# Genesis-Embodied-AI/ThinShellLab

Measured on AMD Instinct MI355X. Metric: element-steps/s (fwd+adjoint), 100k-tri cloth; 1/2/4/8-GPU scaling, higher is better.
Workload: dtype f64

## Files before the change

thinshelllab_amd/csrc/direct_group.hpp:

```cpp
#pragma once
#include <condition_variable>
#include <functional>
#include <thread>
#include "direct_host.hpp"

struct GroupPool {
  std::vector<std::thread> th;
  std::mutex mu;
  std::condition_variable cv, cv_done;
  std::function<int(int)> job;
  std::vector<int> rc;
  std::vector<std::string> err;
  int gen = 0, pending = 0, dev = 0;
  bool stop = false;
  void start(int n, int device) {
    dev = device; rc.assign(n, 0); err.assign(n, "");
    for (int i = 1; i < n; i++) th.emplace_back([this, i] {
      (void)hipSetDevice(dev);
      int seen = 0;
      for (;;) {
        std::unique_lock<std::mutex> lk(mu);
        cv.wait(lk, [&] { return stop || gen != seen; });
        if (stop) return;
        seen = gen;
// ... 40 lines not shown
  std::vector<tsl_ctx*> m;
  tsl_ctx* g = nullptr;
  DevBuf<double> vals, cH, vb, vx, arena, sarena, garena, w;
  std::vector<size_t> vals_off, cH_off, vec_off;
  std::vector<int> nv_off, nc_off;
  std::vector<size_t> cap_a, cap_s, cap_g, cap_w, off_a, off_s, off_g, off_w;
  std::vector<long> seen_gen;
  bool merged_valid = false;
  bool flow_lost = false;
  std::vector<hipEvent_t> ev_m;
  hipEvent_t ev_g = nullptr;
  long n_merge = 0, n_relayout = 0, n_own_path = 0;
  double t_merge = 0;
  std::unique_ptr<GroupPool> pool;
  ~tsl_group();
};

static inline size_t grp_align(size_t n) { return (n + 31) & ~(size_t)31; }

static int group_ensure_arenas(tsl_ctx* c) {
  tsl_group* G = c->group;
  std::lock_guard<std::mutex> lk(G->mu_layout);
  int me = -1;
  for (size_t i = 0; i < G->m.size(); i++) if (G->m[i] == c) me = (int)i;
  if (me < 0) return tsl_fail("scene group: context is not a member");
  const DirectPlan& P = c->ds.plan;
  if ((size_t)P.arena <= G->cap_a[me] && (size_t)P.sarena <= G->cap_s[me] && (size_t)P.garena <= G->cap_g[me] && (size_t)P.ylen <= G->cap_w[me]) return 0;
  HIP_OK(hipDeviceSynchronize());
  auto grow = [&](std::vector<size_t>& cap, size_t need) { if (need > cap[me]) cap[me] = grp_align(need + need / 4 + 32); };
  grow(G->cap_a, (size_t)P.arena); grow(G->cap_s, (size_t)P.sarena); grow(G->cap_g, (size_t)P.garena); grow(G->cap_w, (size_t)P.ylen);
  const size_t n = G->m.size();
  auto lay = [&](const std::vector<size_t>& cap, std::vector<size_t>& off, DevBuf<double>& buf, const char* what) -> int {
    size_t tot = 0;
    for (size_t i = 0; i < n; i++) { off[i] = tot; tot += cap[i]; }
    if (buf.n < tot) { if (buf.alloc(tot + tot / 16 + 32)) return tsl_fail("scene group: out of device memory (%.2f GB of %s for %zu scenes)", tot * 8e-9, what, n); }
    return 0;
  };
  TSL_TRY(lay(G->cap_a, G->off_a, G->arena, "front panels")); TSL_TRY(lay(G->cap_s, G->off_s, G->sarena, "Schur complements"));
  TSL_TRY(lay(G->cap_g, G->off_g, G->garena, "G panels")); TSL_TRY(lay(G->cap_w, G->off_w, G->w, "sweep vectors"));
  for (size_t i = 0; i < n; i++) {
    DirectSolver& d = G->m[i]->ds;
    d.arena.view(G->arena.p + G->off_a[i], G->cap_a[i]); d.sarena.view(G->sarena.p + G->off_s[i], G->cap_s[i]);
    d.garena.view(G->garena.p + G->off_g[i], G->cap_g[i]); d.w.view(G->w.p + G->off_w[i], G->cap_w[i]);
    d.numeric_valid = false; d.have_factor = false; d.prezero_pending = false;
  }
  DirectSolver& gd = G->g->ds;
  gd.arena.view(G->arena.p, G->arena.n); gd.sarena.view(G->sarena.p, G->sarena.n); gd.garena.view(G->garena.p, G->garena.n); gd.w.view(G->w.p, G->w.n);
  gd.numeric_valid = false; gd.have_factor = false; gd.prezero_pending = false;
  G->merged_valid = false;
  G->n_relayout++;
  return 0;
}

static int group_merge(tsl_group* G) {
  const auto t0 = std::chrono::steady_clock::now();
  tsl_ctx* g = G->g;
  DirectSolver& gd = g->ds;
  DirectPlan& M = gd.plan;
  hipStream_t s = g->stream;
  const int n = (int)G->m.size();
  HIP_OK(hipStreamSynchronize(s));
  if (gd.zstream) HIP_OK(hipStreamSynchronize(gd.zstream));
  gd.prezero_pending = false;
  std::vector<int> sn_base(n + 1, 0), pmap_base(n + 1, 0), vtx_base(n + 1, 0), ch_base(n + 1, 0);
  int L = 0, nc_tot = 0;
  for (int i = 0; i < n; i++) {
    const DirectSolver& d = G->m[i]->ds;
    if (!d.plan_valid) return tsl_fail("scene group: member %d has no plan", i);
    const DirectPlan& P = d.plan;
    sn_base[i + 1] = sn_base[i] + (int)P.fr.size(); pmap_base[i + 1] = pmap_base[i] + (int)P.pmap.size();
    vtx_base[i + 1] = vtx_base[i] + (int)P.vtx.size(); ch_base[i + 1] = ch_base[i] + (int)P.ch_rec.size();
    L = std::max(L, P.n_levels);
    nc_tot += G->m[i]->nc;
    if ((long long)pmap_base[i] + (long long)P.pmap.size() > 0x7fffffffLL) return tsl_fail("scene group: child tables exceed 2^31 entries");
  }
  g->nc = nc_tot;
  M.n_cu = G->m[0]->ds.plan.n_cu; M.split_small = G->m[0]->ds.plan.split_small; M.split_rem = G->m[0]->ds.plan.split_rem;
  M.fr.resize(sn_base[n]); M.pmap.resize(pmap_base[n]); M.ch_rec.resize(ch_base[n]);
  std::vector<int> vtxp(vtx_base[n]), owner(sn_base[n]);
  M.arena = (long long)G->arena.n; M.sarena = (long long)G->sarena.n; M.garena = (long long)G->garena.n; M.ylen = (long long)G->w.n;
  M.flops = 0; M.leaf_ranges.clear(); M.arena_leaf = 0;
  std::vector<std::vector<int>> by_level(L);
  std::vector<int> all(n);
  for (int i = 0; i < n; i++) all[i] = i;
  TSL_TRY(G->pool->run(all, [&](int i) -> int {
    tsl_ctx* c = G->m[i];
    const DirectPlan& P = c->ds.plan;
    const long long oa = (long long)G->off_a[i], os = (long long)G->off_s[i], og = (long long)G->off_g[i];
    const int ow = (int)G->off_w[i];
    for (size_t q = 0; q < P.fr.size(); q++) {
      DsFrontDesc f = P.fr[q];
      f.off += oa; f.off21 += oa; f.soff += os; f.goff += og;
      if (f.parent >= 0) f.parent += sn_base[i];
      f.pmap_off += pmap_base[i]; f.vtx_off += vtx_base[i]; f.yoff += ow; f.ch_off += ch_base[i];
      for (int k = 0; k < std::min(4, f.nchild); k++) { f.cpm[k] += pmap_base[i]; f.cy[k] += ow; }
      M.fr[sn_base[i] + q] = f;
      owner[sn_base[i] + q] = i;
    }
    std::copy(P.pmap.begin(), P.pmap.end(), M.pmap.begin() + pmap_base[i]);
    for (size_t q = 0; q < P.vtx.size(); q++) vtxp[vtx_base[i] + q] = c->h_rowpos[P.vtx[q]] + G->nv_off[i];
    for (size_t q = 0; q < P.ch_rec.size(); q++) {
      DsChildRec r = P.ch_rec[q];
      r.soff += os; r.pmap_off += pmap_base[i]; r.sn += sn_base[i]; r.yoff += ow;
      M.ch_rec[ch_base[i] + q] = r;
    }
    return 0;
  }));
  for (int i = 0; i < n; i++) {
    const DirectPlan& P = G->m[i]->ds.plan;
    for (int l = 0; l < P.n_levels; l++)
      for (int q = P.level_ptr[l]; q < P.level_ptr[l + 1]; q++) by_level[l].push_back(sn_base[i] + P.level_sn[q]);
    M.flops += P.flops;
    M.leaf_ranges.push_back({(long long)G->off_a[i], P.arena_leaf});
    M.arena_leaf += P.arena_leaf;
  }
  M.build_levels(by_level);
  {
    const int wb = gd.gemv_wide_below;
    M.wl_front.clear(); M.wl_row.clear(); M.wl_own_ptr.assign(L + 1, 0); M.wl_bnd_ptr.assign(L, 0); M.wl_own_wide.assign(L, 0); M.wl_bnd_wide.assign(L, 0);
    for (int l = 0; l < L; l++) {
      auto wide = [&](int i, bool bnd) {
        const DirectPlan& P = G->m[i]->ds.plan;
        if (l >= P.n_levels) return false;
        const int cnt = bnd ? P.wl_own_ptr[l + 1] - P.wl_bnd_ptr[l] : P.wl_bnd_ptr[l] - P.wl_own_ptr[l];
        return wb > 0 && cnt < wb;
      };
      M.wl_own_ptr[l] = (int)M.wl_front.size();
      for (int part = 0; part < 2; part++) {
        if (part == 1) M.wl_own_wide[l] = (int)M.wl_front.size();
        for (int q = M.level_ptr[l]; q < M.level_ptr[l + 1]; q++) {
          const int sfr = M.level_sn[q];
          if ((int)wide(owner[sfr], false) != part) continue;
          for (int r = 0; r < M.fr[sfr].p; r += 16) { M.wl_front.push_back(sfr); M.wl_row.push_back(r); }
        }
      }
      M.wl_bnd_ptr[l] = (int)M.wl_front.size();
      for (int part = 0; part < 2; part++) {
        if (part == 1) M.wl_bnd_wide[l] = (int)M.wl_front.size();
        for (int q = M.level_ptr[l]; q < M.level_ptr[l + 1]; q++) {
          const int sfr = M.level_sn[q];
          if ((int)wide(owner[sfr], true) != part) continue;
          for (int r = 0; r < M.fr[sfr].b; r += 16) { M.wl_front.push_back(sfr); M.wl_row.push_back(r); }
        }
      }
    }
    M.wl_own_ptr[L] = (int)M.wl_front.size();
  }
  M.level_maxld.assign(L, 0);
  for (int l = 0; l < L; l++) for (int q = M.level_ptr[l]; q < M.level_ptr[l + 1]; q++) M.level_maxld[l] = std::max(M.level_maxld[l], M.fr[M.level_sn[q]].ld);
  size_t nbk = 0, ngr = 0, nge = 0;
  for (int i = 0; i < n; i++) { const DirectPlan& P = G->m[i]->ds.plan; nbk += P.blk_q.size(); ngr += P.cgr_dst.size(); nge += P.cgr_ent.size(); }
  std::vector<int> src(nbk), ld(nbk), cg_ptr, cg_ent, cg_ld;
  std::vector<long long> dst(nbk), cg_dst;
  cg_ptr.reserve(ngr + 1); cg_ent.reserve(nge); cg_ld.reserve(ngr); cg_dst.reserve(ngr);
  M.blk_lptr.assign(L + 1, 0); M.cgr_lptr.assign(L + 1, 0);
  {
    std::vector<size_t> at((size_t)L * n, 0);
    size_t o = 0;
    for (int l = 0; l < L; l++) {
      for (int i = 0; i < n; i++) {
        tsl_ctx* c = G->m[i];
        const DirectPlan& P = c->ds.plan;
        if (l >= P.n_levels) continue;
        if (G->vals_off[i] + c->vals.n > 0x7fffffffULL) return tsl_fail("scene group: matrix values exceed 2^31 doubles");
        at[(size_t)l * n + i] = o;
        o += (size_t)(P.blk_lptr[l + 1] - P.blk_lptr[l]);
        if (c->nc > 0 && !P.cgr_lptr.empty()) {
          const long long oa = (long long)G->off_a[i];
          const int eo = 16 * G->nc_off[i];
          for (int gq = P.cgr_lptr[l]; gq < P.cgr_lptr[l + 1]; gq++) {
            cg_ptr.push_back((int)cg_ent.size());
            for (int e = P.cgr_ptr[gq]; e < P.cgr_ptr[gq + 1]; e++) cg_ent.push_back(P.cgr_ent[e] + eo);
            cg_dst.push_back(P.cgr_dst[gq] + oa); cg_ld.push_back(P.cgr_ld[gq]);
          }
        }
      }
      M.blk_lptr[l + 1] = (int)o;
      M.cgr_lptr[l + 1] = (int)cg_dst.size();
    }
    cg_ptr.push_back((int)cg_ent.size());
    TSL_TRY(G->pool->run(all, [&](int i) -> int {
      tsl_ctx* c = G->m[i];
      const DirectPlan& P = c->ds.plan;
      const int vo = (int)G->vals_off[i];
      const long long oa = (long long)G->off_a[i];
      for (int l = 0; l < P.n_levels; l++) {
        size_t w = at[(size_t)l * n + i];
        for (int k = P.blk_lptr[l]; k < P.blk_lptr[l + 1]; k++, w++) { const int q = P.blk_q[k]; src[w] = c->ds.h_c2s[q] + vo; dst[w] = P.blk_dst[q] + oa; ld[w] = P.blk_ld[q]; }
      }
      return 0;
    }));
  }
  std::vector<DsFrontDesc> frl(M.level_sn.size());
  for (size_t i = 0; i < frl.size(); i++) frl[i] = M.fr[M.level_sn[i]];
  ds_pin_reset(gd, 16 * nbk + 2 * sizeof(DsFrontDesc) * M.fr.size() + sizeof(DsChildRec) * M.ch_rec.size() +
                       4 * (M.level_sn.size() + M.pmap.size() + vtxp.size() + M.wl_front.size() + M.wl_row.size()) + 20 * (cg_ent.size() + cg_ptr.size()) + 64 * 256);
  TSL_TRY(ds_upload_grow(gd.fr, M.fr, s, &gd)); TSL_TRY(ds_upload_grow(gd.frl, frl, s, &gd)); TSL_TRY(ds_upload_grow(gd.level_sn, M.level_sn, s, &gd));
  TSL_TRY(ds_upload_grow(gd.pmap, M.pmap, s, &gd)); TSL_TRY(ds_upload_grow(gd.ch_rec, M.ch_rec, s, &gd)); TSL_TRY(ds_upload_grow(gd.vtx, vtxp, s, &gd));
  TSL_TRY(ds_upload_grow(gd.blk_q, src, s, &gd)); TSL_TRY(ds_upload_grow(gd.blk_dst, dst, s, &gd)); TSL_TRY(ds_upload_grow(gd.blk_ld, ld, s, &gd));
  TSL_TRY(ds_upload_grow(gd.cgr_ptr, cg_ptr, s, &gd)); TSL_TRY(ds_upload_grow(gd.cgr_ent, cg_ent, s, &gd)); TSL_TRY(ds_upload_grow(gd.cgr_ld, cg_ld, s, &gd)); TSL_TRY(ds_upload_grow(gd.cgr_dst, cg_dst, s, &gd));
  TSL_TRY(ds_upload_grow(gd.wl_front, M.wl_front, s, &gd)); TSL_TRY(ds_upload_grow(gd.wl_row, M.wl_row, s, &gd));
  if (gd.scr.n < (size_t)M.scratch) { if (gd.scr.alloc((size_t)M.scratch + (size_t)M.scratch / 8)) return -1; }
  HIP_OK(hipStreamSynchronize(s));
  gd.plan_valid = true; gd.numeric_valid = false; gd.have_factor = false;
  for (int i = 0; i < n; i++) G->seen_gen[i] = G->m[i]->ds.plan_gen;
  G->merged_valid = true;
  G->n_merge++;
  G->t_merge += std::chrono::duration<double>(std::chrono::steady_clock::now() - t0).count();
  if (g->verbose >= 3)
    for (const DsBatch& b : M.batches) {
      fprintf(stderr, "[tsl]   merged level %2d: %5d fronts, pivots <= %4d, boundary <= %4d, dataflow workgroups %ld (cap %d)%s; fronts by padded pivot count:", b.level, b.count, b.max_pp, b.max_bp,
              ds_flow_wgs(M, b), gd.flow_cap, ds_use_small(gd, b) ? " (LDS kernel)" : "");
      for (int q = 0, run = 0; q < b.count; q++) {
        run++;
        if (q + 1 == b.count || M.fr[M.level_sn[b.first + q + 1]].pp != M.fr[M.level_sn[b.first + q]].pp) { fprintf(stderr, " %d x %d", run, M.fr[M.level_sn[b.first + q]].pp); run = 0; }
      }
      fprintf(stderr, "\n");
    }
  if (g->verbose >= 2)
    fprintf(stderr, "[tsl] scene group: merged plan of %d scenes: %zu fronts, %d levels, %zu batches, %.1f GFLOP per factorisation, %d constraints; host %.2f ms\n", n, M.fr.size(), L, M.batches.size(),
            M.flops * 1e-9, nc_tot, 1e3 * std::chrono::duration<double>(std::chrono::steady_clock::now() - t0).count());
  return 0;
}

static int group_create(tsl_ctx* const* ctxs, int n, tsl_group** out) {
  if (n < 1 || n > 64) return tsl_fail("tsl_group_create: 1..64 scenes");
  int dev = ctxs[0]->ds.device;
  for (int i = 0; i < n; i++) {
    if (ctxs[i]->group) return tsl_fail("tsl_group_create: scene %d is a member of another group", i);
    if (ctxs[i]->ds.device != dev) return tsl_fail("tsl_group_create: the scenes of a group live on one device");
    for (int j = 0; j < i; j++) if (ctxs[j] == ctxs[i]) return tsl_fail("tsl_group_create: scene %d listed twice", i);
  }
  HIP_OK(hipDeviceSynchronize());
  std::unique_ptr<tsl_group> G(new tsl_group());
  G->m.assign(ctxs, ctxs + n);
  G->vals_off.resize(n); G->cH_off.resize(n); G->vec_off.resize(n); G->nv_off.resize(n); G->nc_off.resize(n);
  for (auto* v : {&G->cap_a, &G->cap_s, &G->cap_g, &G->cap_w, &G->off_a, &G->off_s, &G->off_g, &G->off_w}) v->assign(n, 0);
  G->seen_gen.assign(n, -1);
  size_t tv = 0, th = 0, tx = 0;
  int tnv = 0, tnc = 0;
  for (int i = 0; i < n; i++) {
    tsl_ctx* c = ctxs[i];
    G->vals_off[i] = tv; tv += grp_align(c->vals.n);
    G->cH_off[i] = th; G->nc_off[i] = tnc; th += c->c_H.n; tnc += (int)(c->c_H.n / 144);
    G->vec_off[i] = tx; G->nv_off[i] = tnv; tx += 3 * (size_t)c->NV; tnv += c->NV;
    if (c->c_H.n % 144) return tsl_fail("tsl_group_create: contact block buffer of scene %d is not a multiple of 144 doubles", i);
  }
  TSL_TRY(G->vals.alloc(tv + 32)); TSL_TRY(G->cH.alloc(th + 144)); TSL_TRY(G->vb.alloc(tx + 32)); TSL_TRY(G->vx.alloc(tx + 32));
  HIP_OK(hipMemset(G->vals.p, 0, G->vals.n * sizeof(double)));
  tsl_ctx* g = new tsl_ctx();
  G->g = g;
  g->NV = tnv; g->nc = 0; g->verbose = ctxs[0]->verbose;
  HIP_OK(hipStreamCreateWithFlags(&g->stream, hipStreamNonBlocking));
  g->vals.view(G->vals.p, G->vals.n); g->c_H.view(G->cH.p, G->cH.n);
  DirectSolver& gd = g->ds;
  const DirectSolver& d0 = ctxs[0]->ds;
  gd.merged = true; gd.enable = 1; gd.device = dev; gd.flow = d0.flow; gd.small_rounds = d0.small_rounds * n; gd.xcd_map = d0.xcd_map; gd.gemv_wide_below = d0.gemv_wide_below;
  gd.g32_below = d0.g32_below; gd.piv_tol = d0.piv_tol; gd.prezero = d0.prezero;
  gd.static_ready = true;
  if (gd.bad.alloc(DS_BAD_INTS)) return -1;
  HIP_OK(hipFuncSetAttribute((const void*)k_ds_inv_small, hipFuncAttributeMaxDynamicSharedMemorySize, (int)ds_small_lds(DS_SMALL)));
  HIP_OK(hipEventCreateWithFlags(&G->ev_g, hipEventDisableTiming));
  G->ev_m.assign(n, nullptr);
  for (int i = 0; i < n; i++) HIP_OK(hipEventCreateWithFlags(&G->ev_m[i], hipEventDisableTiming));
  for (int i = 0; i < n; i++) {
    tsl_ctx* c = ctxs[i];
    auto copy = [&](const DevBuf<double>& b, double* dstp, size_t cnt) -> int {
      if (b.n && b.p) HIP_OK(hipMemcpy(dstp, b.p, std::min(b.n, cnt) * sizeof(double), hipMemcpyDeviceToDevice));
      return 0;
    };
    TSL_TRY(copy(c->vals, G->vals.p + G->vals_off[i], c->vals.n)); TSL_TRY(copy(c->c_H, G->cH.p + G->cH_off[i], c->c_H.n));
    TSL_TRY(copy(c->v_b, G->vb.p + G->vec_off[i], 3 * (size_t)c->NV)); TSL_TRY(copy(c->v_x, G->vx.p + G->vec_off[i], 3 * (size_t)c->NV));
    DirectSolver& d = c->ds;
    if (d.prezero_pending) { HIP_OK(hipEventSynchronize(d.ev_zero)); d.prezero_pending = false; }
  }
  HIP_OK(hipDeviceSynchronize());
  for (int i = 0; i < n; i++) {
    tsl_ctx* c = ctxs[i];
    const size_t nvals = c->vals.n, nch = c->c_H.n;
    c->vals.view(G->vals.p + G->vals_off[i], nvals); c->c_H.view(G->cH.p + G->cH_off[i], nch);
    c->v_b.view(G->vb.p + G->vec_off[i], 3 * (size_t)c->NV); c->v_x.view(G->vx.p + G->vec_off[i], 3 * (size_t)c->NV);
    DirectSolver& d = c->ds;
    d.arena.release(); d.sarena.release(); d.garena.release(); d.w.release();
    d.arena.view(nullptr, 0); d.sarena.view(nullptr, 0); d.garena.view(nullptr, 0); d.w.view(nullptr, 0);
    d.plan_valid = false; d.numeric_valid = false; d.have_factor = false; d.cons_checked = false;
    for (auto& sl : d.cache) sl->used = false;
  }
  for (int i = 0; i < n; i++) { ctxs[i]->group = G.get(); ctxs[i]->ds.token_lender = &gd; ctxs[i]->ds.keep_host_maps = true; ds_flow_token_release(ctxs[i]->ds); }
  G->pool.reset(new GroupPool());
  if (n > 1 && !getenv("TSL_GROUP_NO_THREADS")) G->pool->start(n, dev);
  *out = G.release();
  return 0;
}

static void group_destroy(tsl_group* G) {
  if (!G) return;
  G->pool.reset();
  (void)hipDeviceSynchronize();
  for (tsl_ctx* c : G->m) {
    auto give = [&](DevBuf<double>& b) {
      const double* src = b.p; const size_t cnt = b.n;
      b.view(nullptr, 0); b.release();
      if (cnt && b.alloc(cnt) == 0) (void)hipMemcpy(b.p, src, cnt * sizeof(double), hipMemcpyDeviceToDevice);
      else if (cnt) fprintf(stderr, "[tsl] scene group: out of device memory while a member took back a buffer of %zu doubles: the member is left with an EMPTY buffer (its next call fails loudly)\n", cnt);
    };
    give(c->vals); give(c->c_H); give(c->v_b); give(c->v_x);
    DirectSolver& d = c->ds;
    d.arena.release(); d.sarena.release(); d.garena.release(); d.w.release();
    d.plan_valid = false; d.numeric_valid = false; d.have_factor = false; d.cons_checked = false; d.prezero_pending = false;
    for (auto& sl : d.cache) sl->used = false;
    d.token_lender = nullptr; d.keep_host_maps = false;
    c->group = nullptr;
  }
  delete G;
}

tsl_group::~tsl_group() {
  pool.reset();
  if (g) {
    ds_flow_token_release(g->ds);
    DirectSolver& gd = g->ds;
    if (gd.zstream) (void)hipStreamDestroy(gd.zstream);
    for (int k = 0; k < DS_NSIDE; k++) if (gd.fstream[k]) (void)hipStreamDestroy(gd.fstream[k]);
    if (gd.pin) (void)hipHostFree(gd.pin);
    if (g->stream) (void)hipStreamDestroy(g->stream);
    delete g;
    g = nullptr;
  }
  for (hipEvent_t e : ev_m) if (e) (void)hipEventDestroy(e);
  if (ev_g) (void)hipEventDestroy(ev_g);
}
```

thinshelllab_amd/csrc/direct_host.hpp:

```cpp
#pragma once
#include <array>
#include <chrono>

#include "k_direct.hpp"
#include "tsl_ctx.hpp"

#include <cerrno>
#include <fcntl.h>
#include <sys/file.h>
#include <sys/stat.h>
#include <unistd.h>
static void ds_flow_token_acquire(DirectSolver& d) {
  char bus[64] = "dev";
  if (hipDeviceGetPCIBusId(bus, sizeof(bus), d.device) != hipSuccess) { (void)hipGetLastError(); snprintf(bus, sizeof(bus), "dev%d", d.device); }
  for (char* q = bus; *q; q++) if (*q == ':' || *q == '/') *q = '_';
  d.flow_token = -1; d.flow_token_asked = d.n_factor;
  for (const char* dir : {"/dev/shm", "/tmp"}) {
    const std::string path = std::string(dir) + "/tsl_flow_" + bus;
    int fd = open(path.c_str(), O_RDWR | O_CLOEXEC);
    if (fd < 0 && errno == ENOENT) {
      fd = open(path.c_str(), O_CREAT | O_RDWR | O_CLOEXEC, 0666);
      if (fd < 0 && (errno == ENOENT || errno == ENOTDIR)) continue;
      if (fd < 0 && errno == EEXIST) fd = open(path.c_str(), O_RDWR | O_CLOEXEC);
    } else if (fd < 0 && errno == ENOTDIR) continue;
    if (fd < 0) return;
    (void)fchmod(fd, 0666);
    if (flock(fd, LOCK_EX | LOCK_NB) == 0) { d.flow_token = 1; d.flow_token_fd = fd; }
    else close(fd);
    return;
  }
}
static void ds_flow_token_release(DirectSolver& d) {
  if (d.flow_token_fd >= 0) { (void)flock(d.flow_token_fd, LOCK_UN); close(d.flow_token_fd); }
  d.flow_token_fd = -1; d.flow_token = 0;
}
static bool ds_flow_token_held(DirectSolver& d) {
  if (d.token_lender) return ds_flow_token_held(*d.token_lender);
  if (d.flow_token == 0 || (d.flow_token < 0 && d.n_factor - d.flow_token_asked >= 256)) ds_flow_token_acquire(d);
  return d.flow_token > 0;
}

static inline int ds_nblk(long n, int b) { return (int)((n + b - 1) / b); }

static inline bool ds_use_small(const DirectSolver& d, const DsBatch& b) {
  if (b.max_pp > DS_SMALL) return false;
  return (size_t)b.count <= (size_t)d.plan.n_cu * ds_small_per_cu(b.max_pp) * (size_t)d.small_rounds;
}

static void ds_launch_gemm(hipStream_t s, const DsDev& D, const DsBatch& b, int mode, int ds_xcd_map, int ds_g32_below = 0, int part = 0, int max_lead = 0) {
  const int rows = mode == 0 ? b.max_pp : b.max_bp, cols = b.max_bp;
  const dim3 grid((cols + 63) / 64, (rows + 63) / 64, b.count);
  const long tiles = (long)grid.x * grid.y * grid.z;
  const int ta = (max_lead + 63) / 64;
  if (part == 1 && ta == 0) return;
  if (mode == 1 && part != 0) {
    hipLaunchKernelGGL((k_ds_gemm<1, 4>), part == 1 ? dim3(ta, ta, b.count) : grid, dim3(256), 0, s, D, b.first, part);
    return;
  }
  if (mode == 0 && ds_g32_below > 0 && tiles < ds_g32_below) {
    hipLaunchKernelGGL(k_ds_gemm_g32, dim3(part == 1 ? 2 * ta : (cols + 31) / 32, (rows + 31) / 32, b.count), dim3(256), 0, s, D, b.first, part);
    return;
  }
  if (mode == 0 && part != 0) {
    hipLaunchKernelGGL((k_ds_gemm<0, 4>), part == 1 ? dim3(ta, grid.y, b.count) : grid, dim3(256), 0, s, D, b.first, part);
    return;
  }
  if (ds_xcd_map > 0 && b.count >= ds_xcd_map) {
    const int gx = grid.x, gy = grid.y, nf = b.count;
    const long ng = ((long)nf + 7) / 8 * 8 * gx * gy;
    if (mode == 0) hipLaunchKernelGGL((k_ds_gemm_x<0, 4>), dim3((unsigned)ng), dim3(256), 0, s, D, b.first, gx, gy, nf);
    else hipLaunchKernelGGL((k_ds_gemm_x<1, 4>), dim3((unsigned)ng), dim3(256), 0, s, D, b.first, gx, gy, nf);
    return;
  }
  if (mode == 0) hipLaunchKernelGGL((k_ds_gemm<0, 4>), grid, dim3(256), 0, s, D, b.first, 0);
  else hipLaunchKernelGGL((k_ds_gemm<1, 4>), grid, dim3(256), 0, s, D, b.first, 0);
}
static void ds_launch_extend(hipStream_t s, const DsDev& D, int lv0, int nf, int max_ld, int part = 0, int max_span = 0) {
  const int xspan = part == 1 ? 64 * DS_XU : DS_XSPAN;
  const int nsp = ((part == 0 ? max_ld : max_span) + xspan - 1) / xspan;
  if (nsp <= 0) return;
  hipLaunchKernelGGL(k_ds_extend_panels, dim3(((max_ld / 3 + 2 + 3) / 4) * nsp, nf), dim3(256), 0, s, D, lv0, nsp, part, xspan);
}
static void ds_launch_level_start(tsl_ctx* c, hipStream_t s, const DsDev& D, int l, int part = 0, const DsBatch* b = nullptr) {
  DirectSolver& d = c->ds;
  const DirectPlan& P = d.plan;
  const int lv0 = P.level_ptr[l], nf = P.level_ptr[l + 1] - lv0;
  if (l > 0) ds_launch_extend(s, D, lv0, nf, P.level_maxld[l], part, part == 0 ? 0 : part == 1 ? b->max_pp : std::max(b->max_bp, b->max_pp));
  const int i0 = part == 2 ? P.blk_lmid[l] : P.blk_lptr[l], i1 = part == 1 ? P.blk_lmid[l] : P.blk_lptr[l + 1];
  const int nb = i1 - i0, npad = part == 2 ? 0 : nf;
  const long nt = (long)nb * 9 + (long)npad * DS_T;
  if (nt > 0)
    hipLaunchKernelGGL(k_ds_assemble_level, dim3(ds_nblk(nt, 256)), dim3(256), 0, s, i0, nb, (const int*)d.blk_q.p, (const double*)c->vals.p, (const long long*)d.blk_dst.p,
                       (const int*)d.blk_ld.p, lv0, npad, d.frl.p, d.arena.p, l == 0 ? 1 : 0);
  if (c->nc > 0) {
    const int g0 = part == 2 ? P.cgr_lmid[l] : P.cgr_lptr[l], g1 = part == 1 ? P.cgr_lmid[l] : P.cgr_lptr[l + 1];
    const int ng = g1 - g0;
    if (ng > 0) hipLaunchKernelGGL(k_ds_assemble_contacts_level, dim3(ds_nblk((long)ng * 64, 256)), dim3(256), 0, s, g0, ng, (const int*)d.cgr_ptr.p, (const int*)d.cgr_ent.p,
                                   (const long long*)d.cgr_dst.p, (const int*)d.cgr_ld.p, (const double*)c->c_H.p, d.arena.p);
  }
}


static long ds_flow_wgs(const DirectPlan& P, const DsBatch& b) {
  long n = 0;
  for (int z = 0; z < b.count; z++) { const long ns = (P.fr[P.level_sn[b.first + z]].pp / DS_T + DS_FLOW_B - 1) / DS_FLOW_B; n += ns * ns; }
  return n;
}
static bool ds_flow_eligible(DirectSolver& d, const DirectPlan& P, const DsBatch& b, hipStream_t s) {
  if (!d.flow || b.count > DS_FLOW_MAXF || b.max_pp < 2 * DS_T) return false;
  { hipStreamCaptureStatus cs = hipStreamCaptureStatusNone;
    if (hipStreamIsCapturing(s, &cs) != hipSuccess || cs != hipStreamCaptureStatusNone) return false; }
  if (!ds_flow_token_held(d)) return false;
  if (ds_use_small(d, b) && !(d.flow & 2)) return false;
  if (d.flow_cap == 0) {
    int occ = 0, dev = 0;
    hipDeviceProp_t prop;
    if (hipGetDevice(&dev) != hipSuccess || hipGetDeviceProperties(&prop, dev) != hipSuccess ||
        hipOccupancyMaxActiveBlocksPerMultiprocessor(&occ, (const void*)k_ds_gj_flow<DS_FLOW_B>, 256, 0) != hipSuccess) { d.flow_cap = -1; return false; }
    d.flow_cap = std::max(1, occ * prop.multiProcessorCount);
    if (getenv("TSL_FLOW_DEBUG")) fprintf(stderr, "[tsl] k_ds_gj_flow: %d workgroups per CU x %d CUs resident\n", occ, prop.multiProcessorCount);
  }
  return ds_flow_wgs(P, b) <= d.flow_cap;
}
static bool ds_flow_prepare(DirectSolver& d, const DirectPlan& P, const DsBatch& b, bool flow_free, DsFlowArgs& a, hipStream_t s) {
  if (!flow_free || !ds_flow_eligible(d, P, b, s)) return false;
  long wgs = 0, x = 0, fl = 0;
  for (int z = 0; z < b.count; z++) {
    const long nt = P.fr[P.level_sn[b.first + z]].pp / DS_T, ns = (nt + DS_FLOW_B - 1) / DS_FLOW_B;
    a.tile0[z] = (int)wgs; a.xoff[z] = x; a.foff[z] = (int)fl;
    wgs += ns * ns; x += (nt + 2 * nt * nt) * (DS_T * DS_T); fl += 32 * nt + 2 * nt * nt;
  }
  a.tile0[b.count] = (int)wgs; a.nf = b.count;
  if (d.flow_x.n < (size_t)x) { if (d.flow_x.alloc((size_t)x)) return false; }
  if (d.flow_f.n < (size_t)fl) {
    if (d.flow_f.alloc((size_t)fl + 1024)) return false;
    if (hipMemsetAsync(d.flow_f.p, 0, d.flow_f.n * sizeof(int), s) != hipSuccess) return false;
  }
  a.epoch = ++d.flow_epoch;
  return true;
}
#define DS_FLOW_PIECES 4
static std::vector<DsBatch> ds_flow_pieces(DirectSolver& d, const DirectPlan& P, const DsBatch& b, bool flow_free, hipStream_t s) {
  std::vector<DsBatch> out;
  if (!flow_free) return out;
  if (ds_flow_eligible(d, P, b, s)) { out.push_back(b); return out; }
  if (ds_use_small(d, b) || b.count < 2) return out;
  DsBatch one = b;
  one.count = 1;
  if (!ds_flow_eligible(d, P, one, s) || d.flow_cap <= 0) return out;
  int start = 0;
  while (start < b.count) {
    DsBatch pc{};
    pc.first = b.first + start; pc.level = b.level; pc.act_off = b.act_off;
    long wgs = 0;
    while (start + pc.count < b.count && pc.count < DS_FLOW_MAXF) {
      const DsFrontDesc& f = P.fr[P.level_sn[pc.first + pc.count]];
      const long ns = (f.pp / DS_T + DS_FLOW_B - 1) / DS_FLOW_B;
      if (pc.count > 0 && wgs + ns * ns > d.flow_cap) break;
      wgs += ns * ns; pc.count++;
      pc.max_pp = std::max(pc.max_pp, f.pp); pc.max_bp = std::max(pc.max_bp, f.bp); pc.max_ld = std::max(pc.max_ld, f.ld);
    }
    if (pc.max_pp < 2 * DS_T || !ds_flow_eligible(d, P, pc, s) || (int)out.size() == DS_FLOW_PIECES) { out.clear(); return out; }
    out.push_back(pc);
    start += pc.count;
  }
  return out;
}
static void ds_flow_launch(hipStream_t s, const DsDev& D, int lv0, const DsFlowArgs& fa, DirectSolver& d) {
  hipLaunchKernelGGL(k_ds_gj_flow<DS_FLOW_B>, dim3(fa.tile0[fa.nf]), dim3(256), 0, s, D, lv0, fa, d.flow_x.p, d.flow_f.p);
}

static bool direct_enabled(tsl_ctx* c) {
  DirectSolver& d = c->ds;
  if (d.enable == 0) return false;
  if (d.enable == 1) return true;
  for (const DsGrid& g : d.grids) if ((long)g.N * g.M >= 1024) return true;
  return false;
}

static DsDev ds_dev(tsl_ctx* c) {
  DirectSolver& d = c->ds;
  DsDev D;
  D.fr = d.fr.p; D.frl = d.frl.p; D.level_sn = d.level_sn.p; D.A = d.arena.p; D.S = d.sarena.p; D.Y = d.w.p; D.G = d.garena.p; D.scr = d.scr.p; D.ch = d.ch_rec.p; D.pmap = d.pmap.p; D.vtx = d.vtx.p; D.bad = d.bad.p; D.dbg = d.dbg; D.piv_tol = d.piv_tol;
  D.tlog = (d.dbg == 30 && d.tlog.n >= 1024) ? d.tlog.p : nullptr;
  return D;
}

static void ds_pin_reset(DirectSolver& d, size_t need) {
  if (d.pin_cap < need) {
    if (d.pin) (void)hipHostFree(d.pin);
    d.pin = nullptr; d.pin_cap = 0;
    void* p = nullptr;
    if (hipHostMalloc(&p, need + need / 4) == hipSuccess) { d.pin = (char*)p; d.pin_cap = need + need / 4; }
    else (void)hipGetLastError();
  }
  d.pin_off = 0;
}
static void* ds_pin_take(DirectSolver& d, size_t bytes) {
  const size_t o = (d.pin_off + 255) & ~(size_t)255;
  if (!d.pin || o + bytes > d.pin_cap) return nullptr;
  d.pin_off = o + bytes;
  return d.pin + o;
}
template <class T>
static int ds_upload_grow(DevBuf<T>& buf, const std::vector<T>& h, hipStream_t s, DirectSolver* d = nullptr) {
  if (buf.n < h.size()) { if (buf.alloc(h.size() + h.size() / 4 + 16)) return -1; }
  if (h.empty()) return 0;
  const void* src = h.data();
  if (d) if (void* st = ds_pin_take(*d, h.size() * sizeof(T))) { memcpy(st, h.data(), h.size() * sizeof(T)); src = st; }
  HIP_OK(hipMemcpyAsync(buf.p, src, h.size() * sizeof(T), hipMemcpyHostToDevice, s));
  return 0;
}

static int ds_upload_con(DirectSolver& d, hipStream_t s) {
  const DirectPlan& P = d.plan;
  TSL_TRY(ds_upload_grow(d.cgr_ptr, P.cgr_ptr, s, &d)); TSL_TRY(ds_upload_grow(d.cgr_ent, P.cgr_ent, s, &d)); TSL_TRY(ds_upload_grow(d.cgr_ld, P.cgr_ld, s, &d));
  TSL_TRY(ds_upload_grow(d.cgr_dst, P.cgr_dst, s, &d));
  return 0;
}

static int direct_static(tsl_ctx* c) {
  DirectSolver& d = c->ds;
  if (d.static_ready) return 0;
  const int NV = c->NV;
  d.row_ptr.assign(NV + 1, 0);
  for (int v = 0; v < NV; v++) d.row_ptr[v + 1] = d.row_ptr[v] + (int)c->h_rows[v].size();
  std::vector<int> c2s(d.row_ptr[NV]);
  for (int v = 0; v < NV; v++) {
    const int p = c->h_rowpos[v], s = p >> 6, lane = p & 63;
    for (int k = 0; k < (int)c->h_rows[v].size(); k++) c2s[d.row_ptr[v] + k] = (int)(((long)c->h_slice_off[s] + 64L * k) * 9 + lane);
  }
  d.h_c2s = c2s;
  if (d.bad.alloc(DS_BAD_INTS)) return -1;
  HIP_OK(hipFuncSetAttribute((const void*)k_ds_inv_small, hipFuncAttributeMaxDynamicSharedMemorySize, (int)ds_small_lds(DS_SMALL)));
  { hipDeviceProp_t prop;
    if (hipGetDeviceProperties(&prop, d.device) == hipSuccess && prop.multiProcessorCount > 0) d.plan.n_cu = prop.multiProcessorCount; else (void)hipGetLastError(); }
  d.plan.sym.build_partition(NV, c->h_rows, d.grids, d.blocks, d.leaf);
  d.cache.clear();
  d.static_ready = true;
  d.plan_valid = false;
  return 0;
}

static uint64_t ds_cons_key(const std::vector<int>& cons) {
  uint64_t h = 1469598103934665603ull;
  for (int v : cons) { h ^= (uint64_t)(uint32_t)v; h *= 1099511628211ull; }
  return h ^ (uint64_t)cons.size();
}
static void ds_swap_slot(DirectSolver& d, DsPlanSlot& sl) {
  std::swap(d.plan, sl.plan); d.h_cons.swap(sl.h_cons); d.h_cset.swap(sl.h_cset);
  if (!d.keep_host_maps) { d.plan.blk_dst.swap(sl.plan.blk_dst); d.plan.blk_ld.swap(sl.plan.blk_ld); d.plan.blk_q.swap(sl.plan.blk_q); d.plan.pmap.swap(sl.plan.pmap); }
  d.plan.lists.swap(sl.plan.lists); d.plan.locs.swap(sl.plan.locs); d.plan.tpos.swap(sl.plan.tpos);
  d.level_sn.swap(sl.level_sn); d.pmap.swap(sl.pmap); d.ch_rec.swap(sl.ch_rec); d.vtx.swap(sl.vtx); d.blk_ld.swap(sl.blk_ld); 
  d.wl_front.swap(sl.wl_front); d.wl_row.swap(sl.wl_row); d.blk_dst.swap(sl.blk_dst); d.fr.swap(sl.fr); d.frl.swap(sl.frl); d.blk_q.swap(sl.blk_q); d.cgr_ptr.swap(sl.cgr_ptr); d.cgr_ent.swap(sl.cgr_ent); d.cgr_ld.swap(sl.cgr_ld); d.cgr_dst.swap(sl.cgr_dst);
}

static size_t ds_slot_bytes(const DsPlanSlot& sl) {
  const DirectPlan& P = sl.plan;
  size_t b = 4 * (sl.level_sn.n + sl.pmap.n + sl.vtx.n + sl.blk_ld.n + sl.cgr_ptr.n + sl.cgr_ent.n + sl.cgr_ld.n + sl.wl_front.n + sl.wl_row.n + sl.blk_q.n) + 8 * (sl.blk_dst.n + sl.cgr_dst.n) +
             sizeof(DsFrontDesc) * (sl.fr.n + sl.frl.n) + sizeof(DsChildRec) * sl.ch_rec.n;
  b += 4 * (P.pmap.size() + P.vtx.size() + P.blk_ld.size() + P.blk_q.size() + P.wl_front.size() + P.wl_row.size() + P.level_sn.size()) + 8 * P.blk_dst.size() + sizeof(DsFrontDesc) * P.fr.size();
  return b;
}
static void ds_cache_trim(DirectSolver& d) {
  for (;;) {
    size_t total = 0;
    DsPlanSlot* lru = nullptr;
    for (auto& sl : d.cache) if (sl->used) { total += ds_slot_bytes(*sl); if (!lru || sl->stamp < lru->stamp) lru = sl.get(); }
    if (!lru || total <= (size_t)d.cache_mb << 20) return;
    lru->used = false;
    lru->level_sn.release(); lru->pmap.release(); lru->vtx.release(); lru->blk_ld.release(); lru->cgr_ptr.release(); lru->cgr_ent.release(); lru->cgr_ld.release(); lru->cgr_dst.release(); lru->wl_front.release(); lru->wl_row.release();
    lru->blk_q.release(); lru->blk_dst.release(); lru->fr.release(); lru->frl.release(); lru->ch_rec.release();
    d.n_plan_evicted++;
  }
}

static int group_ensure_arenas(tsl_ctx* c);
static int direct_plan(tsl_ctx* c) {
  DirectSolver& d = c->ds;
  if (d.merged) return 0;
  hipStream_t s = c->stream;
  TSL_TRY(direct_static(c));
  if (d.plan_valid && d.cons_checked) return 0;
  std::vector<int> cons((size_t)c->nc * 4);
  if (c->nc > 0) {
    HIP_OK(hipMemcpyAsync(cons.data(), c->c_idx.p, cons.size() * sizeof(int), hipMemcpyDeviceToHost, s));
    HIP_OK(hipStreamSynchronize(s));
  }
  d.cons_checked = true;
  if (d.plan_valid && cons == d.h_cons) return 0;
  std::vector<std::array<int, 4>> canon((size_t)c->nc);
  for (int e = 0; e < c->nc; e++) canon[e] = {cons[4 * e], cons[4 * e + 1], cons[4 * e + 2], cons[4 * e + 3]};
  std::sort(canon.begin(), canon.end());
  std::vector<int> cset((size_t)c->nc * 4);
  for (int e = 0; e < c->nc; e++) for (int k = 0; k < 4; k++) cset[4 * e + k] = canon[e][k];
  auto same_set_new_order = [&]() -> int {
    if (cons != d.h_cons) {
      HIP_OK(hipStreamSynchronize(s));
      if (d.plan.build_con(cons.data(), c->nc)) return tsl_fail("direct solver: constraint vertex outside its front");
      ds_pin_reset(d, 20 * (d.plan.cgr_ent.size() + d.plan.cgr_ptr.size()) + 4096);
      TSL_TRY(ds_upload_con(d, s));
      HIP_OK(hipStreamSynchronize(s));
      d.h_cons = cons;
      d.plan_gen++;
    }
    d.numeric_valid = false; d.have_factor = false;
    return 0;
  };
  if (d.plan_valid && cset == d.h_cset) return same_set_new_order();
  if (d.cache_cap > 0) {
    const uint64_t key = ds_cons_key(cset);
    HIP_OK(hipStreamSynchronize(s));
    for (auto& sl : d.cache)
      if (sl->used && sl->key == key && sl->h_cset == cset) {
        ds_swap_slot(d, *sl);
        sl->used = d.plan_valid; sl->key = ds_cons_key(sl->h_cset); sl->stamp = ++d.cache_clock;
        d.plan_valid = true;
        d.n_plan_hits++; d.plan_gen++;
        if (c->group) TSL_TRY(group_ensure_arenas(c));
        if (c->verbose >= 2) fprintf(stderr, "[tsl] direct plan: cached plan reused (nc %d, %d supernodes)\n", c->nc, d.plan.sym.n_sn);
        return same_set_new_order();
      }
    if (d.plan_valid) {
      DsPlanSlot* dst = nullptr;
      for (auto& sl : d.cache) if (!sl->used) { dst = sl.get(); break; }
      if (!dst && (int)d.cache.size() < d.cache_cap) {
        d.cache.emplace_back(new DsPlanSlot());
        dst = d.cache.back().get();
        dst->plan.sym.copy_partition(d.plan.sym); dst->plan.threads = d.plan.threads; dst->plan.n_cu = d.plan.n_cu; dst->plan.split_small = d.plan.split_small; dst->plan.split_rem = d.plan.split_rem;
      }
      if (!dst) { for (auto& sl : d.cache) if (!dst || sl->stamp < dst->stamp) dst = sl.get(); }
      ds_swap_slot(d, *dst);
      dst->used = true; dst->key = ds_cons_key(dst->h_cset); dst->stamp = ++d.cache_clock;
      d.plan_valid = false;
      ds_cache_trim(d);
    }
  }
  const auto t0 = std::chrono::steady_clock::now();
  const int rc = d.plan.build(c->h_rows, d.row_ptr, cons.data(), c->nc);
  const auto t_build = std::chrono::steady_clock::now();
  if (rc) return tsl_fail("direct solver: inconsistent elimination tree (code %d)", rc);
  DirectPlan& P = d.plan;
  std::vector<int> vtxp(P.vtx.size());
  for (size_t i = 0; i < vtxp.size(); i++) vtxp[i] = c->h_rowpos[P.vtx[i]];
  HIP_OK(hipStreamSynchronize(s));
  const size_t nbk = P.blk_q.size();
  ds_pin_reset(d, 16 * nbk + 2 * sizeof(DsFrontDesc) * P.fr.size() + sizeof(DsChildRec) * P.ch_rec.size() +
                      4 * (P.level_sn.size() + P.pmap.size() + vtxp.size() + P.wl_front.size() + P.wl_row.size()) + 20 * (P.cgr_ent.size() + P.cgr_ptr.size()) + 64 * 256);
  TSL_TRY(ds_upload_grow(d.fr, P.fr, s, &d)); TSL_TRY(ds_upload_grow(d.level_sn, P.level_sn, s, &d)); TSL_TRY(ds_upload_grow(d.pmap, P.pmap, s, &d)); TSL_TRY(ds_upload_grow(d.ch_rec, P.ch_rec, s, &d));
  TSL_TRY(ds_upload_grow(d.vtx, vtxp, s, &d));
  {
    std::vector<int> src_v, ld_v;
    std::vector<long long> dst_v;
    int* src_l = (int*)ds_pin_take(d, 4 * nbk); int* ld_l = (int*)ds_pin_take(d, 4 * nbk); long long* dst_l = (long long*)ds_pin_take(d, 8 * nbk);
    if (!src_l || !ld_l || !dst_l) { src_v.resize(nbk); ld_v.resize(nbk); dst_v.resize(nbk); src_l = src_v.data(); ld_l = ld_v.data(); dst_l = dst_v.data(); }
    ds_parallel_for((int)((nbk + 4095) / 4096), P.n_threads(), 1, [&](int, int ch) {
      for (size_t i = (size_t)ch * 4096; i < std::min(nbk, (size_t)(ch + 1) * 4096); i++) { const int q = P.blk_q[i]; src_l[i] = d.h_c2s[q]; dst_l[i] = P.blk_dst[q]; ld_l[i] = P.blk_ld[q]; }
    });
    if (d.blk_dst.n < nbk) { if (d.blk_dst.alloc(nbk + nbk / 4 + 16)) return -1; }
    if (d.blk_ld.n < nbk) { if (d.blk_ld.alloc(nbk + nbk / 4 + 16)) return -1; }
    if (d.blk_q.n < nbk) { if (d.blk_q.alloc(nbk + nbk / 4 + 16)) return -1; }
    if (nbk > 0) {
      HIP_OK(hipMemcpyAsync(d.blk_dst.p, dst_l, 8 * nbk, hipMemcpyHostToDevice, s));
      HIP_OK(hipMemcpyAsync(d.blk_ld.p, ld_l, 4 * nbk, hipMemcpyHostToDevice, s));
      HIP_OK(hipMemcpyAsync(d.blk_q.p, src_l, 4 * nbk, hipMemcpyHostToDevice, s));
      if (!src_v.empty()) HIP_OK(hipStreamSynchronize(s));
    }
  }
  TSL_TRY(ds_upload_con(d, s));
  std::vector<DsFrontDesc> frl(P.level_sn.size());
  for (size_t i = 0; i < frl.size(); i++) frl[i] = P.fr[P.level_sn[i]];
  TSL_TRY(ds_upload_grow(d.frl, frl, s, &d));
  TSL_TRY(ds_upload_grow(d.wl_front, P.wl_front, s, &d)); TSL_TRY(ds_upload_grow(d.wl_row, P.wl_row, s, &d));
  if (c->group) TSL_TRY(group_ensure_arenas(c));
  else {
    if (d.prezero_pending && d.arena.n < (size_t)P.arena) { HIP_OK(hipEventSynchronize(d.ev_zero)); d.prezero_pending = false; }
    if (d.arena.n < (size_t)P.arena) { if (d.arena.alloc((size_t)P.arena + (size_t)P.arena / 8)) return tsl_fail("direct solver: out of device memory (%.2f GB of front panels)", P.arena * 8e-9); }
    if (d.sarena.n < (size_t)P.sarena) { if (d.sarena.alloc((size_t)P.sarena + (size_t)P.sarena / 8 + 16)) return tsl_fail("direct solver: out of device memory (%.2f GB of Schur complements)", P.sarena * 8e-9); }
    if (d.garena.n < (size_t)P.garena) { if (d.garena.alloc((size_t)P.garena + (size_t)P.garena / 8 + 16)) return tsl_fail("direct solver: out of device memory (G arena)"); }
    if (d.w.n < (size_t)P.ylen) { if (d.w.alloc((size_t)P.ylen + (size_t)P.ylen / 4 + 16)) return -1; }
  }
  if (d.scr.n < (size_t)P.scratch) { if (d.scr.alloc((size_t)P.scratch + (size_t)P.scratch / 8)) return -1; }
  HIP_OK(hipStreamSynchronize(s));
  d.h_cons.swap(cons); d.h_cset.swap(cset);
  d.plan_valid = true;
  d.numeric_valid = false;
  d.have_factor = false;
  d.n_plans++; d.plan_gen++;
  d.t_plan += std::chrono::duration<double>(std::chrono::steady_clock::now() - t0).count();
  if (c->verbose >= 2)
    fprintf(stderr, "[tsl] direct plan: %d supernodes, %d levels, %zu batches, %.2f + %.2f GB of panels + Schur complements, %.1f GFLOP per factorisation, nc %d; host %.2f ms (tree + maps %.2f)\n", P.sym.n_sn, P.n_levels, P.batches.size(), P.arena * 8e-9, P.sarena * 8e-9,
            P.flops * 1e-9, c->nc, 1e3 * std::chrono::duration<double>(std::chrono::steady_clock::now() - t0).count(), 1e3 * std::chrono::duration<double>(t_build - t0).count());
  if (c->verbose >= 2) fprintf(stderr, "[tsl]   plan phases (ms): tree %.2f, descriptors + parent maps %.2f, levels %.2f, static block map %.2f, contact map %.2f\n", P.phase_ms[0], P.phase_ms[1], P.phase_ms[2], P.phase_ms[3], P.phase_ms[4]);
  if (c->verbose >= 3)
    for (const DsBatch& b : P.batches) {
      fprintf(stderr, "[tsl]   level %2d: %5d fronts, pivots <= %4d, boundary <= %4d%s; fronts by padded pivot count:", b.level, b.count, b.max_pp, b.max_bp, ds_use_small(d, b) ? " (LDS kernel)" : "");
      for (int q = 0, run = 0; q < b.count; q++) {
        run++;
        if (q + 1 == b.count || P.fr[P.level_sn[b.first + q + 1]].pp != P.fr[P.level_sn[b.first + q]].pp) { fprintf(stderr, " %d x %d", run, P.fr[P.level_sn[b.first + q]].pp); run = 0; }
      }
      fprintf(stderr, "\n");
    }
  return 0;
}

static int direct_prezero(tsl_ctx* c) {
  DirectSolver& d = c->ds;
  if (!d.prezero || !d.plan_valid || d.arena.n == 0 || d.prezero_pending) return 0;
  if (d.zstream == nullptr) {
    HIP_OK(hipStreamCreateWithFlags(&d.zstream, hipStreamNonBlocking));
    HIP_OK(hipEventCreateWithFlags(&d.ev_zfork, hipEventDisableTiming));
    HIP_OK(hipEventCreateWithFlags(&d.ev_zero, hipEventDisableTiming));
  }
  HIP_OK(hipEventRecord(d.ev_zfork, c->stream));
  HIP_OK(hipStreamWaitEvent(d.zstream, d.ev_zfork, 0));
  d.prezero_n = (size_t)d.plan.arena_leaf;
  if (d.plan.leaf_ranges.empty()) HIP_OK(hipMemsetAsync(d.arena.p, 0, d.prezero_n * sizeof(double), d.zstream));
  else for (const auto& r : d.plan.leaf_ranges) HIP_OK(hipMemsetAsync(d.arena.p + r.first, 0, (size_t)r.second * sizeof(double), d.zstream));
  HIP_OK(hipEventRecord(d.ev_zero, d.zstream));
  d.prezero_pending = true;
  d.numeric_valid = false; d.have_factor = false;
  return 0;
}

static void ds_launch_gemv(hipStream_t s, const DsDev& D, DirectSolver& d, int o, int n, int mode, const double* vin, double* vout, int wide_from = -1) {
  if (n <= 0) return;
  if (wide_from >= 0) {
    const int n0 = wide_from - o, n1 = o + n - wide_from;
    if (n0 > 0) hipLaunchKernelGGL(k_ds_gemv, dim3(n0), dim3(256), 0, s, D, d.wl_front.p, d.wl_row.p, o, mode, vin, vout);
    if (n1 > 0) hipLaunchKernelGGL(k_ds_gemv_wide, dim3(4 * n1), dim3(256), 0, s, D, d.wl_front.p, d.wl_row.p, wide_from, mode, vin, vout);
    return;
  }
  if (d.gemv_wide_below > 0 && n < d.gemv_wide_below) hipLaunchKernelGGL(k_ds_gemv_wide, dim3(4 * n), dim3(256), 0, s, D, d.wl_front.p, d.wl_row.p, o, mode, vin, vout);
  else hipLaunchKernelGGL(k_ds_gemv, dim3(n), dim3(256), 0, s, D, d.wl_front.p, d.wl_row.p, o, mode, vin, vout);
}
static void ds_sweep_up_level(hipStream_t s, const DsDev& D, DirectSolver& d, int l, const double* r, double* z) {
  const DirectPlan& P = d.plan;
  const int o0 = P.wl_own_ptr[l], b0 = P.wl_bnd_ptr[l], o1 = P.wl_own_ptr[l + 1];
  ds_launch_gemv(s, D, d, o0, b0 - o0, 0, r, z, P.wl_own_wide.empty() ? -1 : P.wl_own_wide[l]);
  ds_launch_gemv(s, D, d, b0, o1 - b0, 1, (const double*)z, nullptr, P.wl_bnd_wide.empty() ? -1 : P.wl_bnd_wide[l]);
}
static int direct_factor(tsl_ctx* c, int stop_sn = -1, const char* dump_path = nullptr, const double* eager_r = nullptr, double* eager_z = nullptr) {
  DirectSolver& d = c->ds;
  hipStream_t s = c->stream;
  TSL_TRY(direct_plan(c));
  if (d.numeric_valid) return 0;
  d.eager_n = 0;
  const DirectPlan& P = d.plan;
  const DsDev D = ds_dev(c);
  if (d.prezero_pending) {
    HIP_OK(hipStreamWaitEvent(s, d.ev_zero, 0));
    d.prezero_pending = false;
    if (P.leaf_ranges.empty() && d.prezero_n < (size_t)P.arena_leaf) HIP_OK(hipMemsetAsync(d.arena.p + d.prezero_n, 0, ((size_t)P.arena_leaf - d.prezero_n) * sizeof(double), s));
  } else if (P.leaf_ranges.empty()) HIP_OK(hipMemsetAsync(d.arena.p, 0, (size_t)P.arena_leaf * sizeof(double), s));
  else for (const auto& r : P.leaf_ranges) HIP_OK(hipMemsetAsync(d.arena.p + r.first, 0, (size_t)r.second * sizeof(double), s));
  HIP_OK(hipMemsetAsync(d.bad.p, 0, 8 * sizeof(int), s));
  bool swept_at_root = false;
  int flow_wgs_sent = 0;
  auto invert_batch = [&](const DsBatch& b, hipStream_t bs, bool& flow_free) {
    const int lv0 = b.first, nf = b.count;
    const int tp = b.max_pp / DS_T;
    bool flowed = false;
    {
      const std::vector<DsBatch> pieces = ds_flow_pieces(d, P, b, flow_free, bs);
      std::vector<DsFlowArgs> fas(pieces.size());
      bool ready = !pieces.empty();
      for (size_t i = 0; ready && i < pieces.size(); i++) ready = ds_flow_prepare(d, P, pieces[i], true, fas[i], bs);
      if (ready) {
        for (size_t i = 0; i < pieces.size(); i++) { ds_flow_launch(bs, D, pieces[i].first, fas[i], d); d.n_flow++; flow_wgs_sent += fas[i].tile0[fas[i].nf]; }
        flowed = true; flow_free = false;
      }
    }
    if (flowed) {}
    else if (ds_use_small(d, b)) hipLaunchKernelGGL(k_ds_inv_small, dim3(nf), dim3(256), ds_small_lds(b.max_pp), bs, D, lv0, b.max_pp + 1);
    else {
      hipLaunchKernelGGL(k_ds_pivot0, dim3(nf), dim3(256), 0, bs, D, lv0);
      for (int k = 0; k < tp; k++) { const int na = P.act_n[b.act_off + k]; hipLaunchKernelGGL(k_ds_gj_step, dim3(na + na * tp * tp), dim3(256), 0, bs, D, lv0, k, tp, na); }
      hipLaunchKernelGGL(k_ds_gj_finish, dim3(tp, nf), dim3(256), 0, bs, D, lv0);
    }
  };
  auto run_batch = [&](const DsBatch& b, hipStream_t bs, bool& flow_free) {
    invert_batch(b, bs, flow_free);
    if (b.max_bp > 0) {
      ds_launch_gemm(bs, D, b, 0, d.xcd_map, d.g32_below);
      ds_launch_gemm(bs, D, b, 1, d.xcd_map);
    }
  };
  auto side_streams = [&]() -> int {
    if (d.fstream[0] == nullptr)
      for (int k = 0; k < DS_NSIDE; k++) { HIP_OK(hipStreamCreateWithFlags(&d.fstream[k], hipStreamNonBlocking)); HIP_OK(hipEventCreateWithFlags(&d.ev_fjoin[k], hipEventDisableTiming)); }
    if (d.ev_ffork == nullptr) HIP_OK(hipEventCreateWithFlags(&d.ev_ffork, hipEventDisableTiming));
    for (int k = 0; k < 5; k++) if (d.ev_la[k] == nullptr) HIP_OK(hipEventCreateWithFlags(&d.ev_la[k], hipEventDisableTiming));
    if (d.lastream == nullptr) {
      int lo = 0, hi = 0;
      HIP_OK(hipDeviceGetStreamPriorityRange(&lo, &hi));
      HIP_OK(hipStreamCreateWithPriority(&d.lastream, hipStreamNonBlocking, lo));
    }
    return 0;
  };
  const bool la_on = (d.lookahead & 1) && stop_sn < 0 && !P.blk_lmid.empty() && P.la_from < P.n_levels && ds_flow_token_held(d);
  if (la_on) TSL_TRY(side_streams());
  hipStream_t ls = d.lastream;
  enum { LA_W = 0, LA_GA = 1, LA_A = 2, LA_REST = 3, LA_DRAIN = 4 };
  for (size_t bi = 0; bi < P.batches.size();) {
    size_t be = bi;
    while (be < P.batches.size() && P.batches[be].level == P.batches[bi].level) be++;
    bool stop_here = false;
    if (stop_sn >= 0) for (int q = P.batches[bi].first; q < P.batches[be - 1].first + P.batches[be - 1].count; q++) stop_here |= P.level_sn[q] == stop_sn;
    const int lvl = P.batches[bi].level;
    const bool la_level = la_on && lvl >= P.la_from;
    const bool la_in = la_level && lvl > P.la_from;
    if (la_in) {
      ds_launch_level_start(c, s, D, lvl, 1, &P.batches[bi]);
      HIP_OK(hipStreamWaitEvent(ls, d.ev_la[LA_A], 0));
      ds_launch_level_start(c, ls, D, lvl, 2, &P.batches[bi]);
      HIP_OK(hipEventRecord(d.ev_la[LA_REST], ls));
    } else
    ds_launch_level_start(c, s, D, lvl);
    if (la_level) {
      const DsBatch& b = P.batches[bi];
      bool flow_free = true;
      if (la_in && ds_flow_wgs(P, b) > P.n_cu) {
// ... 36 lines not shown
    }
    if (stop_here) {
      const DsFrontDesc& f = P.fr[stop_sn];
      std::vector<double> h((size_t)f.pp * f.ld);
      HIP_OK(hipStreamSynchronize(s));
      HIP_OK(hipMemcpy(h.data(), d.arena.p + f.off, h.size() * sizeof(double), hipMemcpyDeviceToHost));
      if (FILE* fp = fopen(dump_path, "wb")) {
        const int hdr[8] = {f.p, f.pp, f.b, f.bp, f.ld, f.nv_own, f.nv_bnd, 0};
        fwrite(hdr, sizeof(int), 8, fp);
        fwrite(&P.vtx[f.vtx_off], sizeof(int), (size_t)f.nv_own + f.nv_bnd, fp);
        fwrite(h.data(), sizeof(double), h.size(), fp);
        fclose(fp);
      }
      d.numeric_valid = false; d.have_factor = false;
      return 0;
    }
    const int nside = (int)std::min<size_t>(be - bi - 1, DS_NSIDE);
    if (nside > 0) {
      TSL_TRY(side_streams());
      HIP_OK(hipEventRecord(d.ev_ffork, s));
      for (int k = 0; k < nside; k++) HIP_OK(hipStreamWaitEvent(d.fstream[k], d.ev_ffork, 0));
    }
    bool flow_free = true;
    for (size_t q = bi; q < be; q++) {
      const int k = (int)(q - bi);
      run_batch(P.batches[q], (nside > 0 && k > 0) ? d.fstream[(k - 1) % nside] : s, flow_free);
    }
    for (int k = 0; k < nside; k++) { HIP_OK(hipEventRecord(d.ev_fjoin[k], d.fstream[k])); HIP_OK(hipStreamWaitEvent(s, d.ev_fjoin[k], 0)); }
    bi = be;
  }
  if (++d.anorm_age >= 64) d.anorm_valid = false;
  if (stop_sn >= 0 || c->verbose >= 2) HIP_OK(hipStreamSynchronize(s));
  if (d.dbg == 30) {
    if (d.tlog.n < 1024) { if (d.tlog.alloc(1024)) return -1; HIP_OK(hipMemset(d.tlog.p, 0, 1024 * sizeof(unsigned long long))); HIP_OK(hipMemset(d.tlog.p + 194, 0xff, sizeof(unsigned long long))); }
    else {
      unsigned long long h[1024];
      HIP_OK(hipStreamSynchronize(s));
      HIP_OK(hipMemcpy(h, d.tlog.p, sizeof(h), hipMemcpyDeviceToHost));
      int khz = 100000;
      (void)hipDeviceGetAttribute(&khz, hipDeviceAttributeWallClockRate, d.device);
      auto us = [&](unsigned long long t) { return t ? (double)(long long)(t - h[192]) * 1e3 / khz : -1.0; };
      fprintf(stderr, "[tsl] dataflow chain of the last launch (us since its start): pivot published | step finished by the last workgroup | by the first of the last super-row; first workgroup started at %.2f, last ended at %.2f\n", us(h[194]), us(h[193]));
      for (int k = 0; k < 64 && (h[k] || h[64 + k]); k++) {
        fprintf(stderr, "[tsl]   %2d  %8.2f (+%5.2f)   %8.2f   %8.2f   | owner of the pivot, relative to the publication of the previous one: flags seen, operands in LDS, R' done, tile updated, inverted:", k, us(h[k]), k ? us(h[k]) - us(h[k - 1]) : 0.0, us(h[64 + k]), us(h[128 + k]));
        for (int i = 0; i < 5; i++) fprintf(stderr, " %6.2f", h[256 + 8 * k + i] && k ? us(h[256 + 8 * k + i]) - us(h[k - 1]) : 0.0);
        fprintf(stderr, "\n");
      }
      HIP_OK(hipMemset(d.tlog.p, 0, 1024 * sizeof(unsigned long long)));
      HIP_OK(hipMemset(d.tlog.p + 194, 0xff, sizeof(unsigned long long)));
    }
  }
  if (swept_at_root) HIP_OK(hipStreamWaitEvent(s, d.ev_la[LA_DRAIN], 0));
  HIP_OK(hipGetLastError());
  d.flow_wgs_last = flow_wgs_sent;
  d.numeric_valid = true;
  d.have_factor = true;
  d.n_factor++;
  return 0;
}

static int direct_anorm(tsl_ctx* c) {
  DirectSolver& d = c->ds;
  if (d.anorm_valid) return 0;
  hipStream_t s = c->stream;
  if (d.anorm_dev.n == 0 && d.anorm_dev.alloc(1)) return -1;
  if (d.h_anorm == nullptr) HIP_OK(hipHostMalloc((void**)&d.h_anorm, sizeof(double)));
  HIP_OK(hipMemsetAsync(d.anorm_dev.p, 0, sizeof(double), s));
  hipLaunchKernelGGL(k_ds_rownorm, dim3(ds_nblk(c->NV, 256)), dim3(256), 0, s, c->NV, c->slice_off.p, c->slice_len.p, c->vals.p, d.anorm_dev.p);
  HIP_OK(hipMemcpyAsync(d.h_anorm, d.anorm_dev.p, sizeof(double), hipMemcpyDeviceToHost, s));
  HIP_OK(hipStreamSynchronize(s));
  d.anorm = *d.h_anorm;
  d.anorm_valid = true; d.anorm_age = 0;
  return 0;
}

static int direct_apply(tsl_ctx* c, const double* r, double* z) {
  DirectSolver& d = c->ds;
  hipStream_t s = c->stream;
  const DirectPlan& P = d.plan;
  const DsDev D = ds_dev(c);
  const int l0 = (d.eager_n > 0 && r == d.eager_r && z == d.eager_z) ? d.eager_n : 0;
  d.eager_n = 0;
  for (int l = l0; l < P.n_levels; l++) ds_sweep_up_level(s, D, d, l, r, z);
  for (int l = P.n_levels - 2; l >= 0; l--) {
    const int o0 = P.wl_own_ptr[l], b0 = P.wl_bnd_ptr[l];
    ds_launch_gemv(s, D, d, o0, b0 - o0, 2, (const double*)z, z, P.wl_own_wide.empty() ? -1 : P.wl_own_wide[l]);
  }
  d.n_apply++;
  return 0;
}

static int direct_bench(tsl_ctx* c, int cls, int reps, double* out) {
  DirectSolver& d = c->ds;
  hipStream_t s = c->stream;
  if (!d.plan_valid || d.arena.n == 0) return tsl_fail("tsl_bench_direct: no factorisation yet");
  if (d.prezero_pending) { HIP_OK(hipStreamWaitEvent(s, d.ev_zero, 0)); d.prezero_pending = false; }
  const DirectPlan& P = d.plan;
  if (!d.have_factor) {
    HIP_OK(hipMemsetAsync(d.arena.p, 0x3F, (size_t)P.arena * sizeof(double), s));
    HIP_OK(hipMemsetAsync(d.sarena.p, 0x3F, (size_t)P.sarena * sizeof(double), s));
    HIP_OK(hipMemsetAsync(d.garena.p, 0x3F, (size_t)P.garena * sizeof(double), s));
  }
  const DsDev D = ds_dev(c);
  if (cls == 0 || cls == 3 || cls == 5) {
    HIP_OK(hipMemsetAsync(d.arena.p, 0x3F, (size_t)P.arena * sizeof(double), s));
    hipLaunchKernelGGL(k_ds_bench_diag, dim3((unsigned)P.fr.size()), dim3(256), 0, s, D);
    d.have_factor = false;
  }
  double flops = 0, bytes = 0;
  long launches = 0;
  auto child_entries = [&](const DsFrontDesc& f, double& to_s, double& to_panels) {
    to_s = 0; to_panels = 0;
    for (int q = f.ch_off; q < f.ch_off + f.nchild; q++) {
      const DsChildRec& cr = P.ch_rec[q];
      const double nb = cr.nb, b = cr.b;
      to_s += nb * nb; to_panels += b * b - nb * nb;
    }
  };
  auto issue = [&](bool count) {
    if (cls == 4) {
      (void)direct_apply(c, c->v_b.p, c->v_t4.p);
      d.n_apply--;
      if (count) {
        for (int l = 0; l < P.n_levels; l++) launches += 1 + (P.wl_own_ptr[l + 1] > P.wl_bnd_ptr[l]) + (l < P.n_levels - 1);
        for (const DsFrontDesc& f : P.fr) { bytes += 8.0 * ((double)f.p * f.p + 2.0 * (double)f.p * f.b); flops += 2.0 * ((double)f.p * f.p + 2.0 * (double)f.p * f.b); }
      }
      return;
    }
    if (cls == 7) {
      const int bq = d.bench_batch;
      if (bq < 1 || bq >= (int)P.batches.size()) return;
      const DsBatch& bf = P.batches[bq];
      const DsBatch& bg = P.batches[bq - 1];
      DsFlowArgs fa;
      if (!ds_flow_prepare(d, P, bf, true, fa, s) || bg.max_bp == 0) return;
      (void)hipEventRecord(d.ev_ffork, s);
      (void)hipStreamWaitEvent(d.fstream[0], d.ev_ffork, 0);
      ds_flow_launch(s, D, bf.first, fa, d);
      ds_launch_gemm(d.fstream[0], D, bg, 0, d.xcd_map, d.g32_below);
      ds_launch_gemm(d.fstream[0], D, bg, 1, d.xcd_map);
      (void)hipEventRecord(d.ev_fjoin[0], d.fstream[0]);
      (void)hipStreamWaitEvent(s, d.ev_fjoin[0], 0);
      if (count) launches++;
      return;
    }
    int bi = -1;
    for (const DsBatch& b : P.batches) {
      bi++;
      if (d.bench_batch >= 0 && bi != d.bench_batch) continue;
      const int lv0 = b.first, nf = b.count;
      const int tp = b.max_pp / DS_T, tb = b.max_bp / DS_T;
      if (cls == 6) {
        if (b.level == 0) continue;
        ds_launch_extend(s, D, b.first, b.count, b.max_pp + b.max_bp);
        if (count) {
          launches++;
          for (int i = 0; i < nf; i++) {
            const DsFrontDesc& f = P.fr[P.level_sn[lv0 + i]];
            double to_s, to_p;
            child_entries(f, to_s, to_p);
            bytes += 8.0 * (to_p + (double)f.pp * f.ld + (double)f.bp * f.pp); flops += to_p;
          }
        }
      } else if (cls == 0 || cls == 3 || cls == 5) {
        bool flow_free = true;
        for (int q = 0; q < bi; q++) if (P.batches[q].level == b.level && !ds_flow_pieces(d, P, P.batches[q], true, s).empty()) flow_free = false;
        const std::vector<DsBatch> pieces = ds_flow_pieces(d, P, b, flow_free, s);
        const int mine = !pieces.empty() ? 5 : (ds_use_small(d, b) ? 3 : 0);
        if (mine != cls) continue;
        if (cls == 5) { for (const DsBatch& pc : pieces) { DsFlowArgs fa; if (ds_flow_prepare(d, P, pc, true, fa, s)) { ds_flow_launch(s, D, pc.first, fa, d); if (count) launches++; } } }
        else if (cls == 3) { hipLaunchKernelGGL(k_ds_inv_small, dim3(nf), dim3(256), ds_small_lds(b.max_pp), s, D, lv0, b.max_pp + 1); if (count) launches++; }
        else {
          hipLaunchKernelGGL(k_ds_pivot0, dim3(nf), dim3(256), 0, s, D, lv0);
          for (int k = 0; k < tp; k++) { const int na = P.act_n[b.act_off + k]; hipLaunchKernelGGL(k_ds_gj_step, dim3(na + na * tp * tp), dim3(256), 0, s, D, lv0, k, tp, na); }
          hipLaunchKernelGGL(k_ds_gj_finish, dim3(tp, nf), dim3(256), 0, s, D, lv0);
          if (count) launches += tp + 2;
        }
        if (count) for (int i = 0; i < nf; i++) {
          const DsFrontDesc& f = P.fr[P.level_sn[lv0 + i]];
          flops += 2.0 * (double)f.pp * f.pp * f.pp;
          bytes += 16.0 * (double)f.pp * f.pp * (cls != 0 ? 1.0 : f.pp / (double)DS_T);
        }
      } else if (tb > 0) {
        if (cls == 1 || cls == 2) ds_launch_gemm(s, D, b, cls == 2 ? 0 : 1, d.xcd_map, cls == 2 ? d.g32_below : 0);
        else continue;
        if (count) {
          launches++;
          for (int i = 0; i < nf; i++) {
            const DsFrontDesc& f = P.fr[P.level_sn[lv0 + i]];
            if (cls == 1) {
              double to_s, to_p;
              child_entries(f, to_s, to_p);
              flops += 2.0 * (double)f.bp * f.bp * f.pp; bytes += 8.0 * (2.0 * (double)f.bp * f.pp + (double)f.b * f.b + to_s);
            } else { flops += 2.0 * (double)f.pp * f.pp * f.bp; bytes += 8.0 * ((double)f.pp * f.pp + 2.0 * (double)f.pp * f.bp); }
          }
        }
      }
    }
  };
  if (d.ev0 == nullptr) { HIP_OK(hipEventCreate(&d.ev0)); HIP_OK(hipEventCreate(&d.ev1)); }
  if (cls == 7) {
    if (d.fstream[0] == nullptr)
      for (int k = 0; k < DS_NSIDE; k++) { HIP_OK(hipStreamCreateWithFlags(&d.fstream[k], hipStreamNonBlocking)); HIP_OK(hipEventCreateWithFlags(&d.ev_fjoin[k], hipEventDisableTiming)); }
    if (d.ev_ffork == nullptr) HIP_OK(hipEventCreateWithFlags(&d.ev_ffork, hipEventDisableTiming));
  }
  issue(true);
  HIP_OK(hipEventRecord(d.ev0, s));
  for (int r = 0; r < reps; r++) issue(false);
  HIP_OK(hipEventRecord(d.ev1, s));
  HIP_OK(hipEventSynchronize(d.ev1));
  HIP_OK(hipGetLastError());
  float ms = 0;
  HIP_OK(hipEventElapsedTime(&ms, d.ev0, d.ev1));
  d.numeric_valid = false; d.have_factor = false;
  out[0] = launches > 0 ? ms * 1e3 / ((double)launches * reps) : 0.0;
  out[1] = launches > 0 ? flops / launches : 0.0;
  out[2] = launches > 0 ? bytes / launches : 0.0;
  out[3] = (double)launches;
  return 0;
}
```

thinshelllab_amd/csrc/direct_plan.hpp:

```cpp
#pragma once
#include <atomic>
#include <chrono>
#include <thread>
#include "direct_sym.hpp"

#define DS_T 32
#define DS_SMALL 128
static inline size_t ds_small_lds(int max_pp) { return (size_t)max_pp * (max_pp + 1) * sizeof(double); }
static inline int ds_small_per_cu(int max_pp) { return (int)std::max<size_t>(1, std::min<size_t>(8, (160 * 1024) / (ds_small_lds(max_pp) + 5 * 1024))); }

struct DsFrontDesc {
  long long off;
  long long off21;
  long long soff;
  long long goff;
  int p, pp, b, bp, ld;
  int parent;
  int pmap_off;
  int vtx_off;
  int nv_own, nv_bnd;
  int scr_off;
  int yoff;
  int cpm[4], cy[4];
  int ch_off, nchild;
  int lead;
};
struct DsChildRec {
  long long soff;
  int bp, b;
  int pmap_off;
  int sn;
  int nb;
  int yoff;
};

struct DsBatch {
  int first, count, level;
  int max_pp, max_ld, max_bp;
  int act_off;
};

template <class F>
static void ds_parallel_for(int n, int nt, int chunk, F body) {
  nt = std::max(1, std::min(nt, (n + chunk - 1) / chunk));
  if (nt == 1) { for (int i = 0; i < n; i++) body(0, i); return; }
  std::atomic<int> next{0};
  auto work = [&](int t) {
    for (;;) {
      const int i0 = next.fetch_add(chunk);
      if (i0 >= n) break;
      for (int i = i0; i < std::min(n, i0 + chunk); i++) body(t, i);
    }
  };
  std::vector<std::thread> th;
  for (int t = 1; t < nt; t++) th.emplace_back(work, t);
  work(0);
  for (auto& x : th) x.join();
}

struct DirectPlan {
  DirectSym sym;
  std::vector<DsFrontDesc> fr;
  std::vector<int> pmap, vtx;
  std::vector<DsChildRec> ch_rec;
  std::vector<long long> blk_dst;
  std::vector<int> blk_ld;
  std::vector<int> blk_q, blk_lptr;
  std::vector<int> blk_lmid, cgr_lmid;
  int la_from = 1 << 30;
  std::vector<long long> con_dst;
  std::vector<int> con_ld, con_lvl;
  std::vector<int> cgr_lptr, cgr_ptr, cgr_ent, cgr_ld;
  std::vector<long long> cgr_dst;
  std::vector<int> level_maxld;
  long long arena_leaf = 0;
  std::vector<std::pair<long long, long long>> leaf_ranges;
  std::vector<int> wl_own_wide, wl_bnd_wide;
  std::vector<std::vector<int>> lists;
  std::vector<int> level_ptr, level_sn;
  std::vector<DsBatch> batches;
  std::vector<int> act_n, act_ld;
  std::vector<int> sweep_cache; int sweep_cache_L0 = -1;
  std::vector<int> wl_front, wl_row, wl_own_ptr, wl_bnd_ptr;
  int n_levels = 0;
  long long arena = 0;
  long long sarena = 0;
  long long garena = 0;
  long long ylen = 0;
  long long scratch = 0;
  double phase_ms[6] = {0, 0, 0, 0, 0, 0};
  std::vector<int> tpos;
  std::vector<std::vector<int>> locs;
  int threads = 0;
  int n_cu = 256;
  bool split_small = true, split_rem = true;
  int n_threads() const { return threads > 0 ? threads : (int)std::max(1u, std::min(8u, std::thread::hardware_concurrency())); }
  double flops = 0;

  static int pad(int n) { return (n + DS_T - 1) / DS_T * DS_T; }

  int local_dof(int s, int v) const {
    const int l = sym.local(s, v);
    if (l < 0) return -1;
    const int no = sym.own(s);
    return l < no ? 3 * l : fr[s].pp + 3 * (l - no);
  }
  static long long panel_addr(const DsFrontDesc& f, int lr, int lc, int* ld_out) {
    if (lr < f.pp) { *ld_out = f.ld; return f.off + (long long)lr * f.ld + lc; }
    if (lc >= f.pp) { *ld_out = 0; return -1; }
    *ld_out = f.pp;
    return f.off21 + (long long)(lr - f.pp) * f.pp + lc;
  }

  void build_levels(std::vector<std::vector<int>>& by_level) {
    const int L = (int)by_level.size();
    n_levels = L;
    level_ptr.assign(L + 1, 0); level_sn.clear();
    batches.clear(); act_n.clear(); act_ld.clear();
    wl_front.clear(); wl_row.clear(); wl_own_ptr.assign(L + 1, 0); wl_bnd_ptr.assign(L, 0);
    sweep_cache_L0 = -1;
    scratch = 0;
    for (int l = 0; l < L; l++) {
      std::vector<int>& fl = by_level[l];
      std::stable_sort(fl.begin(), fl.end(), [&](int a, int b) { return fr[a].pp > fr[b].pp; });
      long long scr = 0;
      for (size_t i = 0; i < fl.size(); i++) {
        const int s = fl[i];
        DsFrontDesc& f = fr[s];
        if (i == 0 || 4 * f.pp <= batches.back().max_pp || (fl.size() > 256 && batches.back().count >= 32 && f.pp < fr[fl[i - 1]].pp) ||
            (split_small && batches.back().max_pp > DS_SMALL && f.pp <= DS_SMALL && 2 * f.pp <= batches.back().max_pp)) {
          DsBatch b{};
          b.first = (int)level_sn.size(); b.count = 0; b.level = l;
          batches.push_back(b);
        }
        DsBatch& b = batches.back();
        b.count++;
        b.max_pp = std::max(b.max_pp, f.pp); b.max_ld = std::max(b.max_ld, f.ld); b.max_bp = std::max(b.max_bp, f.bp);
        level_sn.push_back(s);
        f.scr_off = (int)scr;
        scr += 2LL * DS_T * DS_T + 4LL * DS_T * f.pp;
      }
      if (split_rem)
        for (size_t q = 0; q < batches.size(); q++) {
          DsBatch& b = batches[q];
          if (b.level != l || b.max_pp > DS_SMALL) continue;
          const int cap = n_cu * ds_small_per_cu(b.max_pp), rem = b.count % cap;
          if (b.count <= cap || rem == 0 || rem > cap / 8) continue;
          DsBatch r{};
          r.first = b.first + b.count - rem; r.count = rem; r.level = l;
          b.count -= rem;
          for (int z = 0; z < r.count; z++) { const DsFrontDesc& f = fr[level_sn[r.first + z]]; r.max_pp = std::max(r.max_pp, f.pp); r.max_ld = std::max(r.max_ld, f.ld); r.max_bp = std::max(r.max_bp, f.bp); }
          b.max_ld = 0; b.max_bp = 0;
          for (int z = 0; z < b.count; z++) { const DsFrontDesc& f = fr[level_sn[b.first + z]]; b.max_ld = std::max(b.max_ld, f.ld); b.max_bp = std::max(b.max_bp, f.bp); }
          batches.insert(batches.begin() + q + 1, r);
          q++;
        }
      level_ptr[l + 1] = (int)level_sn.size();
      scratch = std::max(scratch, scr);
      wl_own_ptr[l] = (int)wl_front.size();
      for (int s : fl) for (int r = 0; r < fr[s].p; r += 16) { wl_front.push_back(s); wl_row.push_back(r); }
      wl_bnd_ptr[l] = (int)wl_front.size();
      for (int s : fl) for (int r = 0; r < fr[s].b; r += 16) { wl_front.push_back(s); wl_row.push_back(r); }
    }
    wl_own_ptr[L] = (int)wl_front.size();
    {
      std::vector<int> nb(L, 0);
      for (const DsBatch& b : batches) nb[b.level]++;
      int l0 = L;
      while (l0 > 0 && nb[l0 - 1] == 1) l0--;
      la_from = (L - l0 >= 2) ? std::max(l0, 1) : (1 << 30);
    }
    for (DsBatch& b : batches) {
      b.act_off = (int)act_n.size();
      for (int k = 0; k * DS_T < b.max_pp; k++) {
        int n = 0, mld = 0;
        while (n < b.count && fr[level_sn[b.first + n]].pp > k * DS_T) { mld = std::max(mld, fr[level_sn[b.first + n]].ld); n++; }
        act_n.push_back(n); act_ld.push_back(mld);
      }
    }
  }

  int build(const std::vector<std::vector<int>>& adj, const std::vector<int>& row_ptr, const int* cons, int n_cons) {
    auto tick = std::chrono::steady_clock::now();
    auto lap = [&](int k) { const auto n = std::chrono::steady_clock::now(); phase_ms[k] = 1e3 * std::chrono::duration<double>(n - tick).count(); tick = n; };
    sym.build_tree(adj, cons, n_cons, 4);
    lap(0);
    const int S = sym.n_sn;
    fr.assign(S, DsFrontDesc{});
    pmap.clear(); vtx.clear(); ch_rec.clear();
    arena = 0; sarena = 0; garena = 0; flops = 0; ylen = 0;
    for (int s = 0; s < S; s++) {
      DsFrontDesc& f = fr[s];
      f.nv_own = sym.own(s); f.nv_bnd = (int)sym.bnd[s].size();
      f.p = 3 * f.nv_own; f.b = 3 * f.nv_bnd;
      f.pp = pad(f.p); f.bp = pad(f.b); f.ld = f.pp + f.bp;
      f.parent = sym.parent[s];
      f.vtx_off = (int)vtx.size();
      for (int q = sym.sn_ptr[s]; q < sym.sn_ptr[s + 1]; q++) vtx.push_back(sym.order[q]);
      for (int v : sym.bnd[s]) vtx.push_back(v);
      const double p = f.pp, b = f.bp;
      flops += 2.0 * p * p * p + 2.0 * p * p * b + 2.0 * p * b * b;
    }
    {
      std::vector<int> cnt(sym.n_levels + 1, 0), ord(S);
      for (int s = 0; s < S; s++) cnt[sym.level[s] + 1]++;
      for (int l = 0; l < sym.n_levels; l++) cnt[l + 1] += cnt[l];
      for (int s = 0; s < S; s++) ord[cnt[sym.level[s]]++] = s;
      for (int s : ord) {
        DsFrontDesc& f = fr[s];
        f.off = arena; f.off21 = arena + (long long)f.pp * f.ld;
        arena += (long long)f.pp * f.ld + (long long)f.bp * f.pp;
        f.soff = sarena; sarena += (long long)f.bp * f.bp;
        f.goff = garena; garena += (long long)f.pp * f.bp;
        f.yoff = (int)ylen; ylen += f.bp;
      }
    }
    {
      std::vector<int> cptr(S + 1, 0);
      for (int s = 0; s < S; s++) if (fr[s].parent >= 0) { cptr[fr[s].parent + 1]++; fr[fr[s].parent].nchild++; }
      for (int s = 0; s < S; s++) cptr[s + 1] += cptr[s];
      ch_rec.assign(cptr[S], DsChildRec{});
      long long total = 0;
      { std::vector<int> fill(cptr.begin(), cptr.end() - 1);
        for (int s = 0; s < S; s++) { fr[s].ch_off = cptr[s]; if (fr[s].parent >= 0) { fr[s].pmap_off = (int)total; total += fr[fr[s].parent].ld; ch_rec[fill[fr[s].parent]++].sn = s; } } }
      if (total > 0x7fffffffLL) return -1;
      pmap.assign((size_t)total, -1);
      if (locs.empty()) locs.resize(1);
      std::vector<int>& lc = locs[0];
      if ((int)lc.size() != sym.NV) lc.assign(sym.NV, -1);
      bool bad = false;
      for (int p = 0; p < S; p++) {
        if (cptr[p] == cptr[p + 1]) continue;
        const DsFrontDesc& f = fr[p];
        const int* fv = &vtx[f.vtx_off];
        for (int i = 0; i < f.nv_own; i++) lc[fv[i]] = 3 * i;
        for (int i = 0; i < f.nv_bnd; i++) lc[fv[f.nv_own + i]] = f.pp + 3 * i;
        for (int q = cptr[p]; q < cptr[p + 1]; q++) {
          DsChildRec& cr = ch_rec[q];
          const DsFrontDesc& ch = fr[cr.sn];
          cr.soff = ch.soff; cr.bp = ch.bp; cr.b = ch.b; cr.pmap_off = ch.pmap_off; cr.yoff = ch.yoff;
          if (q - cptr[p] < 4) { fr[p].cpm[q - cptr[p]] = ch.pmap_off; fr[p].cy[q - cptr[p]] = ch.yoff; }
          const int* cv = &vtx[ch.vtx_off + ch.nv_own];
          int* pm = &pmap[ch.pmap_off];
          int prev = -1;
          for (int i = 0; i < ch.nv_bnd; i++) {
            const int l = lc[cv[i]];
            if (l < 0 || l <= prev) { bad = true; continue; }
            prev = l;
            pm[l] = 3 * i; pm[l + 1] = 3 * i + 1; pm[l + 2] = 3 * i + 2;
            if (l >= f.pp) cr.nb += 3;
          }
          fr[cr.sn].lead = ch.b - cr.nb;
        }
        for (int i = 0; i < f.nv_own + f.nv_bnd; i++) lc[fv[i]] = -1;
      }
      if (bad) return -1;
      for (int s = 0; s < S; s++) if (fr[s].parent < 0 && fr[s].nv_bnd > 0) return -1;
    }
    lap(1);
    {
      std::vector<std::vector<int>> by_level(sym.n_levels);
      for (int s = 0; s < S; s++) by_level[sym.level[s]].push_back(s);
      build_levels(by_level);
    }
    const int L = sym.n_levels;
    const std::vector<int>& alap = sym.level;
    lap(2);
    const int NV = sym.NV;
    if ((int)tpos.size() != row_ptr[NV]) {
      tpos.assign(row_ptr[NV], -1);
      for (int r = 0; r < NV; r++)
        for (int k = 0; k < (int)adj[r].size(); k++) {
          const int c = adj[r][k];
          const auto& rc = adj[c];
          const auto it = std::lower_bound(rc.begin(), rc.end(), r);
          if (it != rc.end() && *it == r) tpos[row_ptr[r] + k] = row_ptr[c] + (int)(it - rc.begin());
        }
    }
    blk_dst.resize(row_ptr[NV]); blk_ld.resize(row_ptr[NV]);
    {
      const int nt = n_threads();
      if ((int)locs.size() < nt) locs.resize(nt);
      if ((int)lists.size() < 2 * nt * L) lists.resize((size_t)2 * nt * L);
      for (auto& v : lists) v.clear();
      std::atomic<int> bad{0};
      std::atomic<long long> written{0};
      ds_parallel_for(S, nt, 16, [&](int t, int s) {
        std::vector<int>& loc = locs[t];
        if ((int)loc.size() != NV) loc.assign(NV, -1);
        std::vector<int>& mine11 = lists[2 * ((size_t)t * L + alap[s])];
        std::vector<int>& mine = lists[2 * ((size_t)t * L + alap[s]) + 1];
        const DsFrontDesc& f = fr[s];
        const int no = f.nv_own;
        long long nw = 0;
        const int* fv = &vtx[f.vtx_off];
        for (int i = 0; i < no; i++) loc[fv[i]] = 3 * i;
        for (int i = 0; i < f.nv_bnd; i++) loc[fv[no + i]] = f.pp + 3 * i;
        for (int i = 0; i < no; i++) {
          const int r = fv[i];
          const auto& row = adj[r];
          for (int k = 0; k < (int)row.size(); k++) {
            const int c = row[k];
            if (sym.sn_of[c] < s) continue;
            const int lc = loc[c];
            if (lc < 0) { bad = 1; continue; }
            const int q = row_ptr[r] + k;
            blk_dst[q] = f.off + (long long)(3 * i) * f.ld + lc; blk_ld[q] = f.ld; nw++; (lc < f.pp ? mine11 : mine).push_back(q);
            if (sym.sn_of[c] > s) {
              const int qt = tpos[q];
              if (qt >= 0) { blk_dst[qt] = f.off21 + (long long)(lc - f.pp) * f.pp + 3 * i; blk_ld[qt] = f.pp; nw++; mine.push_back(qt); }
            }
          }
        }
        for (int i = 0; i < no + f.nv_bnd; i++) loc[fv[i]] = -1;
        written += nw;
      });
      if (bad || written != row_ptr[NV]) return -2;
      blk_q.resize(row_ptr[NV]); blk_lptr.assign(L + 1, 0); blk_lmid.assign(L, 0);
      size_t o = 0;
      for (int l = 0; l < L; l++) {
        for (int part = 0; part < 2; part++) {
          for (int t = 0; t < nt; t++) { const std::vector<int>& v = lists[2 * ((size_t)t * L + l) + part]; std::copy(v.begin(), v.end(), blk_q.begin() + o); o += v.size(); }
          if (part == 0) blk_lmid[l] = (int)o;
        }
        blk_lptr[l + 1] = (int)o;
      }
    }
    arena_leaf = 0;
    for (int q = level_ptr[0]; q < level_ptr[1]; q++) { const DsFrontDesc& f = fr[level_sn[q]]; arena_leaf = std::max(arena_leaf, f.off21 + (long long)f.bp * f.pp); }
    level_maxld.assign(L, 0);
    for (int l = 0; l < L; l++) for (int q = level_ptr[l]; q < level_ptr[l + 1]; q++) level_maxld[l] = std::max(level_maxld[l], fr[level_sn[q]].ld);
    lap(3);
    const int rc = build_con(cons, n_cons);
    lap(4);
    return rc;
  }

  int build_con(const int* cons, int n_cons) {
    con_dst.assign((size_t)n_cons * 16, -1); con_ld.assign((size_t)n_cons * 16, 0); con_lvl.assign((size_t)n_cons * 16, 0);
    for (int e = 0; e < n_cons; e++)
      for (int a = 0; a < 4; a++)
        for (int b = 0; b < 4; b++) {
          const int va = cons[4 * e + a], vb = cons[4 * e + b];
          const int s = std::min(sym.sn_of[va], sym.sn_of[vb]);
          const int lr = local_dof(s, va), lc = local_dof(s, vb);
          if (lr < 0 || lc < 0) return -3;
          int ldq = 0;
          const long long dst = panel_addr(fr[s], lr, lc, &ldq);
          if (dst < 0) return -3;
          con_dst[(size_t)e * 16 + a * 4 + b] = dst;
          con_ld[(size_t)e * 16 + a * 4 + b] = ldq;
          con_lvl[(size_t)e * 16 + a * 4 + b] = 2 * sym.level[s] + ((lr < fr[s].pp && lc < fr[s].pp) ? 0 : 1);
        }
    {
      const size_t n = (size_t)n_cons * 16;
      std::vector<int> ord(n);
      for (size_t i = 0; i < n; i++) ord[i] = (int)i;
      std::sort(ord.begin(), ord.end(), [&](int x, int y) {
        if (con_lvl[x] != con_lvl[y]) return con_lvl[x] < con_lvl[y];
        if (con_dst[x] != con_dst[y]) return con_dst[x] < con_dst[y];
        return x < y;
      });
      cgr_lptr.assign(n_levels + 1, 0); cgr_lmid.assign(n_levels, 0); cgr_ptr.clear(); cgr_ent.assign(ord.begin(), ord.end()); cgr_ld.clear(); cgr_dst.clear();
      for (size_t i = 0; i < n; i++) {
        const int x = ord[i];
        if (i == 0 || con_dst[x] != con_dst[ord[i - 1]] || con_lvl[x] != con_lvl[ord[i - 1]]) {
          cgr_ptr.push_back((int)i); cgr_dst.push_back(con_dst[x]); cgr_ld.push_back(con_ld[x]);
          cgr_lptr[(con_lvl[x] >> 1) + 1]++;
          if ((con_lvl[x] & 1) == 0) cgr_lmid[con_lvl[x] >> 1]++;
        }
      }
      cgr_ptr.push_back((int)n);
      for (int l = 0; l < n_levels; l++) { cgr_lmid[l] += cgr_lptr[l]; cgr_lptr[l + 1] += cgr_lptr[l]; }
    }
    return 0;
  }
};
```

thinshelllab_amd/csrc/k_direct.hpp:

```cpp
#pragma once
#include "direct_plan.hpp"
#include "tsl_device.hpp"

typedef double ds_d4 __attribute__((ext_vector_type(4)));

struct DsDev {
  const DsFrontDesc* fr;
  const DsFrontDesc* frl;
  const int* level_sn;
  double* A;
  double* S;
  double* G;
  double* scr;
  double* Y;
  const DsChildRec* ch;
  const int* pmap;
  const int* vtx;
  int* bad;
  double piv_tol;
  int dbg;
  unsigned long long* tlog;
};

__global__ void k_ds_rownorm(int NV, const int* __restrict__ slice_off, const int* __restrict__ slice_len, const double* __restrict__ vals, double* out) {
// ... 867 lines not shown
  }
}

#define DS_SK 32
#define DS_GMC 8
template <int mode, int WPC>
TSL_DEV void ds_gemm_tile(const DsDev& D, int lv0, int bx, int by, int bz, int part = 0) {
  constexpr int SA = DS_SK + 1, SB = 64 + 1;
  __shared__ double As[64 * SA];
  __shared__ double Bs[DS_SK * SB];
  const DsFrontDesc f = D.frl[lv0 + bz];
  const int Mr = mode == 0 ? f.pp : f.bp, Nc = f.bp, K = f.pp;
  const int I0 = by * 64, J0 = bx * 64;
  if (I0 >= Mr || J0 >= Nc) return;
  if (mode == 1 && part != 0 && ((I0 < f.lead && J0 < f.lead) != (part == 1))) return;
  if (mode == 0 && part != 0 && ((J0 < f.lead) != (part == 1))) return;
  const double* F = D.A + f.off;
  double* G = D.G + f.goff;
  const int ld = f.ld, pp = f.pp;
  const double* Am = mode == 0 ? F : D.A + f.off21;
  const int lda = mode == 0 ? ld : pp;
  const double* Bm = mode == 0 ? F + pp : G;
  const int ldb = mode == 0 ? ld : f.bp;
  const int lane = threadIdx.x & 63, w = threadIdx.x >> 6;
  const int wi = w >> 1, wj = w & 1;
  const int lr = lane & 15, lk = lane >> 4;
  const bool rows_hi = I0 + 32 < Mr, cols_hi = J0 + 32 < Nc;
  ds_d4 acc[2][2];
#pragma unroll
  for (int a = 0; a < 2; a++)
#pragma unroll
    for (int b = 0; b < 2; b++) acc[a][b] = ds_d4{0.0, 0.0, 0.0, 0.0};
  const int tx = threadIdx.x & 31, ty = threadIdx.x >> 5;
  double pa[8], pb0[4], pb1[4];
  auto gload = [&](int k0) {
#pragma unroll
    for (int q = 0; q < 8; q++) {
      const int r = ty + 8 * q;
      pa[q] = (r < 32 || rows_hi) ? Am[(size_t)(I0 + r) * lda + k0 + tx] : 0.0;
    }
#pragma unroll
    for (int q = 0; q < 4; q++) {
      const int r = ty + 8 * q;
      pb0[q] = Bm[(size_t)(k0 + r) * ldb + J0 + tx];
      pb1[q] = cols_hi ? Bm[(size_t)(k0 + r) * ldb + J0 + 32 + tx] : 0.0;
    }
  };
  gload(0);
  constexpr int GMC = DS_GMC;
  __shared__ int s_map[mode == 1 ? GMC : 1][128];
  __shared__ long long s_soff[mode == 1 ? GMC : 1];
  __shared__ int s_cbp[mode == 1 ? GMC : 1];
  int pre[GMC / 2];
  auto map_load = [&](int q) {
    const int k = threadIdx.x & 127;
    const int idx = k < 64 ? I0 + k : J0 + k - 64;
    return idx < f.bp ? D.pmap[D.ch[f.ch_off + q].pmap_off + pp + idx] : -1;
  };
  if (mode == 1) {
#pragma unroll
    for (int h = 0; h < GMC / 2; h++) { const int q = 2 * h + (threadIdx.x >> 7); pre[h] = q < f.nchild ? map_load(q) : -1; }
  }
  for (int k0 = 0; k0 < K; k0 += DS_SK) {
#pragma unroll
    for (int q = 0; q < 8; q++) As[(ty + 8 * q) * SA + tx] = pa[q];
#pragma unroll
    for (int q = 0; q < 4; q++) { Bs[(ty + 8 * q) * SB + tx] = pb0[q]; Bs[(ty + 8 * q) * SB + tx + 32] = pb1[q]; }
    __syncthreads();
    if (k0 + DS_SK < K) gload(k0 + DS_SK);
#pragma unroll
    for (int kk = 0; kk < DS_SK / 4; kk++) {
      const double a0 = As[(32 * wi + lr) * SA + 4 * kk + lk], a1 = As[(32 * wi + 16 + lr) * SA + 4 * kk + lk];
      const double b0 = Bs[(4 * kk + lk) * SB + 32 * wj + lr], b1 = Bs[(4 * kk + lk) * SB + 32 * wj + 16 + lr];
      acc[0][0] = __builtin_amdgcn_mfma_f64_16x16x4f64(a0, b0, acc[0][0], 0, 0, 0);
      acc[0][1] = __builtin_amdgcn_mfma_f64_16x16x4f64(a0, b1, acc[0][1], 0, 0, 0);
      acc[1][0] = __builtin_amdgcn_mfma_f64_16x16x4f64(a1, b0, acc[1][0], 0, 0, 0);
      acc[1][1] = __builtin_amdgcn_mfma_f64_16x16x4f64(a1, b1, acc[1][1], 0, 0, 0);
    }
    __syncthreads();
  }
  if (mode == 0) {
#pragma unroll
    for (int a = 0; a < 2; a++)
#pragma unroll
      for (int b = 0; b < 2; b++)
#pragma unroll
        for (int r = 0; r < 4; r++) {
          const int row = I0 + 32 * wi + 16 * a + lk + 4 * r, col = J0 + 32 * wj + 16 * b + lr;
          if (row < Mr && col < Nc) G[(size_t)row * f.bp + col] = acc[a][b][r];
        }
    return;
  }
  if (f.parent < 0) return;
  double s22[2][2][4];
#pragma unroll
  for (int a = 0; a < 2; a++)
#pragma unroll
    for (int b = 0; b < 2; b++)
#pragma unroll
      for (int r = 0; r < 4; r++) s22[a][b][r] = -acc[a][b][r];
  const int row0 = I0 + 32 * wi + lk, col0 = J0 + 32 * wj + lr;
  for (int q0 = 0; q0 < f.nchild; q0 += GMC) {
    const int nq = min(GMC, f.nchild - q0);
    if (q0 > 0) __syncthreads();
#pragma unroll
    for (int h = 0; h < GMC / 2; h++) {
      const int q = 2 * h + (threadIdx.x >> 7);
      if (q < nq) s_map[q][threadIdx.x & 127] = q0 == 0 ? pre[h] : map_load(q0 + q);
    }
    if ((int)threadIdx.x < nq) { const DsChildRec c = D.ch[f.ch_off + q0 + threadIdx.x]; s_soff[threadIdx.x] = c.soff; s_cbp[threadIdx.x] = c.bp; }
    __syncthreads();
    for (int q = 0; q < nq; q++) {
      const double* Sc = D.S + s_soff[q];
      const int cbp = s_cbp[q];
      const int cj0 = s_map[q][64 + 32 * wj + lr], cj1 = s_map[q][64 + 32 * wj + 16 + lr];
      const int dj0 = max(cj0, 0), dj1 = max(cj1, 0);
      int ci[2][4];
      double v0[2][4], v1[2][4];
#pragma unroll
      for (int a = 0; a < 2; a++)
#pragma unroll
        for (int r = 0; r < 4; r++) ci[a][r] = s_map[q][32 * wi + 16 * a + lk + 4 * r];
#pragma unroll
      for (int a = 0; a < 2; a++)
#pragma unroll
        for (int r = 0; r < 4; r++) {
          const double* Srow = Sc + (size_t)max(ci[a][r], 0) * cbp;
          v0[a][r] = Srow[dj0]; v1[a][r] = Srow[dj1];
        }
#pragma unroll
      for (int a = 0; a < 2; a++)
#pragma unroll
        for (int r = 0; r < 4; r++) {
          s22[a][0][r] = (ci[a][r] >= 0 && cj0 >= 0) ? s22[a][0][r] + v0[a][r] : s22[a][0][r];
          s22[a][1][r] = (ci[a][r] >= 0 && cj1 >= 0) ? s22[a][1][r] + v1[a][r] : s22[a][1][r];
        }
    }
  }
  double* Sf = D.S + f.soff;
#pragma unroll
  for (int a = 0; a < 2; a++)
#pragma unroll
    for (int r = 0; r < 4; r++) {
      const int row = row0 + 16 * a + 4 * r;
      if (row >= f.b) continue;
#pragma unroll
      for (int b = 0; b < 2; b++) {
        const int col = col0 + 16 * b;
        if (col < f.b) Sf[(size_t)row * f.bp + col] = s22[a][b][r];
      }
    }
}

#define DS_XU 4
#define DS_XSPAN 1024
#define DS_XMAXC 64
__global__ void __launch_bounds__(256) k_ds_extend_panels(DsDev D, int lv0, int nsp, int part, int xspan) {
  const DsFrontDesc f = D.frl[lv0 + blockIdx.y];
  const int ib = blockIdx.x / nsp, sp = blockIdx.x - ib * nsp;
  const int lane = threadIdx.x & 63, w = __builtin_amdgcn_readfirstlane(threadIdx.x >> 6);
  const int g = 4 * ib + w, ng = f.nv_own + f.nv_bnd;
  if (g >= ng + 2) return;
  const bool top = g >= ng ? g == ng : g < f.nv_own;
  if (!top && part == 1) return;
  const int ncol = top ? f.ld : f.pp;
  const int cA = (top && part == 2) ? f.pp : 0, cB = (top && part == 1) ? f.pp : ncol;
  const int c0 = cA + sp * xspan;
  if (c0 >= cB) return;
  const int c1 = min(cB, c0 + xspan);
  if (g >= ng) {
    const int nrow = top ? f.pp - f.p : f.bp - f.b;
    double* base = top ? D.A + f.off + (size_t)f.p * f.ld : D.A + f.off21 + (size_t)f.b * f.pp;
    for (int i = 0; i < nrow; i++)
      for (int j = c0 + lane; j < c1; j += 64) base[(size_t)i * ncol + j] = 0.0;
    return;
  }
  const int r = top ? 3 * g : f.pp + 3 * (g - f.nv_own);
  double* row = top ? D.A + f.off + (size_t)r * f.ld : D.A + f.off21 + (size_t)(r - f.pp) * f.pp;
  const DsChildRec* ch = D.ch + f.ch_off;
  if (f.nchild <= DS_XMAXC) {
    int my_ci = -1, my_off = 0, my_bp = 0;
    long long my_soff = 0;
    if (lane < f.nchild) { const DsChildRec c = ch[lane]; my_off = c.pmap_off; my_bp = c.bp; my_soff = c.soff; my_ci = D.pmap[c.pmap_off + r]; }
    const unsigned long long mask = __ballot(my_ci >= 0);
    for (int j0 = c0; j0 < c1; j0 += 64 * DS_XU) {
      double v[3][DS_XU];
#pragma unroll
      for (int k = 0; k < 3; k++)
#pragma unroll
        for (int u = 0; u < DS_XU; u++) v[k][u] = 0.0;
      auto child = [&](int q, int& ci, const int*& pm, const double*& S0, int& cbp) {
        ci = __builtin_amdgcn_readlane(my_ci, q);
        const int off = __builtin_amdgcn_readlane(my_off, q);
        cbp = __builtin_amdgcn_readlane(my_bp, q);
        const long long so = ((long long)__builtin_amdgcn_readlane((int)(my_soff >> 32), q) << 32) | (unsigned)__builtin_amdgcn_readlane((int)my_soff, q);
        pm = D.pmap + off;
        S0 = D.S + so + (size_t)ci * cbp;
      };
      unsigned long long m = mask;
      while (m != 0) {
        const int q0 = __builtin_ctzll(m);
        m &= m - 1;
        const bool two = m != 0;
        const int q1 = two ? __builtin_ctzll(m) : q0;
        if (two) m &= m - 1;
        int ci0, ci1, cbp0, cbp1;
        const int *pm0, *pm1;
        const double *Sa, *Sb;
        child(q0, ci0, pm0, Sa, cbp0);
        child(q1, ci1, pm1, Sb, cbp1);
        int cja[DS_XU], cjb[DS_XU];
#pragma unroll
        for (int u = 0; u < DS_XU; u++) { const int j = j0 + 64 * u + lane; cja[u] = j < c1 ? pm0[j] : -1; cjb[u] = (two && j < c1) ? pm1[j] : -1; }
        double sa[3][DS_XU], sb[3][DS_XU];
#pragma unroll
        for (int u = 0; u < DS_XU; u++) {
#pragma unroll
          for (int k = 0; k < 3; k++) { sa[k][u] = cja[u] >= 0 ? Sa[(size_t)k * cbp0 + cja[u]] : 0.0; sb[k][u] = cjb[u] >= 0 ? Sb[(size_t)k * cbp1 + cjb[u]] : 0.0; }
        }
#pragma unroll
        for (int u = 0; u < DS_XU; u++) {
          if (cja[u] >= 0) {
#pragma unroll
            for (int k = 0; k < 3; k++) v[k][u] += sa[k][u];
          }
          if (cjb[u] >= 0) {
#pragma unroll
            for (int k = 0; k < 3; k++) v[k][u] += sb[k][u];
          }
        }
      }
#pragma unroll
      for (int u = 0; u < DS_XU; u++) {
        const int j = j0 + 64 * u + lane;
        if (j < c1) {
#pragma unroll
          for (int k = 0; k < 3; k++) row[(size_t)k * ncol + j] = v[k][u];
        }
      }
    }
    return;
  }
  for (int j = c0 + lane; j < c1; j += 64) {
    double v[3] = {0.0, 0.0, 0.0};
    for (int q = 0; q < f.nchild; q++) {
      const int* pm = D.pmap + ch[q].pmap_off;
      const int ci = pm[r], cj = pm[j];
      if (ci >= 0 && cj >= 0) {
#pragma unroll
        for (int k = 0; k < 3; k++) v[k] += D.S[ch[q].soff + (size_t)(ci + k) * ch[q].bp + cj];
      }
    }
#pragma unroll
    for (int k = 0; k < 3; k++) row[(size_t)k * ncol + j] = v[k];
  }
}

__global__ void __launch_bounds__(256) k_ds_gemm_g32(DsDev D, int lv0, int part) {
  constexpr int SA = DS_SK + 1, SB = 32 + 1;
  __shared__ double As[32 * SA];
  __shared__ double Bs[DS_SK * SB];
  const DsFrontDesc f = D.frl[lv0 + blockIdx.z];
  const int Mr = f.pp, Nc = f.bp, K = f.pp;
  const int I0 = blockIdx.y * 32, J0 = blockIdx.x * 32;
  if (I0 >= Mr || J0 >= Nc) return;
  if (part != 0 && ((J0 < ((f.lead + 63) & ~63)) != (part == 1))) return;
  const double* F = D.A + f.off;
  double* G = D.G + f.goff;
  const int ld = f.ld;
  const double* Am = F;
  const double* Bm = F + f.pp;
  const int lane = threadIdx.x & 63, w = threadIdx.x >> 6, wi = w >> 1, wj = w & 1, lr = lane & 15, lk = lane >> 4;
  const int tx = threadIdx.x & 31, ty = threadIdx.x >> 5;
  ds_d4 acc = {0.0, 0.0, 0.0, 0.0};
  double pa[4], pb[4];
  auto gload = [&](int k0) {
#pragma unroll
    for (int q = 0; q < 4; q++) {
      const int r = ty + 8 * q;
      pa[q] = Am[(size_t)(I0 + r) * ld + k0 + tx];
      pb[q] = Bm[(size_t)(k0 + r) * ld + J0 + tx];
    }
  };
  gload(0);
  for (int k0 = 0; k0 < K; k0 += DS_SK) {
#pragma unroll
    for (int q = 0; q < 4; q++) { As[(ty + 8 * q) * SA + tx] = pa[q]; Bs[(ty + 8 * q) * SB + tx] = pb[q]; }
    __syncthreads();
    if (k0 + DS_SK < K) gload(k0 + DS_SK);
#pragma unroll
    for (int kk = 0; kk < DS_SK / 4; kk++)
      acc = __builtin_amdgcn_mfma_f64_16x16x4f64(As[(16 * wi + lr) * SA + 4 * kk + lk], Bs[(4 * kk + lk) * SB + 16 * wj + lr], acc, 0, 0, 0);
    __syncthreads();
  }
#pragma unroll
  for (int r = 0; r < 4; r++) G[(size_t)(I0 + 16 * wi + lk + 4 * r) * f.bp + J0 + 16 * wj + lr] = acc[r];
}

template <int mode, int WPC>
__global__ void __launch_bounds__(256, WPC) k_ds_gemm(DsDev D, int lv0, int part) {
  ds_gemm_tile<mode, WPC>(D, lv0, blockIdx.x, blockIdx.y, blockIdx.z, part);
}

template <int mode, int WPC>
__global__ void __launch_bounds__(256, WPC) k_ds_gemm_x(DsDev D, int lv0, int gx, int gy, int nf) {
  const unsigned L = blockIdx.x, xcd = L & 7, k = L >> 3;
  const unsigned tpf = (unsigned)gx * gy;
  const unsigned bz = (k / tpf) * 8 + xcd, t = k % tpf;
  if (bz >= (unsigned)nf) return;
  ds_gemm_tile<mode, WPC>(D, lv0, t % gx, t / gx, bz);
}

#define DS_VCHUNK 2048
TSL_DEV double ds_child_sum(const DsDev& D, const DsFrontDesc& f, int d) {
  int ci[4];
#pragma unroll
  for (int q = 0; q < 4; q++) ci[q] = q < f.nchild ? D.pmap[f.cpm[q] + d] : -1;
  double y[4];
#pragma unroll
  for (int q = 0; q < 4; q++) y[q] = ci[q] >= 0 ? D.Y[f.cy[q] + ci[q]] : 0.0;
  double a = ((y[0] + y[1]) + y[2]) + y[3];
  for (int q = 4; q < f.nchild; q++) {
    const DsChildRec c = D.ch[f.ch_off + q];
    const int cq = D.pmap[c.pmap_off + d];
    if (cq >= 0) a += D.Y[c.yoff + cq];
  }
  return a;
}
TSL_DEV void ds_gemv_stage(const DsDev& D, const DsFrontDesc& f, int mode, const int* vt, int in_v0, const double* vin, int c0, int cn, double* xs) {
  __syncthreads();
  for (int j = threadIdx.x; j < cn; j += 256) {
    const int jj = c0 + j;
    const double sub = (mode == 0 && f.nchild > 0) ? ds_child_sum(D, f, jj) : 0.0;
    xs[j] = vin[3 * (size_t)vt[in_v0 + jj / 3] + jj % 3] - sub;
  }
  __syncthreads();
}
__global__ void __launch_bounds__(256) k_ds_gemv(DsDev D, const int* __restrict__ wl_front, const int* __restrict__ wl_row, int wl0, int mode, const double* vin, double* vout) {
  __shared__ double xs[DS_VCHUNK];
  const DsFrontDesc f = D.fr[wl_front[wl0 + blockIdx.x]];
  const int r0 = wl_row[wl0 + blockIdx.x];
  const int nrows = mode == 1 ? f.b : f.p, ncols = mode == 2 ? f.b : f.p;
  const int* vt = D.vtx + f.vtx_off;
  const int in_v0 = mode == 2 ? f.nv_own : 0;
  const double* M = mode == 2 ? D.G + f.goff : D.A + (mode == 1 ? f.off21 : f.off);
  const int rs = mode == 2 ? f.bp : (mode == 1 ? f.pp : f.ld);
  const int lane = threadIdx.x & 63, w = threadIdx.x >> 6;
  double acc[4] = {0.0, 0.0, 0.0, 0.0};
  const int ib = r0 + 4 * w;
  const double* row0 = M + (size_t)min(ib, nrows - 1) * rs;
  const double* row1 = M + (size_t)min(ib + 1, nrows - 1) * rs;
  const double* row2 = M + (size_t)min(ib + 2, nrows - 1) * rs;
  const double* row3 = M + (size_t)min(ib + 3, nrows - 1) * rs;
  for (int c0 = 0; c0 < ncols; c0 += DS_VCHUNK) {
    const int cn = min(DS_VCHUNK, ncols - c0);
    ds_gemv_stage(D, f, mode, vt, in_v0, vin, c0, cn, xs);
#pragma unroll 4
    for (int j = lane; j < cn; j += 64) {
      const double xv = xs[j];
      acc[0] += row0[c0 + j] * xv; acc[1] += row1[c0 + j] * xv; acc[2] += row2[c0 + j] * xv; acc[3] += row3[c0 + j] * xv;
    }
  }
#pragma unroll
  for (int q = 0; q < 4; q++) {
    const int i = r0 + 4 * w + q;
    const double a = wave_sum(acc[q]);
    if (lane == 0 && i < nrows) {
      if (mode == 1) D.Y[f.yoff + i] = (f.nchild > 0 ? ds_child_sum(D, f, f.pp + i) : 0.0) + a;
      else {
        const size_t o = 3 * (size_t)vt[i / 3] + i % 3;
        vout[o] = mode == 0 ? a : vout[o] - a;
      }
    }
  }
}

__global__ void __launch_bounds__(256) k_ds_gemv_wide(DsDev D, const int* __restrict__ wl_front, const int* __restrict__ wl_row, int wl0, int mode, const double* vin, double* vout) {
  __shared__ double xs[DS_VCHUNK];
  __shared__ double part[4][4];
  const int e = wl0 + (blockIdx.x >> 2);
  const DsFrontDesc f = D.fr[wl_front[e]];
  const int nrows = mode == 1 ? f.b : f.p, ncols = mode == 2 ? f.b : f.p;
  const int r0 = wl_row[e] + 4 * (blockIdx.x & 3);
  if (r0 >= nrows) return;
  const int* vt = D.vtx + f.vtx_off;
  const int in_v0 = mode == 2 ? f.nv_own : 0;
  const double* M = mode == 2 ? D.G + f.goff : D.A + (mode == 1 ? f.off21 : f.off);
  const int rs = mode == 2 ? f.bp : (mode == 1 ? f.pp : f.ld);
  const int lane = threadIdx.x & 63, w = threadIdx.x >> 6;
  double acc[4] = {0.0, 0.0, 0.0, 0.0};
  const double* row0 = M + (size_t)min(r0, nrows - 1) * rs;
  const double* row1 = M + (size_t)min(r0 + 1, nrows - 1) * rs;
  const double* row2 = M + (size_t)min(r0 + 2, nrows - 1) * rs;
  const double* row3 = M + (size_t)min(r0 + 3, nrows - 1) * rs;
  for (int c0 = 0; c0 < ncols; c0 += DS_VCHUNK) {
    const int cn = min(DS_VCHUNK, ncols - c0);
    ds_gemv_stage(D, f, mode, vt, in_v0, vin, c0, cn, xs);
#pragma unroll 4
    for (int j = threadIdx.x; j < cn; j += 256) {
      const double xv = xs[j];
      acc[0] += row0[c0 + j] * xv; acc[1] += row1[c0 + j] * xv; acc[2] += row2[c0 + j] * xv; acc[3] += row3[c0 + j] * xv;
    }
  }
#pragma unroll
  for (int q = 0; q < 4; q++) { const double a = wave_sum(acc[q]); if (lane == 0) part[w][q] = a; }
  __syncthreads();
  if (threadIdx.x < 4) {
// ... 12 lines not shown
```

thinshelllab_amd/csrc/tsl_ctx.hpp:

```cpp
#pragma once
#include <memory>
#include <hip/hip_runtime.h>
#include <stdint.h>

#include <algorithm>
#include <cmath>
#include <cstdio>
#include <cstring>
#include <string>
#include <vector>

#include "../../include/tsl_hip.h"
#include "k_body.hpp"
#include "direct_plan.hpp"

#define TSL_SLICE 64

extern thread_local std::string g_tsl_err;
int tsl_fail(const char* fmt, ...);

#define HIP_OK(call)                                                                     \
  do {                                                                                   \
    hipError_t e__ = (call);                                                             \
    if (e__ != hipSuccess) return tsl_fail("%s failed: %s (%s:%d)", #call, hipGetErrorString(e__), __FILE__, __LINE__); \
  } while (0)

template <class T>
struct DevBuf {
  T* p = nullptr;
  size_t n = 0;
  bool owned = true;
  int alloc(size_t count) {
    if (!owned) return tsl_fail("internal: allocation of %zu B requested for a buffer that is a view into a scene group's memory", count * sizeof(T));
    release();
    n = count;
    if (count == 0) return 0;
    hipError_t e = hipMalloc((void**)&p, count * sizeof(T));
    if (e != hipSuccess) { p = nullptr; return tsl_fail("hipMalloc(%zu B) failed: %s", count * sizeof(T), hipGetErrorString(e)); }
    return 0;
  }
  int upload(const std::vector<T>& h) {
    if (alloc(h.size())) return -1;
    if (h.empty()) return 0;
    hipError_t e = hipMemcpy(p, h.data(), h.size() * sizeof(T), hipMemcpyHostToDevice);
    if (e != hipSuccess) return tsl_fail("hipMemcpy H2D failed: %s", hipGetErrorString(e));
    return 0;
  }
  int zero(hipStream_t s = 0) {
    if (!n) return 0;
    hipError_t e = hipMemsetAsync(p, 0, n * sizeof(T), s);
    if (e != hipSuccess) return tsl_fail("hipMemset failed: %s", hipGetErrorString(e));
    return 0;
  }
  void release() { if (p && owned) (void)hipFree(p); p = nullptr; n = 0; owned = true; }
  void view(T* q, size_t count) { release(); p = q; n = count; owned = false; }
  void swap(DevBuf& o) { std::swap(p, o.p); std::swap(n, o.n); std::swap(owned, o.owned); }
  DevBuf() = default;
  DevBuf(const DevBuf&) = delete;
  DevBuf& operator=(const DevBuf&) = delete;
  ~DevBuf() { release(); }
};

struct ClothDev {
  int face_start, NF, v_offset, NV;
  double dx, mass, Kl, Ka, Kb, k_angle;
};
struct ElasticDev {
  int kind, cell_start, n_cells, v_offset, n_verts;
  double mu, lam, alpha;
};

struct SolverScalars {
  double raw[32];
};

struct MgLevel {
  int N = 0, M = 0, n = 0;
  DevBuf<double> A, Dinv, x, x2, r, t;
  DevBuf<float> A32, S32;
  DevBuf<double> S;
  DevBuf<double> omega;
  DevBuf<float> Cinv;
  DevBuf<int> cbad;
  DevBuf<double> gjD, gjR, gjC, gjP;
  int gj_ld = 0;
};
struct MgCloth {
  int v_offset = 0, N0 = 0, M0 = 0;
  std::vector<MgLevel*> lv;
  int dense_lv = -1;
  ~MgCloth() { for (auto* l : lv) delete l; }
};

#define DS_NSIDE 2
struct DsPlanSlot {
  DirectPlan plan;
  std::vector<int> h_cons, h_cset;
  uint64_t key = 0;
  long stamp = 0;
  bool used = false;
  DevBuf<int> level_sn, pmap, vtx, blk_ld, wl_front, wl_row, blk_q, cgr_ptr, cgr_ent, cgr_ld;
  DevBuf<long long> blk_dst, cgr_dst;
  DevBuf<DsFrontDesc> fr, frl;
  DevBuf<DsChildRec> ch_rec;
};
struct DirectSolver {
  char* pin = nullptr; size_t pin_cap = 0, pin_off = 0;
  int enable = -1;
  bool hard = false;
  int hard_steps = 0, probe_cap = 60, probe_every = 16;
  hipStream_t zstream = 0;
  hipEvent_t ev_zfork = nullptr, ev_zero = nullptr;
  bool prezero_pending = false;
  size_t prezero_n = 0;
  int prezero = 1;
  hipStream_t fstream[2] = {nullptr, nullptr};
  hipEvent_t ev_ffork = nullptr, ev_fjoin[2] = {nullptr, nullptr};
  hipEvent_t ev_la[5] = {nullptr, nullptr, nullptr, nullptr, nullptr};
  hipStream_t lastream = nullptr;
  int eager_n = 0; const double* eager_r = nullptr; double* eager_z = nullptr;
  int lookahead = 103;
  int device = 0;
  int flow_wgs_last = 0;
  int flow = 3, flow_cap = 0, flow_epoch = 0;
  int flow_token = 0, flow_token_fd = -1;
  long flow_token_asked = 0;
  int small_rounds = 2;
  int xcd_map = 64;
  long n_flow = 0, n_flow_abort = 0;
  DevBuf<double> flow_x;
  DevBuf<int> flow_f;
  DevBuf<unsigned long long> tlog;
  int gemv_wide_below = 300;
  int g32_below = 1100;
  bool cons_checked = false;
  double* h_anorm = nullptr;
  int bench_batch = -1;
  double piv_tol = 1e-11;
  int fallback_cap = 1000;
  int leaf = 64;
  bool static_ready = false, numeric_valid = false;
  bool have_factor = false;
  int dbg = 0;
  double berr_tol = 1e-12, berr_rel_cap = 50.0;
  long berr_seen = 0, berr_accepted = 0;
  double berr_max = 0, berr_rel_max = 0;
  int n_setup_fail = 0;
  std::vector<std::unique_ptr<DsPlanSlot>> cache;
  int cache_cap = 64, cache_mb = 1024;
  long cache_clock = 0, n_plan_hits = 0, n_plan_evicted = 0;
  DirectPlan plan;
  std::vector<DsGrid> grids;
  std::vector<DsBlock> blocks;
  std::vector<int> row_ptr;
  std::vector<int> h_c2s;
  std::vector<int> h_cons;
  std::vector<int> h_cset;
  bool plan_valid = false;
  DevBuf<int> level_sn, pmap, vtx, blk_ld, bad, wl_front, wl_row, blk_q, cgr_ptr, cgr_ent, cgr_ld;
  DevBuf<long long> blk_dst, cgr_dst;
  DevBuf<DsFrontDesc> fr, frl;
  DevBuf<DsChildRec> ch_rec;
  DevBuf<double> arena, sarena, garena, scr, w;
  long n_plans = 0, n_factor = 0, n_apply = 0, n_perturbed = 0;
  long plan_gen = 0;
  bool keep_host_maps = false;
  bool merged = false;
  DirectSolver* token_lender = nullptr;
  double t_plan = 0;
  double anorm = 0;
  bool anorm_valid = false;
  int anorm_age = 0;
  int anorm_spd = -1;
  DevBuf<double> anorm_dev;
  hipEvent_t ev0 = nullptr, ev1 = nullptr;
};

struct tsl_group;
struct tsl_ctx {
  tsl_group* group = nullptr;
  hipStream_t stream = 0;
  hipStream_t user_stream = 0;
  hipEvent_t ev_in = nullptr, ev_out = nullptr;
  int depth = 0;
  hipGraphExec_t pcg_graph = nullptr;
  long pcg_graph_key = -1;
  hipGraphExec_t mr_graph = nullptr;
  long mr_graph_key = -1;
  int use_graph = 1;
  int NV = 0, NF = 0;
  double dt = 5e-3, k_contact = 1000, eps_contact = 1e-3, eps_v = 0.01, damping = 1.0, mu_cloth_elastic = 1.0, mu_cloth_cloth = 1.0;
  int max_n_constraints = 10000;
  int newton_cap = 1000, plastic = 0, contact_enable = 1;
  int spd_literal = 0;
  double cg_tol = 1e-10;
  int cg_maxit = 200000, cg_check = 32;
  double grid_h = 0.003;
  double grid_extent = 0.2;

  std::vector<ClothDev> h_cloth;
  DevBuf<ClothDev> d_cloth;
  int n_cface = 0, n_hinge = 0;
  DevBuf<int> cf_f2v, cf_cf, cf_cp, cf_cloth;
  DevBuf<double> cf_V, cf_li;
  DevBuf<int> cf_blk;
  DevBuf<int> cf_order;
  DevBuf<int> hg_info;
  DevBuf<int> hg_v;
  DevBuf<int> hg_blk;
  DevBuf<double> norm_dir;
  DevBuf<double> quirk;
  std::vector<int> h_cf_f2v, h_cf_cf, h_cf_cp;
  std::vector<double> h_stvk;
  DevBuf<double> d_stvk, cf_dminv;
  int n_stvk = 0;

  std::vector<ElasticDev> h_el;
  DevBuf<ElasticDev> d_el;
  int n_tet = 0;
  DevBuf<int> tet_v, tet_el, tet_blk;
  DevBuf<double> tet_B, tet_W;

  DevBuf<double> mass, grav, fext;
  DevBuf<int> frozen;
  DevBuf<int> diag_blk;
  std::vector<int> h_frozen;
  std::vector<double> h_mass;

  int n_slices = 0;
  long n_slots = 0;
  std::vector<int> h_rowpos, h_perm, h_slice_off, h_slice_len, h_colidx;
  std::vector<std::vector<int>> h_rows;
  DevBuf<int> rowpos, perm, slice_off, slice_len, colidx, diag_perm;
  DevBuf<double> vals, vals_full;
  DevBuf<float> vals32;
  bool vals32_valid = false;
  int mg_f32 = 1;
  DevBuf<double> Dinv;
  DevBuf<unsigned char> fzmask;
  DevBuf<double> mdt2;
  long nnzb = 0;

  DevBuf<double> v_x, v_r, v_z, v_p, v_Ap, v_b, v_t0, v_t1, v_t2, v_t3, v_t4, v_mg;
  BodyDenseArgs bd_args{};
  int bd_rows_n = 0, bd_n3max = 0, bd_wg = 0, bd_scr_n = 0, bd_enable = -1;
  size_t bd_w_total = 0;
  bool bd_valid = false;
  DevBuf<int> bd_rows, bd_body_of, bd_local_of, bd_bad;
  DevBuf<double> bd_W, bd_scr;
  DevBuf<double> bd_rb;
  int pcg_body_fold = 1;
  int mg_st_f32 = 1;
  int mg_chunk = 0;
  double mr_eta = 0.3;
  int mg_fr_rows = 32;
  DevBuf<float> bd_Binv;
  DevBuf<double> gm_V, gm_h;
  DevBuf<double> gm_Z;
  DevBuf<unsigned> cg_ent;
  DevBuf<int> cg_base, cg_ptr;
  DevBuf<double> cg_hrec, cg_frec;
  DevBuf<int> trans;
  DevBuf<int> vg_ptr, vg_idx;
  DevBuf<double> vg_stage, cg_trec;
  int vg_ns = 0, vg_hinge0 = 0, vg_tet0 = 0;
  DevBuf<double> vg_stage2;
  DevBuf<double> dot_part; DevBuf<int> dot_ticket;
  DevBuf<double> e_part;
  int n_cgblk = 0, n_cgblk_cloth = 0;
  DevBuf<double> tet_V;
  long tet_V_count = 0;
  int tet_warm = 1;
  DevBuf<double> ir_part;
  DevBuf<int> ir_ticket;
  double* h_ir = nullptr;
  double last_xmax = 0;
  bool last_xmax_valid = false;
  int gmres_m = 300, use_gmres = 1, use_minres = 1, verbose = 0;
  double adj_clamp = 1000.0;
  int adj_clamp_angleref = 1;
  DevBuf<double> dmu_accum;
  DevBuf<double> pg_part, pg_out;
  DevBuf<double> vals_pc, c_H_pc;
  bool pc_separate = false, pc_frozen = false, in_step = false;
  bool cdiag_valid = false;
  bool dinv_valid = false;
  const double *st_pos = nullptr, *st_prev = nullptr, *st_vel = nullptr, *st_ref = nullptr;
  int fwd_spd_pc = 1;
  int adj_spd_pc = 1;
  DevBuf<SolverScalars> scal;
  DevBuf<double> part_pAp, part_rz, part_rr;
  SolverScalars* h_scal = nullptr;
  SolverScalars* h_scal2 = nullptr;
  hipEvent_t rb_event[2] = {nullptr, nullptr};
  hipStream_t side = 0;
  hipEvent_t ev_fork = nullptr, ev_fork0 = nullptr, ev_g2 = nullptr, ev_join = nullptr, ev_join2 = nullptr, ev_hh = nullptr, ev_gf = nullptr;
  hipStream_t side2 = 0;

  DevBuf<double> F, pdir, x1;

  int n_body = 0, n_pair = 0;
  std::vector<tsl_body> h_bodies;
  std::vector<tsl_contact_pair> h_pairs;
  std::vector<int> self_contact;
  DevBuf<int> faces;
  DevBuf<int> border;
  DevBuf<double> vn;
  DevBuf<int> proj_flag, proj_dir, proj_idx;
  DevBuf<double> proj_w;
  DevBuf<int> nc_dev;
  int nc = 0;
  DevBuf<int> c_idx;
  DevBuf<double> c_w, c_n, c_dx0, c_k, c_mu, c_T;
// ... 72 lines not shown
```

thinshelllab_amd/csrc/tsl_hip.hip:

```cpp
#include <stdarg.h>
#include <cctype>
#include <chrono>
#include <mutex>

#include <array>
#include <map>

#include "k_cloth.hpp"
#include "k_contact.hpp"
#include "k_fem.hpp"
#include "k_mg.hpp"
#include "k_param.hpp"
#include "k_solver.hpp"
#include "tsl_ctx.hpp"

thread_local std::string g_tsl_err;
int tsl_fail(const char* fmt, ...) {
  char buf[1024];
  va_list ap;
  va_start(ap, fmt);
  vsnprintf(buf, sizeof(buf), fmt, ap);
  va_end(ap);
  g_tsl_err = buf;
  return -1;
// ... 305 lines not shown
  UP(mass, c->h_mass); UP(grav, grav); UP(fext, fext);
  c->h_frozen.assign(d->frozen_host, d->frozen_host + 3 * (size_t)NV);
  if (upload_frozen(c)) { delete c; return -1; }
#undef UP
  int rc = 0;
  rc |= c->norm_dir.alloc((size_t)std::max(c->n_cface, 1) * 3);
  rc |= c->quirk.alloc((size_t)std::max(d->n_cloth, 1) * 90);
  rc |= c->dot_part.alloc(64 * 512); rc |= c->dot_ticket.alloc(512);
  if (!rc) (void)hipMemset(c->dot_ticket.p, 0, 512 * sizeof(int));
  rc |= c->vals.alloc((size_t)P.n_slots * 9); rc |= c->vals_full.alloc((size_t)P.n_slots * 9);
  rc |= c->Dinv.alloc((size_t)NV * 9);
  const size_t n3 = (size_t)NV * 3;
  rc |= c->v_x.alloc(n3); rc |= c->v_r.alloc(n3); rc |= c->v_z.alloc(n3); rc |= c->v_p.alloc(n3); rc |= c->v_Ap.alloc(n3); rc |= c->v_b.alloc(n3);
  rc |= c->v_t0.alloc(n3); rc |= c->v_t1.alloc(n3); rc |= c->v_t2.alloc(n3); rc |= c->v_t3.alloc(n3); rc |= c->v_t4.alloc(n3); rc |= c->v_mg.alloc(n3);
  rc |= c->F.alloc(n3); rc |= c->pdir.alloc(n3); rc |= c->x1.alloc(n3);
  rc |= c->scal.alloc(1);
  rc |= c->part_pAp.alloc((size_t)P.n_slices + (size_t)(c->max_n_constraints + 63) / 64 + 8); rc |= c->part_rz.alloc((size_t)NV / 256 + 8 + 1024); rc |= c->part_rr.alloc((size_t)NV / 256 + 8 + 1024);
  if (rc) { delete c; return -1; }
  if (hipHostMalloc((void**)&c->h_scal, sizeof(SolverScalars) > sizeof(CgScal) ? sizeof(SolverScalars) : sizeof(CgScal)) != hipSuccess) { delete c; return tsl_fail("hipHostMalloc failed"); }
  if (hipHostMalloc((void**)&c->h_scal2, 2 * sizeof(SolverScalars)) != hipSuccess) { delete c; return tsl_fail("hipHostMalloc failed"); }
  for (int i = 0; i < 2; i++)
    if (hipEventCreateWithFlags(&c->rb_event[i], hipEventDisableTiming) != hipSuccess) { delete c; return tsl_fail("hipEventCreate failed"); }
  if (hipStreamCreateWithFlags(&c->side, hipStreamNonBlocking) != hipSuccess || hipStreamCreateWithFlags(&c->side2, hipStreamNonBlocking) != hipSuccess ||
      hipEventCreateWithFlags(&c->ev_join2, hipEventDisableTiming) != hipSuccess || hipEventCreateWithFlags(&c->ev_fork, hipEventDisableTiming) != hipSuccess || hipEventCreateWithFlags(&c->ev_fork0, hipEventDisableTiming) != hipSuccess || hipEventCreateWithFlags(&c->ev_g2, hipEventDisableTiming) != hipSuccess || hipEventCreateWithFlags(&c->ev_hh, hipEventDisableTiming) != hipSuccess || hipEventCreateWithFlags(&c->ev_gf, hipEventDisableTiming) != hipSuccess ||
      hipEventCreateWithFlags(&c->ev_join, hipEventDisableTiming) != hipSuccess) { delete c; return tsl_fail("side stream / event creation failed"); }
  c->vals.zero(); c->vals_full.zero(); c->scal.zero(); c->part_rz.zero(); c->part_rr.zero();

  c->n_body = d->n_body; c->n_pair = d->n_pair;
  if (d->n_body > 0) c->h_bodies.assign(d->bodies, d->bodies + d->n_body);
  if (d->n_pair > 0) c->h_pairs.assign(d->pairs, d->pairs + d->n_pair);
  if (contact_alloc(c, d)) { delete c; return -1; }
  if (mg_build(c, d)) { delete c; return -1; }
  if (body_dense_setup(c)) { delete c; return -1; }
  (void)hipDeviceSynchronize();
  (void)hipGetDevice(&c->ds.device);
  *out = c;
  return 0;
}

static void group_unregister_and_destroy(tsl_group* G);
extern "C" void tsl_ctx_destroy(tsl_ctx* c) {
  if (!c) return;
  if (c->group) group_unregister_and_destroy(c->group);
  (void)hipDeviceSynchronize();
  ds_flow_token_release(c->ds);
  if (c->h_scal) (void)hipHostFree(c->h_scal);
  if (c->h_scal2) (void)hipHostFree(c->h_scal2);
  for (int i = 0; i < 2; i++) if (c->rb_event[i]) (void)hipEventDestroy(c->rb_event[i]);
  if (c->pcg_graph) (void)hipGraphExecDestroy(c->pcg_graph);
  if (c->mr_graph) (void)hipGraphExecDestroy(c->mr_graph);
  if (c->ev_in) (void)hipEventDestroy(c->ev_in);
  if (c->ev_out) (void)hipEventDestroy(c->ev_out);
  for (int k = 0; k < DS_NSIDE; k++) if (c->ds.fstream[k]) { (void)hipStreamSynchronize(c->ds.fstream[k]); (void)hipEventDestroy(c->ds.ev_fjoin[k]); (void)hipStreamDestroy(c->ds.fstream[k]); }
  if (c->ds.ev_ffork) (void)hipEventDestroy(c->ds.ev_ffork);
  for (int k = 0; k < 5; k++) if (c->ds.ev_la[k]) (void)hipEventDestroy(c->ds.ev_la[k]);
  if (c->ds.lastream) { (void)hipStreamSynchronize(c->ds.lastream); (void)hipStreamDestroy(c->ds.lastream); }
  if (c->ds.h_anorm) (void)hipHostFree(c->ds.h_anorm);
  if (c->ds.pin) (void)hipHostFree(c->ds.pin);
  if (c->h_ir) (void)hipHostFree(c->h_ir);
  if (c->ds.zstream) { (void)hipStreamSynchronize(c->ds.zstream); (void)hipEventDestroy(c->ds.ev_zfork); (void)hipEventDestroy(c->ds.ev_zero); (void)hipStreamDestroy(c->ds.zstream); }
  if (c->ev_fork) (void)hipEventDestroy(c->ev_fork);
  if (c->ev_fork0) (void)hipEventDestroy(c->ev_fork0);
  if (c->ev_g2) (void)hipEventDestroy(c->ev_g2);
  if (c->ev_hh) (void)hipEventDestroy(c->ev_hh);
  if (c->ev_gf) (void)hipEventDestroy(c->ev_gf);
  if (c->ev_join) (void)hipEventDestroy(c->ev_join);
  if (c->side) (void)hipStreamDestroy(c->side);
  if (c->ev_join2) (void)hipEventDestroy(c->ev_join2);
  if (c->side2) (void)hipStreamDestroy(c->side2);
  if (c->stream) (void)hipStreamDestroy(c->stream);
  for (auto& e : c->ev_pool) { (void)hipEventDestroy(e.first); (void)hipEventDestroy(e.second); }
  delete c;
}

extern "C" int tsl_set_stream(tsl_ctx* c, void* s) { c->user_stream = (hipStream_t)s; return 0; }

static int stvk_prepare(tsl_ctx* c) {
  if (c->cf_dminv.n > 0 || c->n_cface == 0) return 0;
  std::vector<double> li(3 * (size_t)c->n_cface), dm(4 * (size_t)c->n_cface);
  HIP_OK(hipMemcpy(li.data(), c->cf_li.p, li.size() * sizeof(double), hipMemcpyDeviceToHost));
  std::vector<int> cid(c->n_cface);
  HIP_OK(hipMemcpy(cid.data(), c->cf_cloth.p, cid.size() * sizeof(int), hipMemcpyDeviceToHost));
  for (int f = 0; f < c->n_cface; f++) {
    const double l0 = li[3 * f], l1 = li[3 * f + 1], l2 = li[3 * f + 2];
    if (!(l0 > 0 && l1 > 0 && l2 > 0 && l0 < l1 + l2 && l1 < l2 + l0 && l2 < l0 + l1))
      return tsl_fail("tsl_set_param: StVK membrane: rest lengths (%g, %g, %g) of face %d (cloth %d, face %d of the cloth) violate the triangle inequality", l0, l1, l2, f,
                      cid[f], f - c->h_cloth[cid[f]].face_start);
    const double a = (l0 * l0 + l2 * l2 - l1 * l1) / (2.0 * l0), b = sqrt(l2 * l2 - a * a);
    dm[4 * f] = 1.0 / l0; dm[4 * f + 1] = -a / (l0 * b); dm[4 * f + 2] = 0.0; dm[4 * f + 3] = 1.0 / b;
  }
  return c->cf_dminv.upload(dm);
}

static int stvk_set(tsl_ctx* c, const char* key, long idx, const std::string& f, double v) {
  const int n_cloth = (int)c->h_cloth.size();
  if (f == "membrane") {
    if (v != 0.0 && v != 1.0) return tsl_fail("tsl_set_param: %s must be 0 or 1 (got %g)", key, v);
    if (v == 1.0) TSL_TRY(stvk_prepare(c));
  }
  if (c->h_stvk.empty()) {
    c->h_stvk.assign(4 * (size_t)n_cloth, 0.0);
    TSL_TRY(c->d_stvk.alloc(c->h_stvk.size()));
  }
  c->h_stvk[4 * idx + (f == "membrane" ? 0 : (f == "stvk_mu" ? 1 : 2))] = v;
  c->n_stvk = 0;
  for (int i = 0; i < n_cloth; i++) c->n_stvk += c->h_stvk[4 * i] != 0.0;
  HIP_OK(hipMemcpy(c->d_stvk.p, c->h_stvk.data(), c->h_stvk.size() * sizeof(double), hipMemcpyHostToDevice));
  return 0;
}

extern "C" int tsl_set_param(tsl_ctx* c, const char* key, double v) {
  Scope scope(c);
  (void)hipStreamSynchronize(c->stream);
  c->mg_omega_valid = false; c->mg_cinv_valid = false;
  c->ds.anorm_valid = false;
  std::string k(key);
  if (k == "mu_cloth_elastic") c->mu_cloth_elastic = v;
  else if (k == "mu_cloth_cloth") c->mu_cloth_cloth = v;
  else if (k == "k_contact") c->k_contact = v;
  else if (k == "eps_contact") c->eps_contact = v;
  else if (k == "eps_v") c->eps_v = v;
  else if (k == "damping") c->damping = v;
  else if (k == "cg_tol") c->cg_tol = v;
  else if (k == "cg_maxit") c->cg_maxit = (int)v;
  else if (k == "newton_cap") c->newton_cap = (int)v;
  else if (k == "plastic") c->plastic = (int)v;
  else if (k == "spd_literal") {
    if (v != 0.0 && v != 1.0) return tsl_fail("tsl_set_param: spd_literal must be 0 or 1 (got %g)", v);
    c->spd_literal = (int)v;
  }
  else if (k == "contact") c->contact_enable = (v != 0.0);
  else if (k == "contact_ee") {
    if (v != 0.0 && v != 1.0) return tsl_fail("tsl_set_param: contact_ee must be 0 or 1 (got %g)", v);
    c->contact_ee = (int)v;
    if (c->contact_ee) TSL_TRY(ee_prepare(c));
  }
  else if (k == "grid_h") c->grid_h = v;
  else if (k == "grid_extent") c->grid_extent = v;
  else if (k == "adj_spd_pc") c->adj_spd_pc = (int)v;
  else if (k == "adj_clamp") c->adj_clamp = v;
  else if (k == "adj_clamp_angleref") c->adj_clamp_angleref = (int)v;
  else if (k == "verbose") c->verbose = (int)v;
  else if (k == "direct") { c->ds.enable = (int)v; c->ds.numeric_valid = false; c->ds.hard = false; }
  else if (k == "direct_berr") c->ds.berr_tol = v;
  else if (k == "direct_small_rounds") { c->ds.small_rounds = std::max(1, (int)v); c->ds.plan_valid = false; c->ds.numeric_valid = false; c->ds.cache.clear(); }
  else if (k == "tet_warm") c->tet_warm = (int)v;
  else if (k == "ds_dbg") c->ds.dbg = (int)v;
  else if (k == "ds_bench_batch") c->ds.bench_batch = (int)v;
  else if (k == "direct_flow") c->ds.flow = std::max(0, (int)v);
  else if (k == "direct_flow_token") { if (v == 0) ds_flow_token_release(c->ds); }
  else if (k == "direct_gemv_wide_below") c->ds.gemv_wide_below = std::max(0, (int)v);
  else if (k == "direct_g32_below") c->ds.g32_below = std::max(0, (int)v);
  else if (k == "direct_lookahead") c->ds.lookahead = (int)v;
  else if (k == "direct_piv_tol") { c->ds.piv_tol = v; c->ds.numeric_valid = false; }
  else if (k == "direct_leaf") { c->ds.leaf = std::max(4, (int)v); c->ds.static_ready = false; c->ds.plan_valid = false; c->ds.numeric_valid = false; }
  else if (k == "gmres_m") c->gmres_m = (int)v;
  else if (k == "body_inv") { c->bd_enable = (int)v; c->bd_valid = false; }
  else if (k == "mg") c->mg_enable = (int)v;
  else if (k.rfind("self_contact", 0) == 0 && k.size() > 12) {
    char* endp = nullptr;
    const long b = strtol(k.c_str() + 12, &endp, 10);
    if (*endp != 0 || b < 0 || b >= c->n_body) return tsl_fail("tsl_set_param: bad body index in %s", key);
    if ((long)c->self_contact.size() < c->n_body) c->self_contact.assign(c->n_body, 0);
    c->self_contact[b] = (v != 0.0);
  }
  else if (k == "mg_coarse_exact") c->mg_coarse_exact = (int)v;
  else if (k == "mg_dense_nodes") { c->mg_dense_auto = v < 0; if (v >= 0) c->mg_dense_nodes = (int)v; c->mg_ops_valid = false; }
  else if ((k.rfind("cloth", 0) == 0 || k.rfind("elastic", 0) == 0) && k.find('.') != std::string::npos) {
    const bool is_cloth = k[0] == 'c';
    const size_t p0 = is_cloth ? 5 : 7, dot = k.find('.');
    char* endp = nullptr;
    const long idx = strtol(k.c_str() + p0, &endp, 10);
    if (endp != k.c_str() + dot || dot == p0) return tsl_fail("tsl_set_param: bad index in %s", key);
    const std::string f = k.substr(dot + 1);
    if (is_cloth) {
      if (idx < 0 || idx >= (long)c->h_cloth.size()) return tsl_fail("tsl_set_param: bad cloth index in %s", key);
      ClothDev& cd = c->h_cloth[idx];
      if (f == "membrane" || f == "stvk_mu" || f == "stvk_lam") return stvk_set(c, key, idx, f, v);
      if (f == "Kb") cd.Kb = v; else if (f == "Kl") cd.Kl = v; else if (f == "Ka") cd.Ka = v; else if (f == "k_angle") cd.k_angle = v;
      else return tsl_fail("tsl_set_param: unknown key %s", key);
      HIP_OK(hipMemcpy(c->d_cloth.p, c->h_cloth.data(), c->h_cloth.size() * sizeof(ClothDev), hipMemcpyHostToDevice));
    } else {
      if (idx < 0 || idx >= (long)c->h_el.size()) return tsl_fail("tsl_set_param: bad elastic index in %s", key);
      ElasticDev& ed = c->h_el[idx];
      if (f == "mu") ed.mu = v; else if (f == "lam") ed.lam = v; else if (f == "alpha") ed.alpha = v;
      else return tsl_fail("tsl_set_param: unknown key %s", key);
      HIP_OK(hipMemcpy(c->d_el.p, c->h_el.data(), c->h_el.size() * sizeof(ElasticDev), hipMemcpyHostToDevice));
      c->bd_valid = false;
    }
  } else return tsl_fail("tsl_set_param: unknown key %s", key);
  return 0;
}

extern "C" int tsl_set_frozen(tsl_ctx* c, const int32_t* fr) {
  Scope scope(c);
  (void)hipStreamSynchronize(c->stream);
  c->h_frozen.assign(fr, fr + 3 * (size_t)c->NV);
  c->mg_omega_valid = false; c->mg_cinv_valid = false;
  TSL_TRY(upload_frozen(c));
  if (c->pcg_graph) { (void)hipGraphExecDestroy(c->pcg_graph); c->pcg_graph = nullptr; }
  if (c->mr_graph) { (void)hipGraphExecDestroy(c->mr_graph); c->mr_graph = nullptr; }
  return body_dense_setup(c);
}
extern "C" int tsl_set_ext_force(tsl_ctx* c, const double* f) {
  Scope scope(c);
  (void)hipStreamSynchronize(c->stream);
  HIP_OK(hipMemcpy(c->fext.p, f, 3 * (size_t)c->NV * sizeof(double), hipMemcpyHostToDevice));
  return 0;
}
extern "C" int tsl_set_gravity(tsl_ctx* c, const double* g) {
  Scope scope(c);
  (void)hipStreamSynchronize(c->stream);
  HIP_OK(hipMemcpy(c->grav.p, g, 3 * (size_t)c->NV * sizeof(double), hipMemcpyHostToDevice));
  return 0;
}

template <bool STVK>
TSL_DEV void energy_body(VertArgs VA, ClothArgs CA, TetArgs TA, const double* __restrict__ pos, const double* __restrict__ prev,
                         const double* __restrict__ vel, const double* __restrict__ ref_angle, double* __restrict__ e_part, StvkArgs S) {
  const int t = blockIdx.x * blockDim.x + threadIdx.x;
  double e = 0;
  if (t < VA.NV) e += vert_energy(VA, t, pos, prev, vel);
  if (t < CA.n_cface) {
    int v[3]; d3 P[3];
    load_face(pos, CA.f2v, t, v, P);
    const double li[3] = {CA.li[3 * t], CA.li[3 * t + 1], CA.li[3 * t + 2]};
    if constexpr (STVK) e += cface_energy_sel(CA.cloth[CA.cid[t]], S.stvk + 4 * CA.cid[t], S.dminv + 4 * t, P, CA.V[t], li);
    else e += cface_energy(CA.cloth[CA.cid[t]], P, CA.V[t], li);
  }
  if (t < CA.n_hinge) e += hinge_energy(CA, t, pos, ref_angle);
  if (t < TA.n_tet) e += tet_energy(TA, t, pos);
  e = wave_sum(e);
  __shared__ double sw[4];
  if ((threadIdx.x & 63) == 0) sw[threadIdx.x >> 6] = e;
  __syncthreads();
  if (threadIdx.x == 0) e_part[blockIdx.x] = ((sw[0] + sw[1]) + sw[2]) + sw[3];
}
__global__ void k_energy(VertArgs VA, ClothArgs CA, TetArgs TA, const double* __restrict__ pos, const double* __restrict__ prev,
                         const double* __restrict__ vel, const double* __restrict__ ref_angle, double* __restrict__ e_part) {
  energy_body<false>(VA, CA, TA, pos, prev, vel, ref_angle, e_part, StvkArgs{nullptr, nullptr});
}
__global__ void k_energy_stvk(VertArgs VA, ClothArgs CA, TetArgs TA, const double* __restrict__ pos, const double* __restrict__ prev,
                              const double* __restrict__ vel, const double* __restrict__ ref_angle, double* __restrict__ e_part, StvkArgs S) {
  energy_body<true>(VA, CA, TA, pos, prev, vel, ref_angle, e_part, S);
}
__global__ void __launch_bounds__(256) k_energy_final(int n, const double* __restrict__ part, double* __restrict__ e_out) {
  __shared__ double sh[256];
  double a = 0.0;
  for (int i = threadIdx.x; i < n; i += 256) a += part[i];
  sh[threadIdx.x] = a;
  __syncthreads();
  for (int o = 128; o > 0; o >>= 1) { if ((int)threadIdx.x < o) sh[threadIdx.x] += sh[threadIdx.x + o]; __syncthreads(); }
  if (threadIdx.x == 0) *e_out = sh[0];
}

static CgScal* SC(tsl_ctx* c) { return (CgScal*)c->scal.p; }
static CgScal* HSC(tsl_ctx* c) { return (CgScal*)c->h_scal; }

static int energy_async(tsl_ctx* c, const double* pos, const double* prev, const double* vel, const double* ref) {
  hipStream_t s = c->stream;
  if (c->n_cface) hipLaunchKernelGGL(k_cloth_normals, dim3(nblk(c->n_cface, 256)), dim3(256), 0, s, c->n_cface, pos, c->cf_f2v.p, c->norm_dir.p);
  const int nmax = std::max(std::max(c->NV, c->n_cface), std::max(c->n_hinge, c->n_tet));
  const int nvf = c->nc - c->nc_ee;
  const int nb1 = nblk(nmax, 256), nb2 = nvf > 0 ? nblk(nvf, 64) : 0, nb3 = c->nc_ee > 0 ? nblk(c->nc_ee, 64) : 0;
  if (c->e_part.n < (size_t)nb1 + (size_t)nblk(c->max_n_constraints, 64) + 1) { if (c->e_part.alloc((size_t)nb1 + (size_t)nblk(c->max_n_constraints, 64) + 1)) return -1; }
  if (c->n_stvk > 0) hipLaunchKernelGGL(k_energy_stvk, dim3(nb1), dim3(256), 0, s, vert_args(c), cloth_args(c), tet_args(c), pos, prev, vel, ref, c->e_part.p, stvk_args(c));
  else hipLaunchKernelGGL(k_energy, dim3(nb1), dim3(256), 0, s, vert_args(c), cloth_args(c), tet_args(c), pos, prev, vel, ref, c->e_part.p);
  if (nb2 > 0) hipLaunchKernelGGL(k_contact_energy, dim3(nb2), dim3(64), 0, s, nvf, contact_args(c), pos, c->e_part.p + nb1);
  if (nb3 > 0) hipLaunchKernelGGL(k_ee_energy, dim3(nb3), dim3(64), 0, s, c->nc_ee, ee_args(contact_args(c), nvf), pos, c->e_part.p + nb1 + nb2);
  hipLaunchKernelGGL(k_energy_final, dim3(1), dim3(256), 0, s, nb1 + nb2 + nb3, (const double*)c->e_part.p, &SC(c)->energy);
  return 0;
}
static int energy_sync(tsl_ctx* c, const double* pos, const double* prev, const double* vel, const double* ref, double* E) {
  TSL_TRY(energy_async(c, pos, prev, vel, ref));
  HIP_OK(hipMemcpyAsync(&HSC(c)->energy, &SC(c)->energy, sizeof(double), hipMemcpyDeviceToHost, c->stream));
  HIP_OK(hipStreamSynchronize(c->stream));
  *E = HSC(c)->energy;
  return 0;
}

extern "C" int tsl_energy(tsl_ctx* c, const double* pos, const double* prev, const double* vel, const double* ref, double* E) {
  Scope scope(c);
  return energy_sync(c, pos, prev, vel, ref, E);
}

__global__ void k_vertex_gather(int NV, const int* __restrict__ vg_ptr, const int* __restrict__ vg_idx, const double* __restrict__ stage, int lo, int hi, double* __restrict__ F) {
  const int v = blockIdx.x * blockDim.x + threadIdx.x;
  if (v >= NV) return;
  d3 a = ld3(F, v);
  for (int e = vg_ptr[v]; e < vg_ptr[v + 1]; e++) { const int i = vg_idx[e]; if (i >= lo && i < hi) a = a + ld3(stage, i); }
  st3(F, v, a);
}
__global__ void __launch_bounds__(256) k_contact_row_gather(int NV, const int* __restrict__ rowpos, const int* __restrict__ cr_ptr, const int* __restrict__ cr_ent,
                                                            const double* __restrict__ cg, double* __restrict__ F) {
  const int v = (int)((blockIdx.x * (size_t)blockDim.x + threadIdx.x) >> 6), lane = threadIdx.x & 63;
  if (v >= NV) return;
  const int p = rowpos[v];
  const int r0 = cr_ptr[p], r1 = cr_ptr[p + 1];
  if (r1 <= r0) return;
  double a0 = 0, a1 = 0, a2 = 0;
  for (int e = r0 + lane; e < r1; e += 64) {
    const int q = cr_ent[e];
    const double* g = cg + 12 * (size_t)(q >> 2) + 3 * (q & 3);
    a0 += g[0]; a1 += g[1]; a2 += g[2];
  }
  a0 = wave_sum(a0); a1 = wave_sum(a1); a2 = wave_sum(a2);
// ... 1588 lines not shown
  const std::function<int(int)> assemble_one = [&](int i) -> int {
    tsl_ctx* c = m[i].c;
    TSL_TRY(assemble(c, m[i].pos, m[i].prev, m[i].vel, m[i].ref, 1, c->F.p));
    hipLaunchKernelGGL(k_gather_perm, dim3(nblk(c->NV, 256)), dim3(256), 0, c->stream, c->NV, c->perm.p, (const double*)c->F.p, c->v_b.p);
    return 0;
  };
  std::vector<tsl_solve_stats> ss(n);
  lap(-1);
  for (;;) {
    std::vector<int> act;
    for (int i = 0; i < n; i++) if (active[i] && iter[i] < m[i].c->newton_cap) act.push_back(i);
    if (act.empty()) break;
    for (int i : act) if (++iter[i] == 1) TSL_TRY(energy_issue(i));
    for (int i : act) { if (iter[i] == 1) { HIP_OK(hipStreamSynchronize(m[i].c->stream)); E0[i] = HSC(m[i].c)->energy; } else E0[i] = E[i]; }
    lap(0);
    if (pool) TSL_TRY(pool->run(act, assemble_one));
    else for (int i : act) TSL_TRY(assemble_one(i));
    lap(1);
    TSL_TRY(solve(act, ss, lap));
    lap(5);
    for (int i : act) {
      tsl_ctx* c = m[i].c;
      const size_t n3 = 3 * (size_t)c->NV;
      hipStream_t s = c->stream;
      add_solve_stats(st[i], ss[i]);
      const bool have_pmax = ss[i].method == 4 && ss[i].flag == 0 && c->last_xmax_valid;
      if (have_pmax) HSC(c)->pmax = c->last_xmax;
      else {
        HIP_OK(hipMemsetAsync(&SC(c)->pmax, 0, sizeof(double), s));
        hipLaunchKernelGGL(k_absmax, dim3(gsz(n3)), dim3(256), 0, s, n3, c->pdir.p, &SC(c)->pmax);
        HIP_OK(hipMemcpyAsync(&HSC(c)->pmax, &SC(c)->pmax, sizeof(double), hipMemcpyDeviceToHost, s));
      }
      HIP_OK(hipMemcpyAsync(c->x1.p, m[i].pos, n3 * sizeof(double), hipMemcpyDeviceToDevice, s));
      alpha[i] = 1.0;
    }
    std::vector<int> pend = act;
    while (!pend.empty()) {
      for (int i : pend) {
        tsl_ctx* c = m[i].c;
        const size_t n3 = 3 * (size_t)c->NV;
        hipLaunchKernelGGL(k_linesearch, dim3(gsz(n3)), dim3(256), 0, c->stream, n3, c->x1.p, c->pdir.p, alpha[i], m[i].pos);
        TSL_TRY(energy_issue(i));
      }
      std::vector<int> again;
      for (int i : pend) {
        HIP_OK(hipStreamSynchronize(m[i].c->stream));
        E[i] = HSC(m[i].c)->energy;
        st[i].ls_evals++;
        if (E[i] < E0[i]) continue;
        alpha[i] /= 2;
        if (alpha[i] > 1e-8) again.push_back(i);
      }
      pend.swap(again);
    }
    for (int i : act) {
      tsl_ctx* c = m[i].c;
      delta[i] = HSC(c)->pmax / c->dt;
      st[i].last_alpha = alpha[i]; st[i].energy = E[i];
      if (c->verbose >= 4) fprintf(stderr, "[tsl]   scene %d newton %2d: E0 %.12e  E - E0 %+.3e  alpha %.3g  |p|max %.3e  delta %.3e  (solve: %d its, rel_residual %.1e)\n", i, iter[i], E0[i], E[i] - E0[i], alpha[i],
                                   HSC(c)->pmax, delta[i], ss[i].iters, ss[i].rel_residual);
      if (delta[i] < 1e-7) active[i] = 0;
    }
    lap(6);
  }
  if (timed) {
    long its = 0;
    double loops = 0;
    for (int i = 0; i < n; i++) { its += st[i].cg_iters; loops += m[i].c->tm_loop; }
    fprintf(stderr, "[tsl] step of %d scene(s): %d Newton iterations (most of a scene), %ld solver iterations; energy %.3f s, assembly + preconditioner set-up %.3f s, solves %.3f s "
            "(merged plans + merge %.3f s, factorisation %.3f s, application %.3f s; iteration loops %.3f s), line search %.3f s\n",
            n, *std::max_element(iter.begin(), iter.end()), its, tph[0], tph[1], tph[2] + tph[3] + tph[4] + tph[5], tph[2], tph[3], tph[4], loops, tph[6]);
  }
  for (int i = 0; i < n; i++) {
    tsl_ctx* c = m[i].c;
    const size_t n3 = 3 * (size_t)c->NV;
    st[i].newton_iters = iter[i]; st[i].last_delta = delta[i];
    st[i].factorizations = (int)(c->ds.n_factor - fact0[i]) + (g && i == 0 ? (int)(g->ds.n_factor - gfact0) : 0); st[i].plans = (int)(c->ds.n_plans - plans0[i]);
    hipLaunchKernelGGL(k_update_vel, dim3(gsz(n3)), dim3(256), 0, c->stream, n3, m[i].pos, m[i].prev, c->damping / c->dt, m[i].vel);
    if (c->plastic) TSL_TRY(tsl_update_ref_angle(c, m[i].pos, m[i].ref));
  }
  for (int i = 0; i < n; i++) {
    tsl_ctx* c = m[i].c;
    HIP_OK(hipStreamSynchronize(c->stream));
    if (st[i].solves > 0) c->last_step_iters_per_solve = (double)st[i].cg_iters / st[i].solves;
    if (stats) stats[i] = st[i];
  }
  if (g) HIP_OK(hipStreamSynchronize(g->stream));
  HIP_OK(hipGetLastError());
  return 0;
}

extern "C" int tsl_step(tsl_ctx* c, double* pos, double* prev, double* vel, double* ref, tsl_step_stats* stats) {
  Scope scope(c);
  const StepSolve solve = [c](const std::vector<int>&, std::vector<tsl_solve_stats>& ss, const std::function<void(int)>&) -> int {
    TSL_TRY(solve_perm(c, &ss[0]));
    hipLaunchKernelGGL(k_scatter_perm, dim3(nblk(c->NV, 256)), dim3(256), 0, c->stream, c->NV, c->perm.p, (const double*)c->v_x.p, c->pdir.p);
    HIP_OK(hipGetLastError());
    if (ss[0].method == 4) TSL_TRY(direct_prezero(c));
    return 0;
  };
  return newton_step({StepMember{c, pos, prev, vel, ref}}, nullptr, nullptr, solve, stats);
}

static std::mutex g_group_mu;
static std::vector<tsl_group*> g_groups;
static void group_unregister_and_destroy(tsl_group* G) {
  { std::lock_guard<std::mutex> lk(g_group_mu);
    auto it = std::find(g_groups.begin(), g_groups.end(), G);
    if (it == g_groups.end()) return;
    g_groups.erase(it); }
  group_destroy(G);
}
extern "C" int tsl_group_create(tsl_ctx* const* ctxs, int32_t n, tsl_group** out) {
  for (int i = 0; i < n; i++) if (!direct_enabled(ctxs[i])) return tsl_fail("tsl_group_create: scene %d does not use the sparse direct solve (\"direct\" = 1 or a cloth grid of >= 1024 cells)", i);
  TSL_TRY(group_create(ctxs, n, out));
  std::lock_guard<std::mutex> lk(g_group_mu);
  g_groups.push_back(*out);
  return 0;
}
extern "C" void tsl_group_destroy(tsl_group* G) { if (G) group_unregister_and_destroy(G); }
extern "C" int tsl_group_info(tsl_group* G, double* out9) {
  out9[0] = (double)G->n_merge; out9[1] = (double)G->n_relayout; out9[2] = G->t_merge; out9[3] = 8.0 * (double)(G->arena.n + G->sarena.n + G->garena.n + G->w.n);
  out9[4] = (double)G->g->ds.n_factor; out9[5] = (double)G->g->ds.n_apply; out9[6] = (double)G->n_own_path;
  out9[7] = (double)G->g->ds.n_flow; out9[8] = (double)G->g->ds.n_flow_abort;
  return 0;
}

static int group_solve(tsl_group* G, const std::vector<int>& act, std::vector<tsl_solve_stats>& ss, const std::function<void(int)>& lap) {
  const int n = (int)G->m.size();
  tsl_ctx* g = G->g;
  {
    std::vector<int> todo;
    for (int i = 0; i < n; i++) { tsl_ctx* c = G->m[i]; if (!(c->ds.plan_valid && c->ds.cons_checked)) todo.push_back(i); }
    if (todo.size() > 1) TSL_TRY(G->pool->run(todo, [&](int i) -> int { return direct_plan(G->m[i]); }));
    for (int i = 0; i < n; i++) TSL_TRY(direct_plan(G->m[i]));
  }
  bool stale = !G->merged_valid;
  for (int i = 0; i < n; i++) stale |= G->seen_gen[i] != G->m[i]->ds.plan_gen;
  if (stale) {
    for (int i = 0; i < n; i++) HIP_OK(hipStreamSynchronize(G->m[i]->stream));
    TSL_TRY(group_merge(G));
  }
  lap(2);
  {
    DirectSolver& gd = g->ds;
    const DirectSolver& d0 = G->m[0]->ds;
    for (int i = 1; i < n; i++) {
      const DirectSolver& di = G->m[i]->ds;
      if (di.piv_tol != d0.piv_tol || di.flow != d0.flow || di.g32_below != d0.g32_below || di.gemv_wide_below != d0.gemv_wide_below || di.small_rounds != d0.small_rounds)
        return tsl_fail("scene group: members 0 and %d differ in a parameter of the factorisation (direct_piv_tol / _flow / _g32_below / _gemv_wide_below / _small_rounds)", i);
    }
    if (gd.piv_tol != d0.piv_tol) gd.piv_tol = d0.piv_tol;
    gd.flow = G->flow_lost ? 0 : d0.flow; gd.g32_below = d0.g32_below; gd.gemv_wide_below = d0.gemv_wide_below; gd.small_rounds = d0.small_rounds * n; gd.xcd_map = d0.xcd_map;
    gd.prezero = d0.prezero; gd.dbg = d0.dbg;
  }
  ss.assign(n, tsl_solve_stats{});
  std::vector<char> okv(n, 1);
  for (int attempt = 0; attempt < 2; attempt++) {
    DirectSolver& gd = g->ds;
    for (int i = 0; i < n; i++) { HIP_OK(hipEventRecord(G->ev_m[i], G->m[i]->stream)); HIP_OK(hipStreamWaitEvent(g->stream, G->ev_m[i], 0)); }
    gd.numeric_valid = false;
    if (attempt > 0) {
      gd.have_factor = false;
      if (gd.prezero_pending) { HIP_OK(hipStreamWaitEvent(g->stream, gd.ev_zero, 0)); gd.prezero_pending = false; }
    }
    TSL_TRY(direct_factor(g));
    if (attempt == 0) for (int i = 0; i < n; i++) { DirectSolver& d = G->m[i]->ds; if (++d.anorm_age >= 64) d.anorm_valid = false; }
    lap(3);
    TSL_TRY(direct_apply(g, G->vb.p, G->vx.p));
    HIP_OK(hipEventRecord(G->ev_g, g->stream));
    lap(4);
    for (int i = 0; i < n; i++) HIP_OK(hipStreamWaitEvent(G->m[i]->stream, G->ev_g, 0));
    for (int i : act) TSL_TRY(ir_pass_enqueue(G->m[i]));
    bool any_bad = false;
    for (int i : act) {
      tsl_ctx* c = G->m[i];
      HIP_OK(hipStreamSynchronize(c->stream));
      ss[i] = tsl_solve_stats{};
      const int ok = ir_pass_verdict(c, &ss[i], true);
      if (ok < 0) return -1;
      okv[i] = (char)ok;
      any_bad |= !ok;
    }
    if (attempt == 0) {
      int note[8];
      const int lost = ds_flow_lost(g, any_bad, note);
      if (lost < 0) return -1;
      if (lost) {
        fprintf(stderr, "[tsl] scene group: k_ds_gj_flow of the merged factorisation waited in vain for a flag: \"direct_flow\" disabled for the group, refactorising "
                "(workgroup %d of %d gave up; flag value %d, epoch %d)\n", note[2], note[1], note[3], note[4]);
        gd.flow = 0; gd.n_flow_abort++; G->flow_lost = true;
        continue;
      }
    }
    break;
  }
  for (int i : act) {
    tsl_ctx* c = G->m[i];
    tsl_solve_stats& s1 = ss[i];
    if (okv[i]) { s1.flag = 0; s1.method = 4; continue; }
    c->ds.numeric_valid = true; c->ds.have_factor = true;
    const tsl_solve_stats first = s1;
    TSL_TRY(solve_perm(c, &s1, &first));
    G->n_own_path++;
    if (c->verbose >= 2) fprintf(stderr, "[tsl] scene group: member %d went on from the merged pass (rel_residual %.2e) on its own path: flag %d after %d applications\n", i, first.rel_residual, s1.flag, s1.iters);
  }
  for (int i = 0; i < n; i++) { tsl_ctx* c = G->m[i]; c->ds.numeric_valid = false; c->ds.have_factor = false; HIP_OK(hipEventRecord(G->ev_m[i], c->stream)); HIP_OK(hipStreamWaitEvent(g->stream, G->ev_m[i], 0)); }
  TSL_TRY(direct_prezero(g));
  lap(5);
  return 0;
}

extern "C" int tsl_group_step(tsl_group* G, double* const* pos_a, double* const* prev_a, double* const* vel_a, double* const* ref_a, tsl_step_stats* stats) {
  const int n = (int)G->m.size();
  std::vector<std::unique_ptr<Scope>> scopes;
  for (int i = 0; i < n; i++) scopes.emplace_back(new Scope(G->m[i]));
  std::vector<StepMember> m(n);
  for (int i = 0; i < n; i++) {
    if (!direct_enabled(G->m[i])) return tsl_fail("tsl_group_step: scene %d does not use the sparse direct solve", i);
    m[i] = StepMember{G->m[i], pos_a[i], prev_a[i], vel_a[i], ref_a[i]};
  }
  G->g->verbose = G->m[0]->verbose;
  const StepSolve solve = [G](const std::vector<int>& act, std::vector<tsl_solve_stats>& ss, const std::function<void(int)>& lap) -> int {
    TSL_TRY(group_solve(G, act, ss, lap));
    for (int i : act) {
      tsl_ctx* c = G->m[i];
      hipLaunchKernelGGL(k_scatter_perm, dim3(nblk(c->NV, 256)), dim3(256), 0, c->stream, c->NV, c->perm.p, (const double*)c->v_x.p, c->pdir.p);
    }
    return 0;
  };
  return newton_step(m, G->pool.get(), G->g, solve, stats);
}

extern "C" int tsl_matrix_nnzb(tsl_ctx* c, int32_t* nb, int32_t* nnzb) {
  *nb = c->NV; *nnzb = (int32_t)c->nnzb;
  return 0;
}

extern "C" int tsl_matrix_export(tsl_ctx* c, int32_t* row_ptr, int32_t* col, double* vals) {
  Scope scope(c);
  HIP_OK(hipStreamSynchronize(c->stream));
  std::vector<double> hv(c->vals.n);
  HIP_OK(hipMemcpy(hv.data(), c->vals.p, hv.size() * sizeof(double), hipMemcpyDeviceToHost));
  long k = 0;
  row_ptr[0] = 0;
  for (int v = 0; v < c->NV; v++) {
    const auto& r = c->h_rows[v];
    const int p = c->h_rowpos[v], s = p >> 6, lane = p & 63;
    for (size_t j = 0; j < r.size(); j++, k++) {
      col[k] = r[j];
      const size_t base = ((size_t)c->h_slice_off[s] + 64 * j) * 9 + lane;
      for (int e = 0; e < 9; e++) vals[9 * k + e] = hv[base + 64 * e];
    }
    row_ptr[v + 1] = (int32_t)k;
  }
  return 0;
}

extern "C" int tsl_matrix_import(tsl_ctx* c, const double* vals) {
  Scope scope(c);
  HIP_OK(hipStreamSynchronize(c->stream));
  std::vector<double> hv(c->vals.n);
  HIP_OK(hipMemcpy(hv.data(), c->vals.p, hv.size() * sizeof(double), hipMemcpyDeviceToHost));
  long k = 0;
  for (int v = 0; v < c->NV; v++) {
    const int p = c->h_rowpos[v], s = p >> 6, lane = p & 63;
    for (size_t j = 0; j < c->h_rows[v].size(); j++, k++) {
      const size_t base = ((size_t)c->h_slice_off[s] + 64 * j) * 9 + lane;
      for (int e = 0; e < 9; e++) hv[base + 64 * e] = vals[9 * k + e];
    }
  }
  HIP_OK(hipMemcpy(c->vals.p, hv.data(), hv.size() * sizeof(double), hipMemcpyHostToDevice));
  c->ds.numeric_valid = false; c->ds.anorm_valid = false;
  c->mg_ops_valid = false; c->pc_separate = false;
  c->bd_valid = false; c->mg_omega_valid = false; c->mg_cinv_valid = false;
  return 0;
}

extern "C" int tsl_profile_reset(tsl_ctx* c, int enable) {
  c->prof_enable = enable; c->prof_ms = 0; c->prof_chunks = 0; c->ev_sample_next = false; c->prof_launches = 0; c->prof_samples = 0; c->ev_used = 0; c->prof_dev_used = 0; c->prof_dev_ticks = 0; c->prof_dev_n = 0;
  if (enable) {
    c->prof_waves = (size_t)c->n_slices * PCG_WPS;
    c->prof_dev_cap = 1;
    if (c->prof_dev.n == 0) TSL_TRY(c->prof_dev.alloc(2 * c->prof_waves * (size_t)c->prof_dev_cap));
    HIP_OK(hipMemset(c->prof_dev.p, 0, c->prof_dev.n * sizeof(unsigned long long)));
  }
  if (enable && c->ev_pool.empty()) {
    for (int i = 0; i < 64; i++) {
      hipEvent_t a, b;
      HIP_OK(hipEventCreate(&a)); HIP_OK(hipEventCreate(&b));
      c->ev_pool.push_back({a, b});
    }
  }
  return 0;
}

extern "C" int tsl_profile_read(tsl_ctx* c, double* ms_per_launch, int64_t* launches, int64_t* bytes_per_launch) {
  Scope scope(c);
  HIP_OK(hipStreamSynchronize(c->stream));
  prof_collect(c);
  double dev_ms = 0;
  long n_dev = c->prof_dev_n;
  {
    int dev = 0, khz = 100000;
    (void)hipGetDevice(&dev);
    if (hipDeviceGetAttribute(&khz, hipDeviceAttributeWallClockRate, dev) != hipSuccess || khz <= 0) khz = 100000;
    dev_ms = c->prof_dev_ticks / (double)khz;
// ... 387 lines not shown
```

Before: 518,700.

## Fuse matrix-entry scatter and contact assembly into the front extend-add kernel

Builds per-vertex-row tables of sparse matrix entries and contact Hessian groups at plan time. The extend-panels kernel then adds these original entries directly into each front row while assembling child updates, and level-start skips the separate scatter launch. The intent is to remove one kernel launch and one pass over the front memory per level. In exchange it adds plan-build work, extra device tables, and a per-row serial loop over contact groups inside the extend kernel.

```diff
diff --git a/thinshelllab_amd/csrc/direct_group.hpp b/thinshelllab_amd/csrc/direct_group.hpp
--- a/thinshelllab_amd/csrc/direct_group.hpp
+++ b/thinshelllab_amd/csrc/direct_group.hpp
@@ -216,6 +216,7 @@
   for (int i = 0; i < n; i++) { const DirectPlan& P = G->m[i]->ds.plan; nbk += P.blk_q.size(); ngr += P.cgr_dst.size(); nge += P.cgr_ent.size(); }
   std::vector<int> src(nbk), ld(nbk), cg_ptr, cg_ent, cg_ld;
   std::vector<long long> dst(nbk), cg_dst;
+  std::vector<std::vector<int>> gmap(n);
   cg_ptr.reserve(ngr + 1); cg_ent.reserve(nge); cg_ld.reserve(ngr); cg_dst.reserve(ngr);
   M.blk_lptr.assign(L + 1, 0); M.cgr_lptr.assign(L + 1, 0);
   {
@@ -232,7 +233,9 @@
         if (c->nc > 0 && !P.cgr_lptr.empty()) {
           const long long oa = (long long)G->off_a[i];
           const int eo = 16 * G->nc_off[i];
+          if (gmap[i].empty()) gmap[i].assign(P.cgr_dst.size(), -1);
           for (int gq = P.cgr_lptr[l]; gq < P.cgr_lptr[l + 1]; gq++) {
+            gmap[i][gq] = (int)cg_dst.size();
             cg_ptr.push_back((int)cg_ent.size());
             for (int e = P.cgr_ptr[gq]; e < P.cgr_ptr[gq + 1]; e++) cg_ent.push_back(P.cgr_ent[e] + eo);
             cg_dst.push_back(P.cgr_dst[gq] + oa); cg_ld.push_back(P.cgr_ld[gq]);
@@ -258,12 +261,45 @@
   std::vector<DsFrontDesc> frl(M.level_sn.size());
   for (size_t i = 0; i < frl.size(); i++) frl[i] = M.fr[M.level_sn[i]];
   ds_pin_reset(gd, 16 * nbk + 2 * sizeof(DsFrontDesc) * M.fr.size() + sizeof(DsChildRec) * M.ch_rec.size() +
-                       4 * (M.level_sn.size() + M.pmap.size() + vtxp.size() + M.wl_front.size() + M.wl_row.size()) + 20 * (cg_ent.size() + cg_ptr.size()) + 64 * 256);
+                       4 * (M.level_sn.size() + M.pmap.size() + vtxp.size() + M.wl_front.size() + M.wl_row.size()) + 20 * (cg_ent.size() + cg_ptr.size()) + 64 * 256 + 8 * ((size_t)vtx_base[n] + 1) + 1024 + [&] { size_t b = 0; for (int i = 0; i < n; i++) b += 8 * (G->m[i]->ds.plan.xs_col.size() + G->m[i]->ds.plan.xc_col.size()); return b; }());
   TSL_TRY(ds_upload_grow(gd.fr, M.fr, s, &gd)); TSL_TRY(ds_upload_grow(gd.frl, frl, s, &gd)); TSL_TRY(ds_upload_grow(gd.level_sn, M.level_sn, s, &gd));
   TSL_TRY(ds_upload_grow(gd.pmap, M.pmap, s, &gd)); TSL_TRY(ds_upload_grow(gd.ch_rec, M.ch_rec, s, &gd)); TSL_TRY(ds_upload_grow(gd.vtx, vtxp, s, &gd));
   TSL_TRY(ds_upload_grow(gd.blk_q, src, s, &gd)); TSL_TRY(ds_upload_grow(gd.blk_dst, dst, s, &gd)); TSL_TRY(ds_upload_grow(gd.blk_ld, ld, s, &gd));
   TSL_TRY(ds_upload_grow(gd.cgr_ptr, cg_ptr, s, &gd)); TSL_TRY(ds_upload_grow(gd.cgr_ent, cg_ent, s, &gd)); TSL_TRY(ds_upload_grow(gd.cgr_ld, cg_ld, s, &gd)); TSL_TRY(ds_upload_grow(gd.cgr_dst, cg_dst, s, &gd));
   TSL_TRY(ds_upload_grow(gd.wl_front, M.wl_front, s, &gd)); TSL_TRY(ds_upload_grow(gd.wl_row, M.wl_row, s, &gd));
+  {
+    const size_t nr = (size_t)vtx_base[n];
+    std::vector<size_t> xs0(n + 1, 0), xc0(n + 1, 0);
+    for (int i = 0; i < n; i++) {
+      const DirectPlan& P = G->m[i]->ds.plan;
+      if (P.xs_ptr.size() != P.vtx.size() + 1) return tsl_fail("scene group: member %d has no row lists", i);
+      xs0[i + 1] = xs0[i] + P.xs_col.size();
+      xc0[i + 1] = xc0[i] + ((G->m[i]->nc > 0 && P.xc_ptr.size() == P.vtx.size() + 1) ? P.xc_col.size() : 0);
+    }
+    std::vector<int>& xs = gd.h_xs;
+    std::vector<int>& xc = gd.h_xc;
+    const size_t nx = xs0[n], ncg = xc0[n];
+    xs.assign(nr + 1 + 2 * nx, 0); xc.assign(nr + 1 + 2 * ncg, 0);
+    for (int i = 0; i < n; i++) {
+      tsl_ctx* c = G->m[i];
+      const DirectPlan& P = c->ds.plan;
+      const int vo = (int)G->vals_off[i];
+      const bool hc = xc0[i + 1] > xc0[i];
+      for (size_t r = 0; r < P.vtx.size(); r++) {
+        xs[vtx_base[i] + r] = (int)xs0[i] + P.xs_ptr[r];
+        xc[vtx_base[i] + r] = (int)xc0[i] + (hc ? P.xc_ptr[r] : 0);
+      }
+      for (size_t k = 0; k < P.xs_col.size(); k++) { xs[nr + 1 + xs0[i] + k] = P.xs_col[k]; xs[nr + 1 + nx + xs0[i] + k] = c->ds.h_c2s[P.xs_q[k]] + vo; }
+      if (hc) for (size_t k = 0; k < P.xc_col.size(); k++) {
+        const int gm = gmap[i].empty() ? -1 : gmap[i][P.xc_grp[k]];
+        if (gm < 0) return tsl_fail("scene group: contact group of member %d outside the merged list", i);
+        xc[nr + 1 + xc0[i] + k] = P.xc_col[k]; xc[nr + 1 + ncg + xc0[i] + k] = gm;
+      }
+    }
+    xs[nr] = (int)nx; xc[nr] = (int)ncg;
+    gd.xs_rows = (int)nr; gd.xs_n = (int)nx; gd.xc_n = (int)ncg;
+    TSL_TRY(ds_upload_grow(gd.xs_tab, xs, s, &gd)); TSL_TRY(ds_upload_grow(gd.xc_tab, xc, s, &gd));
+  }
   if (gd.scr.n < (size_t)M.scratch) { if (gd.scr.alloc((size_t)M.scratch + (size_t)M.scratch / 8)) return -1; }
   HIP_OK(hipStreamSynchronize(s));
   gd.plan_valid = true; gd.numeric_valid = false; gd.have_factor = false;
diff --git a/thinshelllab_amd/csrc/direct_host.hpp b/thinshelllab_amd/csrc/direct_host.hpp
--- a/thinshelllab_amd/csrc/direct_host.hpp
+++ b/thinshelllab_amd/csrc/direct_host.hpp
@@ -75,17 +75,33 @@
   if (mode == 0) hipLaunchKernelGGL((k_ds_gemm<0, 4>), grid, dim3(256), 0, s, D, b.first, 0);
   else hipLaunchKernelGGL((k_ds_gemm<1, 4>), grid, dim3(256), 0, s, D, b.first, 0);
 }
-static void ds_launch_extend(hipStream_t s, const DsDev& D, int lv0, int nf, int max_ld, int part = 0, int max_span = 0) {
+static void ds_launch_extend(hipStream_t s, const DsDev& D, const DsXTab& X, int lv0, int nf, int max_ld, int part = 0, int max_span = 0) {
   const int xspan = part == 1 ? 64 * DS_XU : DS_XSPAN;
   const int nsp = ((part == 0 ? max_ld : max_span) + xspan - 1) / xspan;
   if (nsp <= 0) return;
-  hipLaunchKernelGGL(k_ds_extend_panels, dim3(((max_ld / 3 + 2 + 3) / 4) * nsp, nf), dim3(256), 0, s, D, lv0, nsp, part, xspan);
+  hipLaunchKernelGGL(k_ds_extend_panels, dim3(((max_ld / 3 + 2 + 3) / 4) * nsp, nf), dim3(256), 0, s, D, lv0, nsp, part, xspan, X);
+}
+static DsXTab ds_xtab(const tsl_ctx* c) {
+  const DirectSolver& d = c->ds;
+  DsXTab X = {nullptr, nullptr, nullptr, nullptr, nullptr, nullptr, nullptr, nullptr, nullptr, nullptr};
+  if (!d.fused_start || d.xs_rows <= 0) return X;
+  X.sptr = d.xs_tab.p; X.scol = X.sptr + d.xs_rows + 1; X.ssrc = X.scol + d.xs_n;
+  X.vals = c->vals.p;
+  if (c->nc > 0 && d.xc_n > 0) {
+    X.cptr = d.xc_tab.p; X.ccol = X.cptr + d.xs_rows + 1; X.cgrp = X.ccol + d.xc_n;
+    X.gptr = d.cgr_ptr.p; X.gent = d.cgr_ent.p; X.H = c->c_H.p;
+  }
+  return X;
 }
 static void ds_launch_level_start(tsl_ctx* c, hipStream_t s, const DsDev& D, int l, int part = 0, const DsBatch* b = nullptr) {
   DirectSolver& d = c->ds;
   const DirectPlan& P = d.plan;
   const int lv0 = P.level_ptr[l], nf = P.level_ptr[l + 1] - lv0;
-  if (l > 0) ds_launch_extend(s, D, lv0, nf, P.level_maxld[l], part, part == 0 ? 0 : part == 1 ? b->max_pp : std::max(b->max_bp, b->max_pp));
+  if (l > 0) {
+    const DsXTab X = ds_xtab(c);
+    ds_launch_extend(s, D, X, lv0, nf, P.level_maxld[l], part, part == 0 ? 0 : part == 1 ? b->max_pp : std::max(b->max_bp, b->max_pp));
+    if (X.sptr != nullptr) return;
+  }
   const int i0 = part == 2 ? P.blk_lmid[l] : P.blk_lptr[l], i1 = part == 1 ? P.blk_lmid[l] : P.blk_lptr[l + 1];
   const int nb = i1 - i0, npad = part == 2 ? 0 : nf;
   const long nt = (long)nb * 9 + (long)npad * DS_T;
@@ -216,8 +232,14 @@
   const DirectPlan& P = d.plan;
   TSL_TRY(ds_upload_grow(d.cgr_ptr, P.cgr_ptr, s, &d)); TSL_TRY(ds_upload_grow(d.cgr_ent, P.cgr_ent, s, &d)); TSL_TRY(ds_upload_grow(d.cgr_ld, P.cgr_ld, s, &d));
   TSL_TRY(ds_upload_grow(d.cgr_dst, P.cgr_dst, s, &d));
+  std::vector<int>& xc = d.h_xc;
+  xc.assign(P.xc_ptr.begin(), P.xc_ptr.end());
+  xc.insert(xc.end(), P.xc_col.begin(), P.xc_col.end()); xc.insert(xc.end(), P.xc_grp.begin(), P.xc_grp.end());
+  d.xc_n = (int)P.xc_col.size();
+  TSL_TRY(ds_upload_grow(d.xc_tab, xc, s, &d));
   return 0;
 }
+static size_t ds_xtab_pin(const DirectPlan& P) { return 4 * (P.xs_ptr.size() + 2 * P.xs_col.size() + P.xc_ptr.size() + 2 * P.xc_col.size()) + 1024; }
 
 static int direct_static(tsl_ctx* c) {
   DirectSolver& d = c->ds;
@@ -253,13 +275,14 @@
   d.plan.lists.swap(sl.plan.lists); d.plan.locs.swap(sl.plan.locs); d.plan.tpos.swap(sl.plan.tpos);
   d.level_sn.swap(sl.level_sn); d.pmap.swap(sl.pmap); d.ch_rec.swap(sl.ch_rec); d.vtx.swap(sl.vtx); d.blk_ld.swap(sl.blk_ld); 
   d.wl_front.swap(sl.wl_front); d.wl_row.swap(sl.wl_row); d.blk_dst.swap(sl.blk_dst); d.fr.swap(sl.fr); d.frl.swap(sl.frl); d.blk_q.swap(sl.blk_q); d.cgr_ptr.swap(sl.cgr_ptr); d.cgr_ent.swap(sl.cgr_ent); d.cgr_ld.swap(sl.cgr_ld); d.cgr_dst.swap(sl.cgr_dst);
+  d.xs_tab.swap(sl.xs_tab); d.xc_tab.swap(sl.xc_tab); std::swap(d.xs_rows, sl.xs_rows); std::swap(d.xs_n, sl.xs_n); std::swap(d.xc_n, sl.xc_n);
 }
 
 static size_t ds_slot_bytes(const DsPlanSlot& sl) {
   const DirectPlan& P = sl.plan;
-  size_t b = 4 * (sl.level_sn.n + sl.pmap.n + sl.vtx.n + sl.blk_ld.n + sl.cgr_ptr.n + sl.cgr_ent.n + sl.cgr_ld.n + sl.wl_front.n + sl.wl_row.n + sl.blk_q.n) + 8 * (sl.blk_dst.n + sl.cgr_dst.n) +
+  size_t b = 4 * (sl.level_sn.n + sl.pmap.n + sl.vtx.n + sl.blk_ld.n + sl.cgr_ptr.n + sl.cgr_ent.n + sl.cgr_ld.n + sl.wl_front.n + sl.wl_row.n + sl.blk_q.n + sl.xs_tab.n + sl.xc_tab.n) + 8 * (sl.blk_dst.n + sl.cgr_dst.n) +
              sizeof(DsFrontDesc) * (sl.fr.n + sl.frl.n) + sizeof(DsChildRec) * sl.ch_rec.n;
-  b += 4 * (P.pmap.size() + P.vtx.size() + P.blk_ld.size() + P.blk_q.size() + P.wl_front.size() + P.wl_row.size() + P.level_sn.size()) + 8 * P.blk_dst.size() + sizeof(DsFrontDesc) * P.fr.size();
+  b += 4 * (P.pmap.size() + P.vtx.size() + P.blk_ld.size() + P.blk_q.size() + P.wl_front.size() + P.wl_row.size() + P.level_sn.size() + P.xs_ptr.size() + 2 * P.xs_col.size() + P.xc_ptr.size() + 2 * P.xc_col.size()) + 8 * P.blk_dst.size() + sizeof(DsFrontDesc) * P.fr.size();
   return b;
 }
 static void ds_cache_trim(DirectSolver& d) {
@@ -270,6 +293,7 @@
     if (!lru || total <= (size_t)d.cache_mb << 20) return;
     lru->used = false;
     lru->level_sn.release(); lru->pmap.release(); lru->vtx.release(); lru->blk_ld.release(); lru->cgr_ptr.release(); lru->cgr_ent.release(); lru->cgr_ld.release(); lru->cgr_dst.release(); lru->wl_front.release(); lru->wl_row.release();
+    lru->xs_tab.release(); lru->xc_tab.release();
     lru->blk_q.release(); lru->blk_dst.release(); lru->fr.release(); lru->frl.release(); lru->ch_rec.release();
     d.n_plan_evicted++;
   }
@@ -298,7 +322,7 @@
     if (cons != d.h_cons) {
       HIP_OK(hipStreamSynchronize(s));
       if (d.plan.build_con(cons.data(), c->nc)) return tsl_fail("direct solver: constraint vertex outside its front");
-      ds_pin_reset(d, 20 * (d.plan.cgr_ent.size() + d.plan.cgr_ptr.size()) + 4096);
+      ds_pin_reset(d, 20 * (d.plan.cgr_ent.size() + d.plan.cgr_ptr.size()) + 4096 + ds_xtab_pin(d.plan));
       TSL_TRY(ds_upload_con(d, s));
       HIP_OK(hipStreamSynchronize(s));
       d.h_cons = cons;
@@ -346,7 +370,7 @@
   HIP_OK(hipStreamSynchronize(s));
   const size_t nbk = P.blk_q.size();
   ds_pin_reset(d, 16 * nbk + 2 * sizeof(DsFrontDesc) * P.fr.size() + sizeof(DsChildRec) * P.ch_rec.size() +
-                      4 * (P.level_sn.size() + P.pmap.size() + vtxp.size() + P.wl_front.size() + P.wl_row.size()) + 20 * (P.cgr_ent.size() + P.cgr_ptr.size()) + 64 * 256);
+                      4 * (P.level_sn.size() + P.pmap.size() + vtxp.size() + P.wl_front.size() + P.wl_row.size()) + 20 * (P.cgr_ent.size() + P.cgr_ptr.size()) + 64 * 256 + ds_xtab_pin(P));
   TSL_TRY(ds_upload_grow(d.fr, P.fr, s, &d)); TSL_TRY(ds_upload_grow(d.level_sn, P.level_sn, s, &d)); TSL_TRY(ds_upload_grow(d.pmap, P.pmap, s, &d)); TSL_TRY(ds_upload_grow(d.ch_rec, P.ch_rec, s, &d));
   TSL_TRY(ds_upload_grow(d.vtx, vtxp, s, &d));
   {
@@ -368,6 +392,15 @@
     }
   }
   TSL_TRY(ds_upload_con(d, s));
+  {
+    std::vector<int>& xs = d.h_xs;
+    const size_t nr1 = P.xs_ptr.size(), nx = P.xs_col.size();
+    xs.resize(nr1 + 2 * nx);
+    std::copy(P.xs_ptr.begin(), P.xs_ptr.end(), xs.begin()); std::copy(P.xs_col.begin(), P.xs_col.end(), xs.begin() + nr1);
+    for (size_t i = 0; i < nx; i++) xs[nr1 + nx + i] = d.h_c2s[P.xs_q[i]];
+    d.xs_rows = (int)nr1 - 1; d.xs_n = (int)nx;
+    TSL_TRY(ds_upload_grow(d.xs_tab, xs, s, &d));
+  }
   std::vector<DsFrontDesc> frl(P.level_sn.size());
   for (size_t i = 0; i < frl.size(); i++) frl[i] = P.fr[P.level_sn[i]];
   TSL_TRY(ds_upload_grow(d.frl, frl, s, &d));
@@ -710,7 +743,7 @@
       const int tp = b.max_pp / DS_T, tb = b.max_bp / DS_T;
       if (cls == 6) {
         if (b.level == 0) continue;
-        ds_launch_extend(s, D, b.first, b.count, b.max_pp + b.max_bp);
+        ds_launch_extend(s, D, ds_xtab(c), b.first, b.count, b.max_pp + b.max_bp);
         if (count) {
           launches++;
           for (int i = 0; i < nf; i++) {
diff --git a/thinshelllab_amd/csrc/direct_plan.hpp b/thinshelllab_amd/csrc/direct_plan.hpp
--- a/thinshelllab_amd/csrc/direct_plan.hpp
+++ b/thinshelllab_amd/csrc/direct_plan.hpp
@@ -1,4 +1,5 @@
 #pragma once
+#include <array>
 #include <atomic>
 #include <chrono>
 #include <thread>
@@ -72,6 +73,10 @@
   std::vector<int> con_ld, con_lvl;
   std::vector<int> cgr_lptr, cgr_ptr, cgr_ent, cgr_ld;
   std::vector<long long> cgr_dst;
+  std::vector<int> xs_ptr, xs_col, xs_q, xc_ptr, xc_col, xc_grp;
+  std::vector<int> con_row, con_col;
+  std::vector<std::vector<int>> xs_tmp;
+  std::vector<long long> xs_at;
   std::vector<int> level_maxld;
   long long arena_leaf = 0;
   std::vector<std::pair<long long, long long>> leaf_ranges;
@@ -98,6 +103,22 @@
   double flops = 0;
 
   static int pad(int n) { return (n + DS_T - 1) / DS_T * DS_T; }
+
+  void item_entries(const DsFrontDesc& f, int g, int c0, int c1, std::vector<std::array<int, 4>>& st, std::vector<std::array<int, 4>>& cg) const {
+    const int row = f.vtx_off + g;
+    const int r0 = g < f.nv_own ? 3 * g : 3 * (g - f.nv_own);
+    for (int i = xs_ptr[row]; i < xs_ptr[row + 1]; i++)
+      for (int cc = 0; cc < 3; cc++) {
+        const int j = xs_col[i] + cc;
+        if (j >= c0 && j < c1) for (int k = 0; k < 3; k++) st.push_back({xs_q[i], 3 * k + cc, r0 + k, j});
+      }
+    if (!xc_ptr.empty())
+      for (int i = xc_ptr[row]; i < xc_ptr[row + 1]; i++)
+        for (int cc = 0; cc < 3; cc++) {
+          const int j = xc_col[i] + cc;
+          if (j >= c0 && j < c1) for (int k = 0; k < 3; k++) cg.push_back({xc_grp[i], 3 * k + cc, r0 + k, j});
+        }
+  }
 
   int local_dof(int s, int v) const {
     const int l = sym.local(s, v);
@@ -285,6 +306,9 @@
       for (auto& v : lists) v.clear();
       std::atomic<int> bad{0};
       std::atomic<long long> written{0};
+      if ((int)xs_tmp.size() < 3 * nt) xs_tmp.resize((size_t)3 * nt);
+      for (int t = 0; t < 2 * nt; t++) xs_tmp[t].clear();
+      xs_ptr.assign(vtx.size() + 1, 0); xs_at.assign(S, -1);
       ds_parallel_for(S, nt, 16, [&](int t, int s) {
         std::vector<int>& loc = locs[t];
         if ((int)loc.size() != NV) loc.assign(NV, -1);
@@ -294,6 +318,10 @@
         const int no = f.nv_own;
         long long nw = 0;
         const int* fv = &vtx[f.vtx_off];
+        const bool rows = alap[s] > 0;
+        std::vector<int>& xt = xs_tmp[2 * t];
+        std::vector<int>& xw = xs_tmp[2 * t + 1];
+        xw.clear();
         for (int i = 0; i < no; i++) loc[fv[i]] = 3 * i;
         for (int i = 0; i < f.nv_bnd; i++) loc[fv[no + i]] = f.pp + 3 * i;
         for (int i = 0; i < no; i++) {
@@ -306,11 +334,26 @@
             if (lc < 0) { bad = 1; continue; }
             const int q = row_ptr[r] + k;
             blk_dst[q] = f.off + (long long)(3 * i) * f.ld + lc; blk_ld[q] = f.ld; nw++; (lc < f.pp ? mine11 : mine).push_back(q);
+            if (rows) { xw.push_back(i); xw.push_back(lc); xw.push_back(q); }
             if (sym.sn_of[c] > s) {
               const int qt = tpos[q];
-              if (qt >= 0) { blk_dst[qt] = f.off21 + (long long)(lc - f.pp) * f.pp + 3 * i; blk_ld[qt] = f.pp; nw++; mine.push_back(qt); }
+              if (qt >= 0) {
+                blk_dst[qt] = f.off21 + (long long)(lc - f.pp) * f.pp + 3 * i; blk_ld[qt] = f.pp; nw++; mine.push_back(qt);
+                if (rows) { xw.push_back(no + (lc - f.pp) / 3); xw.push_back(3 * i); xw.push_back(qt); }
+              }
             }
           }
+        }
+        if (rows) {
+          int* cnt = &xs_ptr[f.vtx_off + 1];
+          for (size_t k = 0; k < xw.size(); k += 3) cnt[xw[k]]++;
+          const size_t base = xt.size();
+          xs_at[s] = ((long long)t << 40) | (long long)base;
+          xt.resize(base + 2 * (xw.size() / 3));
+          std::vector<int>& at = xs_tmp[2 * nt + t];
+          at.assign((size_t)no + f.nv_bnd + 1, 0);
+          for (int i = 0; i < no + f.nv_bnd; i++) at[i + 1] = at[i] + cnt[i];
+          for (size_t k = 0; k < xw.size(); k += 3) { const int w = at[xw[k]]++; xt[base + 2 * w] = xw[k + 1]; xt[base + 2 * w + 1] = xw[k + 2]; }
         }
         for (int i = 0; i < no + f.nv_bnd; i++) loc[fv[i]] = -1;
         written += nw;
@@ -325,6 +368,15 @@
         }
         blk_lptr[l + 1] = (int)o;
       }
+      for (size_t r = 0; r < vtx.size(); r++) xs_ptr[r + 1] += xs_ptr[r];
+      xs_col.resize(xs_ptr[vtx.size()]); xs_q.resize(xs_ptr[vtx.size()]);
+      ds_parallel_for(S, xs_ptr[vtx.size()] > (1 << 18) ? nt : 1, 64, [&](int, int s) {
+        if (xs_at[s] < 0) return;
+        const DsFrontDesc& f = fr[s];
+        const int* src = xs_tmp[2 * (size_t)(xs_at[s] >> 40)].data() + (xs_at[s] & ((1LL << 40) - 1));
+        const int o = xs_ptr[f.vtx_off], n = xs_ptr[f.vtx_off + f.nv_own + f.nv_bnd] - o;
+        for (int k = 0; k < n; k++) { xs_col[o + k] = src[2 * k]; xs_q[o + k] = src[2 * k + 1]; }
+      });
     }
     arena_leaf = 0;
     for (int q = level_ptr[0]; q < level_ptr[1]; q++) { const DsFrontDesc& f = fr[level_sn[q]]; arena_leaf = std::max(arena_leaf, f.off21 + (long long)f.bp * f.pp); }
@@ -338,6 +390,7 @@
 
   int build_con(const int* cons, int n_cons) {
     con_dst.assign((size_t)n_cons * 16, -1); con_ld.assign((size_t)n_cons * 16, 0); con_lvl.assign((size_t)n_cons * 16, 0);
+    con_row.assign((size_t)n_cons * 16, 0); con_col.assign((size_t)n_cons * 16, 0);
     for (int e = 0; e < n_cons; e++)
       for (int a = 0; a < 4; a++)
         for (int b = 0; b < 4; b++) {
@@ -351,6 +404,8 @@
           con_dst[(size_t)e * 16 + a * 4 + b] = dst;
           con_ld[(size_t)e * 16 + a * 4 + b] = ldq;
           con_lvl[(size_t)e * 16 + a * 4 + b] = 2 * sym.level[s] + ((lr < fr[s].pp && lc < fr[s].pp) ? 0 : 1);
+          con_row[(size_t)e * 16 + a * 4 + b] = fr[s].vtx_off + (lr < fr[s].pp ? lr / 3 : fr[s].nv_own + (lr - fr[s].pp) / 3);
+          con_col[(size_t)e * 16 + a * 4 + b] = lc;
         }
     {
       const size_t n = (size_t)n_cons * 16;
@@ -372,6 +427,13 @@
       }
       cgr_ptr.push_back((int)n);
       for (int l = 0; l < n_levels; l++) { cgr_lmid[l] += cgr_lptr[l]; cgr_lptr[l + 1] += cgr_lptr[l]; }
+      const int g1 = (int)cgr_dst.size(), g0 = n_levels > 0 ? cgr_lptr[1] : g1;
+      xc_ptr.assign(vtx.size() + 1, 0);
+      for (int g = g0; g < g1; g++) xc_ptr[con_row[cgr_ent[cgr_ptr[g]]] + 1]++;
+      for (size_t r = 0; r < vtx.size(); r++) xc_ptr[r + 1] += xc_ptr[r];
+      xc_col.resize(g1 - g0); xc_grp.resize(g1 - g0);
+      std::vector<int> at(xc_ptr.begin(), xc_ptr.end() - 1);
+      for (int g = g0; g < g1; g++) { const int x = cgr_ent[cgr_ptr[g]], w = at[con_row[x]]++; xc_col[w] = con_col[x]; xc_grp[w] = g; }
     }
     return 0;
   }
diff --git a/thinshelllab_amd/csrc/k_direct.hpp b/thinshelllab_amd/csrc/k_direct.hpp
--- a/thinshelllab_amd/csrc/k_direct.hpp
+++ b/thinshelllab_amd/csrc/k_direct.hpp
@@ -1043,10 +1043,16 @@
     }
 }
 
+struct DsXTab {
+  const int *sptr, *scol, *ssrc;
+  const int *cptr, *ccol, *cgrp;
+  const int *gptr, *gent;
+  const double *vals, *H;
+};
 #define DS_XU 4
 #define DS_XSPAN 1024
 #define DS_XMAXC 64
-__global__ void __launch_bounds__(256) k_ds_extend_panels(DsDev D, int lv0, int nsp, int part, int xspan) {
+__global__ void __launch_bounds__(256) k_ds_extend_panels(DsDev D, int lv0, int nsp, int part, int xspan, DsXTab X) {
   const DsFrontDesc f = D.frl[lv0 + blockIdx.y];
   const int ib = blockIdx.x / nsp, sp = blockIdx.x - ib * nsp;
   const int lane = threadIdx.x & 63, w = __builtin_amdgcn_readfirstlane(threadIdx.x >> 6);
@@ -1062,13 +1068,29 @@
   if (g >= ng) {
     const int nrow = top ? f.pp - f.p : f.bp - f.b;
     double* base = top ? D.A + f.off + (size_t)f.p * f.ld : D.A + f.off21 + (size_t)f.b * f.pp;
+    const int dg = (top && X.sptr != nullptr) ? f.p : -1 - nrow;
     for (int i = 0; i < nrow; i++)
-      for (int j = c0 + lane; j < c1; j += 64) base[(size_t)i * ncol + j] = 0.0;
+      for (int j = c0 + lane; j < c1; j += 64) base[(size_t)i * ncol + j] = j == dg + i ? 1.0 : 0.0;
     return;
   }
   const int r = top ? 3 * g : f.pp + 3 * (g - f.nv_own);
   double* row = top ? D.A + f.off + (size_t)r * f.ld : D.A + f.off21 + (size_t)(r - f.pp) * f.pp;
   const DsChildRec* ch = D.ch + f.ch_off;
+  int xs0 = 0, xs1 = 0, xcol = -1;
+  double xa[3] = {0.0, 0.0, 0.0};
+  if (X.sptr != nullptr) {
+    xs0 = X.sptr[f.vtx_off + g]; xs1 = X.sptr[f.vtx_off + g + 1];
+    const int bi = xs0 + lane / 3, cc = lane % 3;
+    if (lane < 63 && bi < xs1) {
+      const int j = X.scol[bi] + cc;
+      if (j >= c0 && j < c1) {
+        xcol = j;
+        const double* a = X.vals + (size_t)X.ssrc[bi] + 64 * cc;
+#pragma unroll
+        for (int k = 0; k < 3; k++) xa[k] = a[192 * k];
+      }
+    }
+  }
   if (f.nchild <= DS_XMAXC) {
     int my_ci = -1, my_off = 0, my_bp = 0;
     long long my_soff = 0;
@@ -1130,8 +1152,7 @@
         }
       }
     }
-    return;
-  }
+  } else
   for (int j = c0 + lane; j < c1; j += 64) {
     double v[3] = {0.0, 0.0, 0.0};
     for (int q = 0; q < f.nchild; q++) {
@@ -1144,6 +1165,52 @@
     }
 #pragma unroll
     for (int k = 0; k < 3; k++) row[(size_t)k * ncol + j] = v[k];
+  }
+  if (X.sptr == nullptr) return;
+  if (xs1 > xs0) {
+    __threadfence_block();
+    if (xcol >= 0) {
+#pragma unroll
+      for (int k = 0; k < 3; k++) { double* a = &row[(size_t)k * ncol + xcol]; *a = *a + xa[k]; }
+    }
+    for (int b0 = xs0 + 21; b0 < xs1; b0 += 21) {
+      const int bi = b0 + lane / 3, cc = lane % 3;
+      if (lane < 63 && bi < xs1) {
+        const int j = X.scol[bi] + cc;
+        if (j >= c0 && j < c1) {
+          const double* a = X.vals + (size_t)X.ssrc[bi] + 64 * cc;
+#pragma unroll
+          for (int k = 0; k < 3; k++) { double* d = &row[(size_t)k * ncol + j]; *d = *d + a[192 * k]; }
+        }
+      }
+    }
+  }
+  if (X.cptr == nullptr) return;
+  const int xc0 = X.cptr[f.vtx_off + g], xc1 = X.cptr[f.vtx_off + g + 1];
+  if (xc1 <= xc0) return;
+  __threadfence_block();
+  for (int i = xc0; i < xc1; i++) {
+    const int col = X.ccol[i];
+    if (col + 3 <= c0 || col >= c1) continue;
+    const int gq = X.cgrp[i];
+    double v[9] = {0, 0, 0, 0, 0, 0, 0, 0, 0};
+    for (int k = X.gptr[gq] + lane; k < X.gptr[gq + 1]; k += 64) {
+      const int x = X.gent[k], c = x >> 4, sub = x & 15;
+      const double* Hb = X.H + (size_t)c * 144 + (3 * (sub >> 2)) * 12 + 3 * (sub & 3);
+#pragma unroll
+      for (int r = 0; r < 3; r++)
+#pragma unroll
+        for (int cc = 0; cc < 3; cc++) v[3 * r + cc] += Hb[12 * r + cc];
+    }
+#pragma unroll
+    for (int e = 0; e < 9; e++) v[e] = wave_sum(v[e]);
+    if (lane == 0) {
+#pragma unroll
+      for (int r = 0; r < 3; r++)
+#pragma unroll
+        for (int cc = 0; cc < 3; cc++)
+          if (col + cc >= c0 && col + cc < c1) row[(size_t)r * ncol + col + cc] += v[3 * r + cc];
+    }
   }
 }
 
diff --git a/thinshelllab_amd/csrc/tsl_ctx.hpp b/thinshelllab_amd/csrc/tsl_ctx.hpp
--- a/thinshelllab_amd/csrc/tsl_ctx.hpp
+++ b/thinshelllab_amd/csrc/tsl_ctx.hpp
@@ -101,6 +101,8 @@
   bool used = false;
   DevBuf<int> level_sn, pmap, vtx, blk_ld, wl_front, wl_row, blk_q, cgr_ptr, cgr_ent, cgr_ld;
   DevBuf<long long> blk_dst, cgr_dst;
+  DevBuf<int> xs_tab, xc_tab;
+  int xs_rows = 0, xs_n = 0, xc_n = 0;
   DevBuf<DsFrontDesc> fr, frl;
   DevBuf<DsChildRec> ch_rec;
 };
@@ -159,6 +161,10 @@
   bool plan_valid = false;
   DevBuf<int> level_sn, pmap, vtx, blk_ld, bad, wl_front, wl_row, blk_q, cgr_ptr, cgr_ent, cgr_ld;
   DevBuf<long long> blk_dst, cgr_dst;
+  DevBuf<int> xs_tab, xc_tab;
+  int xs_rows = 0, xs_n = 0, xc_n = 0;
+  std::vector<int> h_xs, h_xc;
+  int fused_start = 1;
   DevBuf<DsFrontDesc> fr, frl;
   DevBuf<DsChildRec> ch_rec;
   DevBuf<double> arena, sarena, garena, scr, w;
diff --git a/thinshelllab_amd/csrc/tsl_hip.hip b/thinshelllab_amd/csrc/tsl_hip.hip
--- a/thinshelllab_amd/csrc/tsl_hip.hip
+++ b/thinshelllab_amd/csrc/tsl_hip.hip
@@ -481,6 +481,7 @@
   else if (k == "direct_gemv_wide_below") c->ds.gemv_wide_below = std::max(0, (int)v);
   else if (k == "direct_g32_below") c->ds.g32_below = std::max(0, (int)v);
   else if (k == "direct_lookahead") c->ds.lookahead = (int)v;
+  else if (k == "direct_fused_start") c->ds.fused_start = v != 0.0 ? 1 : 0;
   else if (k == "direct_piv_tol") { c->ds.piv_tol = v; c->ds.numeric_valid = false; }
   else if (k == "direct_leaf") { c->ds.leaf = std::max(4, (int)v); c->ds.static_ready = false; c->ds.plan_valid = false; c->ds.numeric_valid = false; }
   else if (k == "gmres_m") c->gmres_m = (int)v;
@@ -2375,7 +2376,7 @@
     }
     if (gd.piv_tol != d0.piv_tol) gd.piv_tol = d0.piv_tol;
     gd.flow = G->flow_lost ? 0 : d0.flow; gd.g32_below = d0.g32_below; gd.gemv_wide_below = d0.gemv_wide_below; gd.small_rounds = d0.small_rounds * n; gd.xcd_map = d0.xcd_map;
-    gd.prezero = d0.prezero; gd.dbg = d0.dbg;
+    gd.prezero = d0.prezero; gd.dbg = d0.dbg; gd.fused_start = d0.fused_start;
   }
   ss.assign(n, tsl_solve_stats{});
   std::vector<char> okv(n, 1);
```

New measurement: 519,300, median of 2. Within noise of the previous version (+0.1%).
